# david-m-rosen/Optimization

Hardware: AMD Instinct MI355X
Metric: TNT Steihaug-CG HVP+inner-product throughput (higher is better)
Workload: dtype f64

## Files before the change

### include/mi355opt.h

```cpp
#ifndef MI355OPT_H
#define MI355OPT_H

#include <stddef.h>
#include <stdint.h>

#ifdef __cplusplus
extern "C" {
#endif

#define MI_API __attribute__((visibility("default")))

typedef enum mi_status {
  MI_OK = 0,
  MI_ERR_INVALID_ARGUMENT = 1,
  MI_ERR_HIP = 2,
  MI_ERR_OOM = 3,
  MI_ERR_NO_DEVICE = 4,
  MI_ERR_COMM = 5,
  MI_ERR_INTERNAL = 6,
  MI_DECLINED = 7
} mi_status;

typedef struct mi_ctx mi_ctx;
typedef struct mi_vec mi_vec;
typedef struct mi_csr mi_csr;
typedef struct mi_bsr3 mi_bsr3;
typedef struct mi_op mi_op;
typedef struct mi_precon mi_precon;
typedef struct mi_stiefel_rq mi_stiefel_rq;
typedef struct mi_so3n mi_so3n;

MI_API const char *mi_version(void);
MI_API const char *mi_last_error(void);
MI_API const char *mi_status_string(int status);
MI_API int mi_device_count(int *count);
MI_API int mi_ctx_create(int device, mi_ctx **out);
MI_API int mi_ctx_destroy(mi_ctx *ctx);
MI_API int mi_ctx_sync(mi_ctx *ctx);
MI_API int mi_ctx_sync_count(mi_ctx *ctx, size_t *count);
typedef struct mi_fusion_counters {
  unsigned long long fused_stpcg_solves;
  unsigned long long generic_stpcg_solves;
  unsigned long long fused_lsqr_solves;
  unsigned long long generic_lsqr_solves;
  unsigned long long fused_trial_steps;
  unsigned long long generic_trial_steps;
  unsigned long long generic_inner_products;
} mi_fusion_counters;
enum { MI_GENERIC_STPCG = 0, MI_GENERIC_LSQR = 1, MI_GENERIC_TRIAL = 2 };
MI_API int mi_ctx_fusion_counters(mi_ctx *ctx, mi_fusion_counters *out);
MI_API int mi_ctx_fusion_counters_reset(mi_ctx *ctx);
MI_API int mi_ctx_note_generic(mi_ctx *ctx, int what, const char *why);
MI_API int mi_ctx_stream(mi_ctx *ctx, void **stream);
MI_API int mi_ctx_device_name(mi_ctx *ctx, char *buf, size_t buflen);
MI_API int mi_ctx_pool_bytes(mi_ctx *ctx, size_t *bytes_reserved);

enum {
  MI_K_NONE = 0,
  MI_K_CG_INIT, MI_K_CG_DOT3, MI_K_CG_SCALAR_A, MI_K_CG_UPDATE, MI_K_CG_SCALAR_B, MI_K_CG_PUPDATE,
  MI_K_SPMM, MI_K_STIEFEL_SPMM_GRAM, MI_K_STIEFEL_GRAM_REDUCE, MI_K_STIEFEL_FINISH_DOTS,
  MI_K_STIEFEL_RETRACT, MI_K_BSR3_SPMV_DOTS, MI_K_BLAS1, MI_K_LOBPCG_GRAM, MI_K_LOBPCG_UPDATE,
  MI_K_LOBPCG_RESIDUAL, MI_K_STIEFEL_HESS_FUSED,
  MI_K_COMM_ALLREDUCE,
  MI_K_COMM_HALO,
  MI_K_SO3_GRAD,
  MI_K_SO3_RESIDUAL,
  MI_K_SO3_JAC,
  MI_K_SO3_JACT,
  MI_K_SO3_EDGE_WEIGHT,
  MI_K_SO3_INC_REWEIGHT,
  MI_K_COUNT
};
MI_API int mi_ctx_set_option(mi_ctx *ctx, const char *name, long value);
MI_API int mi_ktime_enable(mi_ctx *ctx, int kernel_id, int on);
MI_API int mi_ktime_reset(mi_ctx *ctx);
MI_API int mi_ktime_read(mi_ctx *ctx, int kernel_id, size_t *launches, double *total_ms);
MI_API const char *mi_kernel_name(int kernel_id);
MI_API int mi_range_push(const char *name);
MI_API int mi_range_pop(void);
MI_API int mi_timer_start(mi_ctx *ctx);
MI_API int mi_timer_stop(mi_ctx *ctx, double *ms);

MI_API int mi_vec_create(mi_ctx *ctx, size_t n, mi_vec **out);
MI_API int mi_vec_destroy(mi_vec *v);
MI_API int mi_vec_view(const mi_vec *base, size_t offset, size_t n, mi_vec **out);
MI_API int mi_vec_len(const mi_vec *v, size_t *n);
MI_API int mi_vec_data(const mi_vec *v, void **device_ptr);
MI_API int mi_vec_touch(mi_vec *v);
MI_API int mi_vec_upload(mi_vec *v, const double *host, size_t n);
MI_API int mi_vec_download(const mi_vec *v, double *host, size_t n);
MI_API int mi_vec_copy(mi_vec *dst, const mi_vec *src);
MI_API int mi_vec_fill(mi_vec *v, double a);
MI_API int mi_vec_scale(mi_vec *v, double a);
MI_API int mi_vec_div(mi_vec *v, double a);
MI_API int mi_vec_scale_to(mi_vec *z, double a, const mi_vec *x);
MI_API int mi_vec_axpy(mi_vec *y, double a, const mi_vec *x);
MI_API int mi_vec_axpby(mi_vec *z, double a, const mi_vec *x, double b, const mi_vec *y);
MI_API int mi_vec_dot(const mi_vec *x, const mi_vec *y, double *out);
MI_API int mi_vec_dot_batch(mi_ctx *ctx, int k, const mi_vec *const *x, const mi_vec *const *y,
                            double *out);

MI_API int mi_csr_create(mi_ctx *ctx, size_t n, size_t nnz, const int32_t *rowptr,
                         const int32_t *col, const double *val, mi_csr **out);
MI_API int mi_csr_destroy(mi_csr *A);
MI_API int mi_csr_spmm(const mi_csr *A, int p, const mi_vec *V, mi_vec *W);

typedef int (*mi_apply_fn)(void *user, const mi_vec *in, mi_vec *out);
MI_API int mi_op_create_callback(mi_ctx *ctx, size_t n, mi_apply_fn fn, void *user, mi_op **out);
MI_API int mi_op_create_callback_rect(mi_ctx *ctx, size_t n_in, size_t n_out, mi_apply_fn fn, void *user,
                                      mi_op **out);
typedef struct mi_fused_args {
  double *partials;
  size_t partial_stride;
  int max_rows;
  int required_rows;
  void *stream;
} mi_fused_args;
typedef int (*mi_apply_fused_fn)(void *user, const mi_vec *in, mi_vec *out, const mi_fused_args *args, int *rows);
MI_API int mi_op_create_callback_fused(mi_ctx *ctx, size_t n, mi_apply_fn fn, mi_apply_fused_fn fused, void *user,
                                       mi_op **out);
MI_API int mi_op_create_diag(mi_ctx *ctx, const mi_vec *d, mi_op **out);
MI_API int mi_op_create_csr(mi_ctx *ctx, const mi_csr *A, int p, mi_op **out);
MI_API int mi_op_create_compose(mi_ctx *ctx, mi_op *outer, mi_op *inner, mi_op **out);
MI_API int mi_op_apply(mi_op *op, const mi_vec *in, mi_vec *out);
MI_API int mi_op_dims(const mi_op *op, size_t *n_in, size_t *n_out);
MI_API int mi_op_destroy(mi_op *op);

MI_API int mi_precon_create_callback(mi_ctx *ctx, size_t n, mi_apply_fn fn, void *user,
                                     mi_precon **out);
MI_API int mi_precon_create_diag(mi_ctx *ctx, const mi_vec *dinv, mi_precon **out);
MI_API int mi_precon_create_block3(mi_ctx *ctx, const mi_vec *inv_blocks, mi_precon **out);
MI_API int mi_precon_create_constraint(mi_ctx *ctx, size_t n, size_t m, const mi_vec *A_rowmajor,
                                       const mi_vec *Minv_diag, mi_precon **out);
MI_API int mi_precon_create_constraint_csr(mi_ctx *ctx, size_t n, size_t m, const int32_t *rowptr, const int32_t *col,
                                           const double *val, const mi_vec *Minv, double inner_tol,
                                           size_t inner_max_iterations, mi_precon **out);
MI_API int mi_precon_constraint_info(mi_precon *P, size_t *last_inner_iterations, double *last_relative_residual,
                                     double *worst_relative_residual, int *status_code );
MI_API int mi_precon_constraint_solve(mi_precon *P, const mi_vec *r, mi_vec *v, mi_vec *lambda );
MI_API int mi_precon_constraint_At(mi_precon *P, const mi_vec *lambda, mi_vec *out);
MI_API int mi_precon_apply(mi_precon *P, const mi_vec *r, mi_vec *v);
MI_API int mi_precon_destroy(mi_precon *P);

typedef struct mi_stpcg_params {
  double Delta;
  size_t max_iterations;
  double kappa_fgr;
  double theta;
  double epsilon;
  int run_ahead;
  int constraint_At;
  int defer_result;
} mi_stpcg_params;

enum {
  MI_STPCG_EXIT_RESIDUAL = 0,
  MI_STPCG_EXIT_MAXIT = 1,
  MI_STPCG_EXIT_KERNEL = 2,
  MI_STPCG_EXIT_BOUNDARY = 3,
  MI_STPCG_EXIT_USER = 4
};

typedef struct mi_stpcg_result {
  double update_step_M_norm;
  size_t num_iterations;
  int exit_reason;
  size_t hvp_calls;
  double rv_final;
  int precon_status;
} mi_stpcg_result;

typedef struct mi_stpcg_trace {
  size_t cap, len;
  double *alpha, *beta, *kappa, *rv;
} mi_stpcg_trace;

MI_API void mi_stpcg_default_params(mi_stpcg_params *p);
MI_API int mi_stpcg(mi_ctx *ctx, const mi_vec *g, mi_op *H, mi_precon *P ,
                    const mi_stpcg_params *params, mi_vec *s_out, mi_stpcg_result *result,
                    mi_stpcg_trace *trace );
MI_API int mi_stpcg_observer_available(mi_ctx *ctx, const char **why);
typedef int (*mi_stpcg_observer)(void *user, size_t k, const mi_vec *s, const mi_vec *r, const mi_vec *v,
                                 const mi_vec *p, double alpha);
MI_API int mi_stpcg_observed(mi_ctx *ctx, const mi_vec *g, mi_op *H, mi_precon *P ,
                             const mi_stpcg_params *params, mi_stpcg_observer fn, void *user, mi_vec *s_out,
                             mi_stpcg_result *result, mi_stpcg_trace *trace );
MI_API int mi_stpcg_collect(mi_ctx *ctx, mi_stpcg_result *result);

typedef struct mi_lsqr_params {
  size_t max_iterations;
  double lambda;
  double btol, Atol;
  double Acond_limit;
  double Delta;
  int run_ahead;
} mi_lsqr_params;
enum {
  MI_LSQR_EXIT_MAXIT = 0,
  MI_LSQR_EXIT_S1 = 1,
  MI_LSQR_EXIT_S2 = 2,
  MI_LSQR_EXIT_S3 = 3,
  MI_LSQR_EXIT_S4 = 4,
  MI_LSQR_EXIT_TRIVIAL = 5,
  MI_LSQR_EXIT_USER = 6
};
typedef struct mi_lsqr_result {
  double xnorm;
  size_t num_iterations;
  int exit_reason;
  double rbar_norm, Arnorm, Anorm, Acond;
  size_t operator_applications;
} mi_lsqr_result;
MI_API void mi_lsqr_default_params(mi_lsqr_params *p);
MI_API int mi_lsqr(mi_ctx *ctx, mi_op *A, mi_op *At, const mi_vec *b, const mi_lsqr_params *params,
                   mi_vec *x_out, mi_lsqr_result *result);
MI_API int mi_lsqr_observer_available(mi_ctx *ctx, const char **why);
typedef int (*mi_lsqr_observer)(void *user, size_t k, const mi_vec *x, double xnorm, double rbar_norm, double Arnorm,
                                double Anorm, double Acond);
MI_API int mi_lsqr_observed(mi_ctx *ctx, mi_op *A, mi_op *At, const mi_vec *b, const mi_lsqr_params *params,
                            mi_lsqr_observer fn, void *user, mi_vec *x_out, mi_lsqr_result *result);


MI_API int mi_stiefel_gram(mi_ctx *ctx, size_t n, int p, const mi_vec *X, const mi_vec *Z,
                           double *G_host );
MI_API int mi_stiefel_project(mi_ctx *ctx, size_t n, int p, const mi_vec *X, const mi_vec *Z,
                              mi_vec *out);
MI_API int mi_stiefel_retract(mi_ctx *ctx, size_t n, int p, const mi_vec *X, const mi_vec *V,
                              mi_vec *Y);
MI_API int mi_stiefel_rq_create(mi_ctx *ctx, const mi_csr *A, size_t n, int p, mi_stiefel_rq **out);
MI_API int mi_stiefel_rq_destroy(mi_stiefel_rq *prob);
MI_API int mi_stiefel_rq_objective(mi_stiefel_rq *prob, const mi_vec *X, double *f);
MI_API int mi_stiefel_rq_model(mi_stiefel_rq *prob, const mi_vec *X, mi_vec *grad, mi_op **hess);
MI_API int mi_stiefel_rq_trial(mi_stiefel_rq *prob, const mi_vec *X, const mi_vec *h, const mi_vec *g,
                               mi_vec *X_trial, double out[5]);
MI_API int mi_stiefel_rq_armijo_trial(mi_stiefel_rq *prob, const mi_vec *X, const mi_vec *g, double t, mi_vec *h_out,
                                      mi_vec *X_trial, double out[2]);
MI_API int mi_stiefel_rq_precon(mi_stiefel_rq *prob, const mi_vec *X, const mi_vec *dinv_rows,
                                mi_precon **out);

MI_API int mi_so3n_create(mi_ctx *ctx, size_t N, size_t n_edges, const int32_t *ei,
                          const int32_t *ej, const double *Rt , const double *w,
                          mi_so3n **out);
MI_API int mi_so3n_destroy(mi_so3n *prob);
MI_API int mi_so3n_objective(mi_so3n *prob, const mi_vec *R, double *f);
MI_API int mi_so3n_model(mi_so3n *prob, const mi_vec *R, mi_vec *grad, mi_op **hess,
                         mi_precon **block_jacobi );
MI_API int mi_so3n_retract(mi_so3n *prob, const mi_vec *R, const mi_vec *xi, mi_vec *Y);
MI_API int mi_so3n_trial(mi_so3n *prob, const mi_vec *R, const mi_vec *h, const mi_vec *g, int with_precon,
                         mi_vec *R_trial, double out[6]);
MI_API int mi_so3n_gradient(mi_so3n *prob, const mi_vec *R, mi_vec *grad);
MI_API int mi_so3n_armijo_trial(mi_so3n *prob, const mi_vec *R, const mi_vec *g, double t, mi_vec *h_out,
                                mi_vec *R_trial, double out[2]);
MI_API int mi_so3n_residual(mi_so3n *prob, const mi_vec *R, mi_vec *F_out, double *sqnorm_or_null);
MI_API int mi_so3n_jacobian(mi_so3n *prob, const mi_vec *R, mi_op **dF, mi_op **dFt);
MI_API int mi_so3n_gn_scaling(mi_so3n *prob, mi_op **M);
typedef struct mi_so3n_cert mi_so3n_cert;
struct mi_panel_blocks;
MI_API int mi_so3n_certificate(mi_so3n *prob, const mi_vec *R, mi_so3n_cert **out, double info[3]);
MI_API int mi_so3n_cert_apply(mi_so3n_cert *cert, int k, const mi_vec *X, mi_vec *Z);
MI_API int mi_so3n_cert_apply_blocks(mi_so3n_cert *cert, const struct mi_panel_blocks *X, mi_vec *Z);
MI_API int mi_so3n_cert_null_panel(mi_so3n_cert *cert, mi_vec **Y);
MI_API int mi_so3n_laplacian(mi_so3n *prob, mi_so3n_cert **out);
MI_API int mi_so3n_lap_jacobi(mi_so3n *prob, int k, const mi_vec *X, mi_vec *Z);
MI_API int mi_so3n_round(mi_so3n *prob, const mi_vec *V, mi_vec *R, double info[4]);
MI_API int mi_so3n_project(mi_so3n *prob, const mi_vec *M, mi_vec *R, double info[3]);
enum { MI_ROBUST_L2 = 0, MI_ROBUST_HUBER = 1, MI_ROBUST_CAUCHY = 2, MI_ROBUST_GEMAN_MCCLURE = 3 };
MI_API int mi_so3n_reweight(mi_so3n *prob, const mi_vec *R, int kind, double c, double info[3]);
MI_API int mi_so3n_weights(mi_so3n *prob, double *w_host );

MI_API int mi_lobpcg_gram(mi_ctx *ctx, size_t m, int ka, int kb, const mi_vec *S, const mi_vec *AS,
                          double *G_host);
MI_API int mi_lobpcg_gram_split(mi_ctx *ctx, size_t m, int k, const mi_vec *S, int k1, const mi_vec *T1,
                                const mi_vec *T2, double *G_host);
MI_API int mi_lobpcg_gram_pair(mi_ctx *ctx, size_t m, int k, const mi_vec *S, int k1a, const mi_vec *Ta1,
                               const mi_vec *Ta2, int k1b, const mi_vec *Tb1, const mi_vec *Tb2, double *Ga_host,
                               double *Gb_host);
MI_API int mi_lobpcg_gram_pair_sym(mi_ctx *ctx, size_t m, int k, const mi_vec *S, int k1a, const mi_vec *Ta1,
                                   const mi_vec *Ta2, double *Ga_host, double *Gb_host);
typedef struct mi_panel_blocks {
  int nblocks;
  const mi_vec *block[3];
  int cols[3];
} mi_panel_blocks;
MI_API int mi_lobpcg_gram_pair_sym_blocks(mi_ctx *ctx, size_t m, const mi_panel_blocks *S, int k1a, const mi_vec *Ta1,
                                          const mi_vec *Ta2, double *Ga_host, double *Gb_host);
MI_API int mi_lobpcg_gram_pair_sym_tblocks(mi_ctx *ctx, size_t m, const mi_panel_blocks *S, const mi_panel_blocks *T,
                                           double *Ga_host, double *Gb_host);
MI_API int mi_lobpcg_gram_pair_gen_blocks(mi_ctx *ctx, size_t m, const mi_panel_blocks *S, const mi_panel_blocks *AS,
                                          const mi_panel_blocks *BS, double *Ga_host, double *Gb_host);
MI_API int mi_lobpcg_update2_blocks(mi_ctx *ctx, size_t m, const mi_panel_blocks *S, int kc, const double *C_host,
                                    int ldc, mi_vec *Y, int k1, mi_vec *Y2);
MI_API int mi_csr_spmm_colmajor_blocks(const mi_csr *A, const mi_panel_blocks *X, mi_vec *Y);
MI_API int mi_lobpcg_update(mi_ctx *ctx, size_t m, int ks, int kc, const mi_vec *S,
                            const double *C_host, int ldc, mi_vec *Y);
MI_API int mi_lobpcg_update2(mi_ctx *ctx, size_t m, int ks, int kc, const mi_vec *S, const double *C_host, int ldc,
                             mi_vec *Y, int k1, mi_vec *Y2);
MI_API int mi_lobpcg_residual(mi_ctx *ctx, size_t m, int nx, const mi_vec *AX, const mi_vec *BX,
                              const mi_vec *X, const double *theta_host, mi_vec *R, double *rnorm,
                              double *xnorm);
MI_API int mi_rayleigh_ritz(int n, const double *A, const double *B, double *Theta, double *C);
MI_API int mi_rayleigh_ritz_lowest(int n, int k, const double *A, const double *B, double *Theta, double *C);
MI_API int mi_csr_spmm_colmajor(const mi_csr *A, int k, const mi_vec *X, mi_vec *Y);
MI_API int mi_csr_spmm_colmajor_residual(const mi_csr *A, int nx, const mi_vec *X, const double *theta_host,
                                         mi_vec *AX, mi_vec *R, double *rnorm, double *xnorm);
MI_API int mi_panel_rowscale(mi_ctx *ctx, size_t m, int k, const mi_vec *d, const mi_vec *X, mi_vec *Y);

#define MI_COMM_UID_BYTES 128
MI_API int mi_comm_unique_id(unsigned char uid[MI_COMM_UID_BYTES]);
MI_API int mi_comm_init(mi_ctx *ctx, int world_size, int rank,
                        const unsigned char uid[MI_COMM_UID_BYTES]);
MI_API int mi_comm_finalize(mi_ctx *ctx);
MI_API int mi_comm_info(mi_ctx *ctx, int *world_size, int *rank);
MI_API int mi_comm_rccl_count(mi_ctx *ctx, int *nranks);
#define MI_COMM_IPC_HANDLE_BYTES 64
MI_API int mi_comm_ipc_export(mi_ctx *ctx, unsigned char handle[MI_COMM_IPC_HANDLE_BYTES]);
MI_API int mi_comm_ipc_attach(mi_ctx *ctx, int world_size, int rank,
                              const unsigned char *handles );
MI_API int mi_comm_ipc_selftest(mi_ctx *ctx, int *ok);
MI_API int mi_comm_ipc_enable(mi_ctx *ctx, int on);
MI_API int mi_comm_ipc_error(mi_ctx *ctx, int *err);
MI_API int mi_comm_ipc_fold(mi_ctx *ctx, int on);
MI_API int mi_comm_kernel_launches(mi_ctx *ctx, unsigned long long out[4]);
MI_API int mi_debug_csr_window_info(const mi_csr *A, size_t out[4]);
MI_API int mi_debug_csr_format_info(const mi_csr *A, size_t out[5]);
MI_API int mi_debug_so3n_info(const mi_so3n *q, size_t out[6]);
MI_API int mi_debug_op_apply_sub_scaled(mi_op *op, const mi_vec *in, double scale, int mode, mi_vec *inout,
                                        double *sqnorm);
MI_API int mi_debug_window_runs(int ntiles, int max_wgs, int num_cu, size_t far_stride, int *bounds_out, int cap,
                                int *nb_out);
MI_API int mi_debug_stiefel_hess_form(int p, int gram_count, const size_t traits[9], const int switches[9], int out[14]);
MI_API int mi_debug_stiefel_hess_form_of(const mi_ctx *ctx, const mi_csr *A, int p, int gram_count, int out[14]);
MI_API int mi_debug_words16_option(const char *text, int *on);
MI_API int mi_debug_set_rank(mi_ctx *ctx, int world_size, int rank);
MI_API int mi_debug_csr_set_halo(mi_csr *A, int p, const double *halo_rows_host);
MI_API int mi_debug_time_fused_apply(mi_op *op, const mi_vec *in, mi_vec *out, int reps, double *us_per_call);
MI_API int mi_csr_shard_plan(size_t n_global, int world_size, int rank, const size_t *row_starts,
                             size_t nnz_local, const int64_t *col_global, int32_t *col_local, size_t *need_lo,
                             size_t *need_hi);
MI_API int mi_csr_create_sharded(mi_ctx *ctx, size_t n_global, size_t row_begin, size_t row_end,
                                 size_t nnz_local, const int32_t *rowptr, const int64_t *col_global,
                                 const double *val, const size_t *row_starts ,
                                 mi_csr **out);

#ifdef __cplusplus
}
#endif
#endif
```

### optimization_amd/build.py

```python
import concurrent.futures
import glob
import os
import subprocess
import sys

HERE = os.path.dirname(os.path.abspath(__file__))
ROOT = os.path.dirname(HERE)
CSRC = os.path.join(HERE, "csrc")
_TAG = os.environ.get("MI355OPT_BUILD_TAG", "")
OBJ = os.path.join(HERE, "_build" + ("_" + _TAG if _TAG else ""))
LIB = os.path.join(HERE, "libmi355opt" + ("_" + _TAG if _TAG else "") + ".so")
HIPCC = os.environ.get("HIPCC", "/opt/rocm/bin/hipcc")
ARCH = "gfx950"

CFLAGS = [
    f"--offload-arch={ARCH}", "-O3", "-std=c++17", "-fPIC", "-fvisibility=hidden",
    "-fgpu-rdc" if False else "-fno-gpu-rdc", "-Wall", "-Wno-unused-function",
    "-I", os.path.join(ROOT, "include"), "-I", CSRC, "-I", os.path.join(HERE, "include"), "-I", "/opt/rocm/include",
]
CFLAGS += os.environ.get("MI355OPT_EXTRA_CFLAGS", "").split()
LDFLAGS = ["-shared", "-L/opt/rocm/lib", "-lrccl", "-ldl", "-Wl,-rpath,/opt/rocm/lib", "-Wl,--no-undefined"]


def _newer(src, dst, deps):
    if not os.path.exists(dst):
        return True
    t = os.path.getmtime(dst)
    return any(os.path.getmtime(f) > t for f in [src] + deps)


def _compile(src, force):
    obj = os.path.join(OBJ, os.path.basename(src) + ".o")
    deps = glob.glob(os.path.join(CSRC, "*.h")) + glob.glob(os.path.join(ROOT, "include", "*.h")) + \
        glob.glob(os.path.join(HERE, "include", "Optimization", "LinearAlgebra", "DenseSymmetricEigen.h"))
    if not force and not _newer(src, obj, deps):
        return obj, False, ""
    cmd = [HIPCC] + CFLAGS + ["-c", src, "-o", obj]
    r = subprocess.run(cmd, capture_output=True, text=True)
    if r.returncode != 0:
        raise RuntimeError(f"hipcc failed on {src}:\n{r.stderr[-6000:]}")
    return obj, True, r.stderr


HOST_CXX = os.environ.get("CXX", "g++")
HOST_CFLAGS = ["-O3", "-std=c++17", "-fPIC", "-fvisibility=hidden", "-ffp-contract=off", "-Wall",
               "-I", os.path.join(ROOT, "include"), "-I", CSRC, "-I", os.path.join(HERE, "include")]


def _compile_host(src, force):
    obj = os.path.join(OBJ, os.path.basename(src) + ".o")
    deps = glob.glob(os.path.join(HERE, "include", "Optimization", "LinearAlgebra", "*.h"))
    if not force and not _newer(src, obj, deps):
        return obj, False, ""
    import shutil
    if shutil.which(HOST_CXX):
        cmd = [HOST_CXX] + HOST_CFLAGS
    else:
        cmd = [HIPCC, "-x", "c++"] + HOST_CFLAGS
    r = subprocess.run(cmd + ["-c", src, "-o", obj], capture_output=True, text=True)
    if r.returncode != 0:
        raise RuntimeError(f"{cmd[0]} failed on {src}:\n{r.stderr[-6000:]}")
    return obj, True, r.stderr


UNITY = ["stpcg.hip", "stiefel.hip"]


def build(force=False, jobs=None, verbose=False):
    os.makedirs(OBJ, exist_ok=True)
    srcs = sorted(glob.glob(os.path.join(CSRC, "*.hip")))
    if not srcs:
        raise RuntimeError("no HIP sources found")
    if os.environ.get("MI355OPT_NO_UNITY") != "1":
        unity = os.path.join(OBJ, "hot_unity.hip")
        text = "".join(f'#include "{os.path.join(CSRC, u)}"\n' for u in UNITY)
        if not os.path.exists(unity) or open(unity).read() != text:
            with open(unity, "w") as f:
                f.write(text)
        newest = max(os.path.getmtime(os.path.join(CSRC, u)) for u in UNITY)
        if os.path.getmtime(unity) < newest:
            os.utime(unity, (newest, newest))
        srcs = [s_ for s_ in srcs if os.path.basename(s_) not in UNITY] + [unity]
    jobs = jobs or min(len(srcs), os.cpu_count() or 4)
    objs, rebuilt = [], False
    with concurrent.futures.ThreadPoolExecutor(max_workers=jobs) as ex:
        for obj, did, err in ex.map(lambda s: _compile(s, force), srcs):
            objs.append(obj)
            rebuilt |= did
            if verbose and err.strip():
                print(err, file=sys.stderr)
    for src in sorted(glob.glob(os.path.join(CSRC, "*.cpp"))):
        obj, did, err = _compile_host(src, force)
        objs.append(obj)
        rebuilt |= did
    if rebuilt or not os.path.exists(LIB):
        cmd = [HIPCC, f"--offload-arch={ARCH}"] + objs + LDFLAGS + ["-o", LIB]
        r = subprocess.run(cmd, capture_output=True, text=True)
        if r.returncode != 0:
            raise RuntimeError(f"link failed:\n{r.stderr[-6000:]}")
    return LIB


WLGEN_SRC = os.path.join(HERE, "wlgen.c")
WLGEN_LIB = os.path.join(HERE, "libmi355wl.so")


def build_wlgen(force=False):
    if force or _newer(WLGEN_SRC, WLGEN_LIB, []):
        r = subprocess.run(["gcc", "-O2", "-ffp-contract=off", "-fPIC", "-shared", "-Wall", "-Wextra", WLGEN_SRC,
                            "-o", WLGEN_LIB, "-lm"], capture_output=True, text=True)
        if r.returncode != 0:
            raise RuntimeError("wlgen build failed:\n" + r.stderr[-4000:])
    return WLGEN_LIB


def build_harness(force=False):
    tdir = os.path.join(ROOT, "tests", "cpp")
    inc = ["-I", os.path.join(HERE, "include"), "-I", os.path.join(ROOT, "oracle")]
    common = ["g++", "-std=c++17", "-O2", "-ffp-contract=off", "-fPIC", "-shared", "-Wall", "-Wno-type-limits"]
    hdrs = glob.glob(os.path.join(HERE, "include", "Optimization", "*", "*.h")) + \
        glob.glob(os.path.join(ROOT, "oracle", "*.inc")) + glob.glob(os.path.join(ROOT, "include", "*.h"))
    out = []
    host_src = os.path.join(tdir, "harness_host.cpp")
    host_so = os.path.join(tdir, "libharness_host.so")
    if force or _newer(host_src, host_so, hdrs):
        r = subprocess.run(common + ["-march=x86-64-v3"] + inc + [host_src, "-o", host_so],
                           capture_output=True, text=True)
        if r.returncode != 0:
            raise RuntimeError("host harness build failed:\n" + r.stderr[-6000:])
    out.append(host_so)
    dev_src = os.path.join(tdir, "harness_device.cpp")
    dev_so = os.path.join(tdir, "libharness_device.so")
    if force or _newer(dev_src, dev_so, hdrs + [LIB]):
        cmd = common + inc + ["-I", os.path.join(ROOT, "include"), dev_src, "-o", dev_so, "-L", HERE,
                              "-lmi355opt", "-Wl,-rpath," + HERE, "-Wl,-rpath,/opt/rocm/lib"]
        r = subprocess.run(cmd, capture_output=True, text=True)
        if r.returncode != 0:
            raise RuntimeError("device harness build failed:\n" + r.stderr[-6000:])
        clang = "/opt/rocm/lib/llvm/bin/clang++"
        if os.path.exists(clang):
            r = subprocess.run([clang, "-std=c++17", "-fsyntax-only"] + inc +
                               ["-I", os.path.join(ROOT, "include"), dev_src], capture_output=True, text=True)
            if r.returncode != 0:
                raise RuntimeError("clang front-end check of the template layer failed:\n" + r.stderr[-6000:])
    out.append(dev_so)
    ob_src = os.path.join(tdir, "harness_observer.cpp")
    ob_so = os.path.join(tdir, "libharness_observer.so")
    if force or _newer(ob_src, ob_so, hdrs + [LIB]):
        cmd = common + inc + ["-I", os.path.join(ROOT, "include"), ob_src, "-o", ob_so, "-L", HERE,
                              "-lmi355opt", "-Wl,-rpath," + HERE, "-Wl,-rpath,/opt/rocm/lib"]
        r = subprocess.run(cmd, capture_output=True, text=True)
        if r.returncode != 0:
            raise RuntimeError("observer harness build failed:\n" + r.stderr[-6000:])
    out.append(ob_so)
    for name in ("harness_args", "harness_lsqr_observer", "harness_gd_so3n", "harness_tnls_so3n", "harness_certify_so3n",
                 "harness_robust_so3n", "harness_spectral_so3n"):
        src = os.path.join(tdir, name + ".cpp")
        so = os.path.join(tdir, "lib" + name + ".so")
        if force or _newer(src, so, hdrs + [LIB]):
            clang = "/opt/rocm/lib/llvm/bin/clang++"
            if os.path.exists(clang):
                r = subprocess.run([clang, "-std=c++17", "-fsyntax-only"] + inc +
                                   ["-I", os.path.join(ROOT, "include"), src], capture_output=True, text=True)
                if r.returncode != 0:
                    raise RuntimeError(f"clang front-end check of {name} failed:\n" + r.stderr[-6000:])
            cmd = common + inc + ["-I", os.path.join(ROOT, "include"), src, "-o", so, "-L", HERE,
                                  "-lmi355opt", "-Wl,-rpath," + HERE, "-Wl,-rpath,/opt/rocm/lib"]
            r = subprocess.run(cmd, capture_output=True, text=True)
            if r.returncode != 0:
                raise RuntimeError(f"{name} build failed:\n" + r.stderr[-6000:])
        out.append(so)
    sf_src = os.path.join(tdir, "harness_sinfit.hip")
    sf_so = os.path.join(tdir, "libharness_sinfit.so")
    if force or _newer(sf_src, sf_so, hdrs + [LIB]):
        cmd = [HIPCC, f"--offload-arch={ARCH}", "-std=c++17", "-O2", "-fPIC", "-shared", "-Wall",
               "-I", os.path.join(HERE, "include"), "-I", os.path.join(ROOT, "include"), sf_src, "-o", sf_so,
               "-L", HERE, "-lmi355opt", "-Wl,-rpath," + HERE, "-Wl,-rpath,/opt/rocm/lib"]
        r = subprocess.run(cmd, capture_output=True, text=True)
        if r.returncode != 0:
            raise RuntimeError("sin-fit harness build failed:\n" + r.stderr[-6000:])
    out.append(sf_so)
    bc_src = os.path.join(ROOT, "tools", "bench_client.cpp")
    bc_so = os.path.join(ROOT, "tools", "libbench_client.so")
    if force or _newer(bc_src, bc_so, hdrs + [LIB]):
        cmd = common + ["-I", os.path.join(HERE, "include"), "-I", os.path.join(ROOT, "include"), bc_src, "-o", bc_so,
                        "-L", HERE, "-lmi355opt", "-Wl,-rpath," + HERE, "-Wl,-rpath,/opt/rocm/lib"]
        r = subprocess.run(cmd, capture_output=True, text=True)
        if r.returncode != 0:
            raise RuntimeError("bench client build failed:\n" + r.stderr[-6000:])
    out.append(bc_so)
    exdir = os.path.join(ROOT, "examples")
    os.makedirs(os.path.join(exdir, "bin"), exist_ok=True)
    for src in sorted(glob.glob(os.path.join(exdir, "*.cpp"))):
        exe = os.path.join(exdir, "bin", os.path.splitext(os.path.basename(src))[0])
        if force or _newer(src, exe, hdrs + [LIB]):
            cmd = ["g++", "-std=c++17", "-O2", "-Wall"] + inc + ["-I", os.path.join(ROOT, "include"), src, "-o", exe,
                   "-L", HERE, "-lmi355opt", "-Wl,-rpath," + HERE, "-Wl,-rpath,/opt/rocm/lib"]
            r = subprocess.run(cmd, capture_output=True, text=True)
            if r.returncode != 0:
                raise RuntimeError(f"example build failed ({src}):\n" + r.stderr[-6000:])
        out.append(exe)
    for src in sorted(glob.glob(os.path.join(exdir, "*.hip"))):
        exe = os.path.join(exdir, "bin", os.path.splitext(os.path.basename(src))[0])
        if force or _newer(src, exe, hdrs + [LIB]):
            cmd = [HIPCC, f"--offload-arch={ARCH}", "-std=c++17", "-O2", "-Wall"] + inc + \
                  ["-I", os.path.join(ROOT, "include"), src, "-o", exe, "-L", HERE, "-lmi355opt",
                   "-Wl,-rpath," + HERE, "-Wl,-rpath,/opt/rocm/lib"]
            r = subprocess.run(cmd, capture_output=True, text=True)
            if r.returncode != 0:
                raise RuntimeError(f"example build failed ({src}):\n" + r.stderr[-6000:])
        out.append(exe)
    return out


class SanitizerUnavailable(RuntimeError):
    """The host has no usable ASan / UBSan toolchain or runtime: a reason to SKIP the sanitizer target, never a reason
    to refuse the GPU library."""


def _sanitizer_probe(tdir, san):
    import tempfile
    with tempfile.TemporaryDirectory(dir=tdir) as d:
        src, exe = os.path.join(d, "p.c"), os.path.join(d, "p")
        with open(src, "w") as f:
            f.write("#include <stdlib.h>\nint main(void){void*p=malloc(8);free(p);return 0;}\n")
        try:
            r = subprocess.run(["gcc"] + san + [src, "-o", exe], capture_output=True, text=True)
        except FileNotFoundError as e:
            raise SanitizerUnavailable(str(e))
        if r.returncode != 0:
            raise SanitizerUnavailable("gcc cannot build with -fsanitize=address,undefined here:\n" + r.stderr[-800:])
        for opts in ("detect_leaks=1:abort_on_error=0", "detect_leaks=0:abort_on_error=0"):
            r = subprocess.run([exe], capture_output=True, text=True, env=dict(os.environ, ASAN_OPTIONS=opts))
            if r.returncode == 0:
                if "detect_leaks=0" in opts:
                    print("[build] warning: LeakSanitizer cannot run here (ptrace / seccomp restriction?): the sanitizer "
                          "target runs with detect_leaks=0 -- heap errors and undefined behaviour are still checked, "
                          "leaks are NOT", file=sys.stderr)
                return opts
        raise SanitizerUnavailable("a trivial sanitized program does not run here:\n" + r.stderr[-800:])


_SAN = ["-fsanitize=address,undefined", "-fno-sanitize-recover=all", "-fno-omit-frame-pointer", "-g", "-O1", "-ffp-contract=off"]


def build_sanitize(force=False, run=True):
    tdir = os.path.join(ROOT, "tests", "cpp")
    odir = os.path.join(ROOT, "oracle")
    exe = os.path.join(tdir, "sanitize_host")
    src = os.path.join(tdir, "sanitize_host.cpp")
    deps = glob.glob(os.path.join(HERE, "include", "Optimization", "*", "*.h")) + glob.glob(os.path.join(odir, "*.inc")) + \
        glob.glob(os.path.join(odir, "*.[ch]")) + [os.path.join(tdir, "harness_host.cpp")]
    san = _SAN
    asan_opts = _sanitizer_probe(tdir, san)
    if force or _newer(src, exe, deps):
        objs = []
        for c in ("oracle.c", "problems.c"):
            o = os.path.join(tdir, "san_" + c + ".o")
            r = subprocess.run(["gcc"] + san + ["-I", odir, "-c", os.path.join(odir, c), "-o", o],
                               capture_output=True, text=True)
            if r.returncode != 0:
                raise RuntimeError("sanitizer build failed:\n" + r.stderr[-4000:])
            objs.append(o)
        r = subprocess.run(["g++", "-std=c++17", "-Wall", "-Wno-type-limits"] + san +
                           ["-I", os.path.join(HERE, "include"), "-I", odir, "-I", tdir, src] + objs + ["-lm", "-o", exe],
                           capture_output=True, text=True)
        if r.returncode != 0:
            raise RuntimeError("sanitizer build failed:\n" + r.stderr[-6000:])
    if run:
        r = subprocess.run([exe], capture_output=True, text=True, timeout=600,
                           env=dict(os.environ, ASAN_OPTIONS=asan_opts, UBSAN_OPTIONS="print_stacktrace=1"))
        if r.returncode != 0 or "sanitize_host: ok" not in r.stdout:
            raise RuntimeError("the template layer failed under ASan/UBSan:\n" + r.stdout[-2000:] + r.stderr[-6000:])
    if os.path.exists(os.path.join(tdir, "sanitize_so3_pack.cpp")):
        build_sanitize_so3_pack(force=force, run=run)
    return exe


def build_sanitize_so3_pack(force=False, run=True):
    tdir = os.path.join(ROOT, "tests", "cpp")
    exe, src = os.path.join(tdir, "sanitize_so3_pack"), os.path.join(tdir, "sanitize_so3_pack.cpp")
    asan_opts = _sanitizer_probe(tdir, _SAN)
    if force or _newer(src, exe, [os.path.join(CSRC, "so3_pack.h")]):
        r = subprocess.run(["g++", "-std=c++17", "-Wall"] + _SAN + ["-I", CSRC, src, "-o", exe], capture_output=True, text=True)
        if r.returncode != 0:
            raise RuntimeError("sanitizer build failed:\n" + r.stderr[-6000:])
    if run:
        r = subprocess.run([exe], capture_output=True, text=True, timeout=600,
                           env=dict(os.environ, ASAN_OPTIONS=asan_opts, UBSAN_OPTIONS="print_stacktrace=1"))
        if r.returncode != 0 or "sanitize_so3_pack: ok" not in r.stdout:
            raise RuntimeError("so3_pack.h failed under ASan/UBSan:\n" + r.stdout[-2000:] + r.stderr[-6000:])
    return exe


if __name__ == "__main__":
    force = "--force" in sys.argv
    print(build(force=force, verbose=True))
    print(build_wlgen(force=force))
    print(build_harness(force=force))
    print(build_sanitize(force=force))
```

### optimization_amd/csrc/context.hip

```cpp
#include "mi_internal.h"
#include <chrono>
#include <cstring>
#include <strings.h>
#include <unistd.h>

#include <dlfcn.h>

namespace mi {

static thread_local char g_err[1024] = "";

void set_error(const char *fmt, ...) {
  va_list ap;
  va_start(ap, fmt);
  vsnprintf(g_err, sizeof(g_err), fmt, ap);
  va_end(ap);
}

int hip_fail(hipError_t e, const char *what, const char *file, int line) {
  set_error("HIP error %d (%s) in %s at %s:%d", (int)e, hipGetErrorString(e), what, file, line);
  (void)hipGetLastError();
  if (e == hipErrorNoDevice || e == hipErrorInvalidDevice) return MI_ERR_NO_DEVICE;
  if (e == hipErrorOutOfMemory) return MI_ERR_OOM;
  return MI_ERR_HIP;
}

static int readback_reserve(mi_ctx *ctx, size_t total) {
  if (total > ctx->readback_bytes) {
    MI_HIP(hipStreamSynchronize(ctx->stream));
    if (ctx->readback_host) (void)hipHostFree(ctx->readback_host);
    ctx->readback_host = nullptr;
    ctx->readback_bytes = 0;
    const size_t cap = std::max<size_t>(total, 256 * 1024);
    MI_HIP(hipHostMalloc(&ctx->readback_host, cap, hipHostMallocMapped | hipHostMallocCoherent));
    ctx->readback_bytes = cap;
  }
  return MI_OK;
}
int readback_area(mi_ctx *ctx, size_t bytes, void **host, void **dev) {
  MI_TRY(readback_reserve(ctx, bytes));
  *host = ctx->readback_host;
  MI_HIP(hipHostGetDevicePointer(dev, ctx->readback_host, 0));
  return MI_OK;
}
__global__ void k_host_flag(unsigned long long *flag, unsigned long long seq) {
  __hip_atomic_store(flag, seq, __ATOMIC_RELEASE, __HIP_MEMORY_SCOPE_SYSTEM);
}
unsigned long long poll_begin(mi_ctx *ctx, unsigned long long **flag_dev) {
  if (!ctx->poll_flag || ctx->cfg.no_polled_sync) return 0;
  if (hipHostGetDevicePointer((void **)flag_dev, ctx->poll_flag, 0) != hipSuccess) {
    (void)hipGetLastError();
    return 0;
  }
  return ++ctx->poll_seq;
}
static inline void cpu_relax() {
#if !defined(__HIP_DEVICE_COMPILE__) && (defined(__x86_64__) || defined(__i386__))
  __builtin_ia32_pause();
#endif
}
int poll_finish(mi_ctx *ctx, unsigned long long seq, const char *what) {
  if (seq) {
    const auto t0 = std::chrono::steady_clock::now();
    for (unsigned spins = 1;; ++spins) {
      if (__atomic_load_n(ctx->poll_flag, __ATOMIC_ACQUIRE) >= seq) return MI_OK;
      cpu_relax();
      if ((spins & 1023u) == 0 && std::chrono::steady_clock::now() - t0 > std::chrono::milliseconds(2)) break;
    }
  }
  const hipError_t e = hipStreamSynchronize(ctx->stream);
  if (e != hipSuccess) return hip_fail(e, what, __FILE__, __LINE__);
  return MI_OK;
}
int stream_wait(mi_ctx *ctx, const char *what) {
  ctx->host_syncs++;
  unsigned long long *dev = nullptr;
  const unsigned long long seq = poll_begin(ctx, &dev);
  if (seq) {
    hipLaunchKernelGGL(k_host_flag, dim3(1), dim3(1), 0, ctx->stream, dev, seq);
    if (hipGetLastError() != hipSuccess) return poll_finish(ctx, 0, what);
  }
  return poll_finish(ctx, seq, what);
}
int readback_sync(mi_ctx *ctx, int n, const void *const *dev, const size_t *bytes, void *const *host) {
  size_t total = 0;
  for (int i = 0; i < n; ++i) total += (bytes[i] + 63) / 64 * 64;
  MI_TRY(readback_reserve(ctx, total));
  size_t off = 0;
  hipError_t e = hipSuccess;
  for (int i = 0; i < n && e == hipSuccess; ++i) {
    e = hipMemcpyAsync((char *)ctx->readback_host + off, dev[i], bytes[i], hipMemcpyDeviceToHost, ctx->stream);
    off += (bytes[i] + 63) / 64 * 64;
  }
  if (e == hipSuccess) e = hipStreamSynchronize(ctx->stream);
  ctx->host_syncs++;
  if (e != hipSuccess) return hip_fail(e, "read-back", __FILE__, __LINE__);
  off = 0;
  for (int i = 0; i < n; ++i) {
    memcpy(host[i], (const char *)ctx->readback_host + off, bytes[i]);
    off += (bytes[i] + 63) / 64 * 64;
  }
  return MI_OK;
}

int ensure_device() {
  int count = 0;
  hipError_t e = hipGetDeviceCount(&count);
  if (e != hipSuccess || count <= 0) {
    (void)hipGetLastError();
    set_error("no HIP device available (hipGetDeviceCount: %s, count=%d); libmi355opt has no CPU "
              "fallback",
              hipGetErrorString(e), count);
    return MI_ERR_NO_DEVICE;
  }
  return MI_OK;
}

int pool_alloc(mi_ctx *ctx, size_t bytes, void **out) {
  if (bytes == 0) bytes = 8;
  bytes = (bytes + 255) & ~(size_t)255;
  auto it = ctx->pool_free.find(bytes);
  if (it != ctx->pool_free.end()) {
    *out = it->second;
    ctx->pool_free.erase(it);
    return MI_OK;
  }
  void *p = nullptr;
  hipError_t e = hipMalloc(&p, bytes);
  if (e != hipSuccess) {
    for (auto &kv : ctx->pool_free) {
      (void)hipFree(kv.second);
      ctx->pool_all.erase(kv.second);
      ctx->pool_bytes -= kv.first;
    }
    ctx->pool_free.clear();
    (void)hipGetLastError();
    e = hipMalloc(&p, bytes);
    if (e != hipSuccess) return hip_fail(e, "hipMalloc", __FILE__, __LINE__);
  }
  ctx->pool_all[p] = bytes;
  ctx->pool_bytes += bytes;
  *out = p;
  return MI_OK;
}

void pool_free(mi_ctx *ctx, void *p) {
  if (!p) return;
  auto it = ctx->pool_all.find(p);
  if (it == ctx->pool_all.end()) return;
  ctx->pool_free.insert({it->second, p});
}

int upload(void **dst, const void *src, size_t bytes) {
  void *p = nullptr;
  MI_HIP(hipMalloc(&p, bytes ? bytes : 8));
  const hipError_t e = bytes ? hipMemcpy(p, src, bytes, hipMemcpyHostToDevice) : hipSuccess;
  if (e != hipSuccess) {
    (void)hipFree(p);
    return hip_fail(e, "hipMemcpy(p, src, bytes, hipMemcpyHostToDevice)", __FILE__, __LINE__);
  }
  *dst = p;
  return MI_OK;
}

int stage_upload(mi_ctx *ctx, const void *src, size_t bytes, void *dst_dev) {
  MI_REQUIRE(bytes <= mi_ctx::kStageBytes, "staged upload of %zu bytes exceeds the slot size", bytes);
  const int slot = ctx->stage_next;
  ctx->stage_next = (slot + 1) % mi_ctx::kStageSlots;
  if (!ctx->stage_host[slot]) {
    MI_HIP(hipHostMalloc(&ctx->stage_host[slot], mi_ctx::kStageBytes, hipHostMallocDefault));
    MI_HIP(hipEventCreateWithFlags(&ctx->stage_ev[slot], hipEventDisableTiming));
  } else {
    MI_HIP(hipEventSynchronize(ctx->stage_ev[slot]));
  }
  memcpy(ctx->stage_host[slot], src, bytes);
  MI_HIP(hipMemcpyAsync(dst_dev, ctx->stage_host[slot], bytes, hipMemcpyHostToDevice, ctx->stream));
  MI_HIP(hipEventRecord(ctx->stage_ev[slot], ctx->stream));
  return MI_OK;
}

hipEvent_t event_get(mi_ctx *ctx) {
  if (!ctx->event_pool.empty()) {
    hipEvent_t e = ctx->event_pool.back();
    ctx->event_pool.pop_back();
    return e;
  }
  hipEvent_t e = nullptr;
  if (hipEventCreate(&e) != hipSuccess) return nullptr;
  return e;
}

KScope::KScope(mi_ctx *c, int kid) : ctx(c), id(kid) {
  if (ctx->ktime[id].enabled) {
    e0 = event_get(ctx);
    e1 = event_get(ctx);
    if (e0) (void)hipEventRecord(e0, ctx->stream);
  }
}
KScope::~KScope() {
  if (e0 && e1) {
    (void)hipEventRecord(e1, ctx->stream);
    ctx->ktime[id].pending.push_back({e0, e1});
  }
}

}

using namespace mi;

namespace {
struct OptionDesc {
  const char *name;
  int (*set)(mi_ctx *, long);
  bool integer = false;
};
#define OPT_BOOL(FN, FIELD) \
  int FN(mi_ctx *c, long v) { c->FIELD = v != 0; return MI_OK; }
OPT_BOOL(opt_force_slot_path, force_slot_path)
OPT_BOOL(opt_force_lockstep, force_lockstep)
OPT_BOOL(opt_no_dirgram, no_dirgram)
OPT_BOOL(opt_dirgram_direct, dirgram_direct)
OPT_BOOL(opt_force_uniform_grid, cfg.force_uniform_grid)
OPT_BOOL(opt_no_fold, cfg.no_fold)
OPT_BOOL(opt_halo_push_late, cfg.halo_push_late)
OPT_BOOL(opt_no_packed, cfg.no_packed)
OPT_BOOL(opt_no_window, cfg.no_window)
OPT_BOOL(opt_no_win_bounds, cfg.no_win_bounds)
OPT_BOOL(opt_no_far_computed, cfg.no_far_computed)
OPT_BOOL(opt_words16, cfg.words16)
OPT_BOOL(opt_no_spmm_stream, cfg.no_spmm_stream)
OPT_BOOL(opt_no_spmm_win, cfg.no_spmm_win)
OPT_BOOL(opt_no_spmm_sweep, cfg.no_spmm_sweep)
OPT_BOOL(opt_no_zero_copy, cfg.no_zero_copy)
OPT_BOOL(opt_no_polled_sync, cfg.no_polled_sync)
OPT_BOOL(opt_no_update_mfma, cfg.no_update_mfma)
OPT_BOOL(opt_halo_rprime, cfg.halo_rprime)
OPT_BOOL(opt_no_gram_half, cfg.no_gram_half)
OPT_BOOL(opt_so3_no_quat, cfg.so3_no_quat)
OPT_BOOL(opt_so3_no_rquat, cfg.so3_no_rquat)
OPT_BOOL(opt_early_s, cfg.early_s)
OPT_BOOL(opt_defer_s, cfg.defer_s)
OPT_BOOL(opt_no_fused_observer, cfg.no_fused_observer)
OPT_BOOL(opt_no_fused_lsqr_observer, cfg.no_fused_lsqr_observer)
OPT_BOOL(opt_no_update_pair, cfg.no_update_pair)
OPT_BOOL(opt_two_kernel_step, cfg.two_kernel_step)
OPT_BOOL(opt_warn_generic, warn_generic)
OPT_BOOL(opt_tall_prologue, cfg.tall_prologue)
#undef OPT_BOOL
int opt_max_grid(mi_ctx *c, long v) {
  c->max_grid = (int)std::min<long>(kMaxGrid, std::max<long>(1, v));
  return MI_OK;
}
int opt_wide_quad(mi_ctx *c, long v) {
  c->cfg.wide_quad = v < 0 ? -1 : v != 0;
  return MI_OK;
}
int opt_wide_window(mi_ctx *c, long v) {
  c->cfg.wide_window = v < 0 ? -1 : v != 0;
  return MI_OK;
}
int opt_so3_sort_nbr(mi_ctx *c, long v) {
  c->cfg.so3_sort_nbr = (int)v;
  return MI_OK;
}
int opt_sweep_zsegs(mi_ctx *c, long v) {
  c->cfg.sweep_zsegs = (int)std::max<long>(0, std::min<long>(v, 1024));
  return MI_OK;
}
int opt_reanchor(mi_ctx *c, long v) {
  c->cfg.reanchor = (int)std::max<long>(0, std::min<long>(v, 1 << 20));
  return MI_OK;
}
int opt_ipc_timeout_ms(mi_ctx *c, long v) {
  c->cfg.ipc_timeout_ms = std::max<long>(0, v);
  return MI_OK;
}
const OptionDesc kOptions[] = {
    {"FORCE_SLOT_PATH", opt_force_slot_path}, {"FORCE_LOCKSTEP", opt_force_lockstep},
    {"NO_DIRGRAM", opt_no_dirgram}, {"DIRGRAM_DIRECT", opt_dirgram_direct}, {"MAX_GRID", opt_max_grid, true},
    {"FORCE_UNIFORM_GRID", opt_force_uniform_grid}, {"IPC_TIMEOUT_MS", opt_ipc_timeout_ms, true},
    {"NO_FOLD", opt_no_fold}, {"HALO_PUSH_LATE", opt_halo_push_late}, {"NO_PACKED", opt_no_packed},
    {"NO_WINDOW", opt_no_window}, {"NO_WIN_BOUNDS", opt_no_win_bounds}, {"NO_FAR_COMPUTED", opt_no_far_computed},
    {"WORDS16", opt_words16, true}, {"NO_SPMM_STREAM", opt_no_spmm_stream}, {"NO_SPMM_WIN", opt_no_spmm_win},
    {"NO_SPMM_SWEEP", opt_no_spmm_sweep}, {"SWEEP_ZSEGS", opt_sweep_zsegs, true},
    {"NO_ZERO_COPY", opt_no_zero_copy}, {"NO_POLLED_SYNC", opt_no_polled_sync}, {"WIDE_QUAD", opt_wide_quad, true}, {"WIDE_WINDOW", opt_wide_window, true},
    {"NO_UPDATE_MFMA", opt_no_update_mfma}, {"HALO_RPRIME", opt_halo_rprime}, {"NO_GRAM_HALF", opt_no_gram_half}, {"SO3_NO_QUAT", opt_so3_no_quat}, {"SO3_NO_RQUAT", opt_so3_no_rquat}, {"EARLY_S", opt_early_s}, {"DEFER_S", opt_defer_s}, {"NO_FUSED_OBSERVER", opt_no_fused_observer}, {"NO_FUSED_LSQR_OBSERVER", opt_no_fused_lsqr_observer}, {"NO_UPDATE_PAIR", opt_no_update_pair}, {"TWO_KERNEL_STEP", opt_two_kernel_step}, {"SO3_SORT_NBR", opt_so3_sort_nbr, true},
    {"WARN_GENERIC", opt_warn_generic}, {"TALL_PROLOGUE", opt_tall_prologue}, {"REANCHOR", opt_reanchor, true},
};
bool option_value(const OptionDesc &o, const char *e, long *v) {
  char *end = nullptr;
  *v = strtol(e, &end, 0);
  if (end != e && *end == '\0') return true;
  if (o.integer) {
    fprintf(stderr, "[mi355opt] warning: MI355OPT_%s=\"%s\" is not an integer; ignored (the default stays)\n", o.name, e);
    return false;
  }
  *v = (!strcasecmp(e, "no") || !strcasecmp(e, "false") || !strcasecmp(e, "off")) ? 0 : 1;
  return true;
}
void config_from_env(mi_ctx *ctx) {
  for (const OptionDesc &o : kOptions) {
    char name[64];
    snprintf(name, sizeof(name), "MI355OPT_%s", o.name);
    long v = 0;
    if (const char *e = getenv(name))
      if (option_value(o, e, &v)) (void)o.set(ctx, v);
  }
  static bool warned = false;
  if (warned || !environ) return;
  warned = true;
  for (char **ep = environ; *ep; ++ep) {
    if (strncmp(*ep, "MI355OPT_", 9) != 0) continue;
    const char *nm = *ep + 9, *eq = strchr(nm, '=');
    const size_t len = eq ? (size_t)(eq - nm) : strlen(nm);
    bool known = false;
    for (const OptionDesc &o : kOptions) known |= strlen(o.name) == len && strncmp(o.name, nm, len) == 0;
    for (const char *h : {"LIB", "COMM", "BUILD_TAG", "EXTRA_CFLAGS", "NO_UNITY"})
      known |= strlen(h) == len && strncmp(h, nm, len) == 0;
    known |= len >= 6 && strncmp(nm, "BENCH_", 6) == 0;
    if (!known)
      fprintf(stderr, "[mi355opt] warning: environment variable MI355OPT_%.*s is not a switch of this build (removed "
                      "or misspelt?); it changes nothing\n", (int)len, nm);
  }
}
}

extern "C" {

const char *mi_version(void) { return "mi355opt 0.1.0 (gfx950)"; }
const char *mi_last_error(void) { return g_err; }
const char *mi_status_string(int s) {
  switch (s) {
    case MI_OK: return "ok";
    case MI_ERR_INVALID_ARGUMENT: return "invalid argument";
    case MI_ERR_HIP: return "HIP runtime error";
    case MI_ERR_OOM: return "out of device memory";
    case MI_ERR_NO_DEVICE: return "no MI355X/HIP device (no CPU fallback)";
    case MI_ERR_COMM: return "RCCL communicator error";
    case MI_ERR_INTERNAL: return "internal error";
    case MI_DECLINED: return "declined (nothing was done)";
  }
  return "unknown status";
}

static const char *kKernelNames[MI_K_COUNT] = {
    "none", "cg_init", "cg_dot3", "cg_scalar_a", "cg_update", "cg_scalar_b", "cg_pupdate",
    "csr_spmm", "stiefel_spmm_gram", "stiefel_gram_reduce", "stiefel_finish_dots",
    "stiefel_retract", "bsr3_spmv_dots", "blas1", "lobpcg_gram", "lobpcg_update",
    "lobpcg_residual", "stiefel_hess_fused", "comm_allreduce", "comm_halo", "so3_grad",
    "so3_residual", "so3_jac", "so3_jact", "so3_edge_weight", "so3_inc_reweight"};
const char *mi_kernel_name(int id) {
  if (id < 0 || id >= MI_K_COUNT) return "?";
  return kKernelNames[id];
}

int mi_ctx_set_option(mi_ctx *ctx, const char *name, long value) {
  MI_REQUIRE(ctx && name, "null argument");
  if (strncmp(name, "MI355OPT_", 9) == 0) name += 9;
  for (const OptionDesc &o : kOptions)
    if (strcmp(o.name, name) == 0) return o.set(ctx, value);
  set_error("unknown option '%s'", name);
  return MI_ERR_INVALID_ARGUMENT;
}

int mi_debug_words16_option(const char *text, int *on) {
  MI_REQUIRE(on, "null argument");
  mi_ctx scratch;
  long v = 0;
  for (const OptionDesc &o : kOptions)
    if (strcmp(o.name, "WORDS16") == 0 && text && option_value(o, text, &v)) (void)o.set(&scratch, v);
  *on = scratch.cfg.words16;
  return MI_OK;
}

int mi_device_count(int *count) {
  MI_REQUIRE(count, "count is null");
  int c = 0;
  hipError_t e = hipGetDeviceCount(&c);
  if (e != hipSuccess) {
    (void)hipGetLastError();
    c = 0;
  }
  *count = c;
  return MI_OK;
}

static int ctx_init(mi_ctx *ctx, int device) {
  ctx->device = device;
  hipDeviceProp_t prop;
  MI_HIP(hipGetDeviceProperties(&prop, device));
  snprintf(ctx->device_name, sizeof(ctx->device_name), "%s (%s, %d CUs)",
           prop.name[0] ? prop.name : "AMD Instinct", prop.gcnArchName, prop.multiProcessorCount);
  ctx->num_cu = prop.multiProcessorCount;
  MI_HIP(hipStreamCreateWithFlags(&ctx->stream, hipStreamNonBlocking));
  const size_t pbytes = sizeof(double) * kMaxComps * kMaxRows;
  const size_t slab_bytes = 4u << 20;
  MI_HIP(hipMalloc((void **)&ctx->control_slab, slab_bytes));
  MI_HIP(hipMemsetAsync(ctx->control_slab, 0, slab_bytes, ctx->stream));
  {
    char *top = (char *)ctx->control_slab;
    auto carve = [&](size_t bytes) {
      char *p = top;
      top += (bytes + 255) / 256 * 256;
      return p;
    };
    ctx->cg = (CgState *)carve(2 * sizeof(CgState));
    ctx->cg1 = ctx->cg + 1;
    ctx->scalars = (double *)carve(sizeof(double) * kScalarSlots);
    ctx->partials = (double *)carve(pbytes);
    ctx->partials_b = (double *)carve(pbytes);
    ctx->partials2 = (double *)carve(pbytes);
    ctx->partials_user = (double *)carve(pbytes);
    if ((size_t)(top - (char *)ctx->control_slab) > slab_bytes) {
      set_error("control slab overflow");
      return MI_ERR_INTERNAL;
    }
  }
  MI_HIP(hipHostMalloc((void **)&ctx->host_scalars, sizeof(double) * kScalarSlots,
                       hipHostMallocMapped | hipHostMallocCoherent));
  MI_HIP(hipHostMalloc((void **)&ctx->cg_host, sizeof(CgState) + 16, hipHostMallocMapped | hipHostMallocCoherent)  );
  MI_HIP(hipHostMalloc((void **)&ctx->status, sizeof(HostStatus),
                       hipHostMallocMapped | hipHostMallocCoherent));
  MI_HIP(hipHostMalloc((void **)&ctx->poll_flag, 64, hipHostMallocMapped | hipHostMallocCoherent));
  *ctx->poll_flag = 0;
  memset((void *)ctx->status, 0, sizeof(HostStatus));
  MI_HIP(hipHostGetDevicePointer((void **)&ctx->status_dev, (void *)ctx->status, 0));
  config_from_env(ctx);
  MI_HIP(hipEventCreate(&ctx->t_start));
  MI_HIP(hipEventCreate(&ctx->t_stop));
  return MI_OK;
}

int mi_comm_finalize(mi_ctx *ctx);
int mi_ctx_destroy(mi_ctx *ctx);

int mi_ctx_create(int device, mi_ctx **out) {
  MI_REQUIRE(out, "out is null");
  MI_TRY(ensure_device());
  MI_HIP(hipSetDevice(device));
  mi_ctx *ctx = new mi_ctx();
  const int st = ctx_init(ctx, device);
  if (st != MI_OK) {
    (void)mi_ctx_destroy(ctx);
    return st;
  }
  *out = ctx;
  return MI_OK;
}

int mi_ctx_destroy(mi_ctx *ctx) {
  if (!ctx) return MI_OK;
  (void)hipSetDevice(ctx->device);
  if (ctx->stream) (void)hipStreamSynchronize(ctx->stream);
  (void)mi_comm_finalize(ctx);
  for (auto &kv : ctx->pool_all) (void)hipFree(kv.first);
  for (int i = 0; i < MI_K_COUNT; ++i)
    for (auto &pr : ctx->ktime[i].pending) {
      (void)hipEventDestroy(pr.first);
      (void)hipEventDestroy(pr.second);
    }
  for (auto e : ctx->event_pool) (void)hipEventDestroy(e);
  for (int i = 0; i < mi_ctx::kStageSlots; ++i) {
    if (ctx->stage_ev[i]) (void)hipEventDestroy(ctx->stage_ev[i]);
    if (ctx->stage_host[i]) (void)hipHostFree(ctx->stage_host[i]);
  }
  (void)hipFree(ctx->control_slab);
  (void)hipFree(ctx->trace_dev);
  (void)hipHostFree(ctx->host_scalars);
  if (ctx->readback_host) (void)hipHostFree(ctx->readback_host);
  if (ctx->poll_flag) (void)hipHostFree(ctx->poll_flag);
  if (ctx->cg_deferred_ev) (void)hipEventDestroy(ctx->cg_deferred_ev);
  (void)hipHostFree(ctx->cg_host);
  (void)hipHostFree((void *)ctx->status);
  if (ctx->t_start) (void)hipEventDestroy(ctx->t_start);
  if (ctx->t_stop) (void)hipEventDestroy(ctx->t_stop);
  if (ctx->stream) (void)hipStreamDestroy(ctx->stream);
  (void)hipGetLastError();
  delete ctx;
  return MI_OK;
}

int mi_ctx_sync(mi_ctx *ctx) {
  MI_REQUIRE(ctx, "ctx is null");
  MI_HIP(hipStreamSynchronize(ctx->stream));
  ctx->host_syncs++;
  return MI_OK;
}

int mi_ctx_sync_count(mi_ctx *ctx, size_t *count) {
  MI_REQUIRE(ctx && count, "null argument");
  *count = ctx->host_syncs;
  return MI_OK;
}

int mi_ctx_fusion_counters(mi_ctx *ctx, mi_fusion_counters *out) {
  MI_REQUIRE(ctx && out, "null argument");
  *out = ctx->fusion;
  return MI_OK;
}

int mi_ctx_fusion_counters_reset(mi_ctx *ctx) {
  MI_REQUIRE(ctx, "ctx is null");
  ctx->fusion = mi_fusion_counters{0, 0, 0, 0, 0, 0, 0};
  return MI_OK;
}

int mi_ctx_note_generic(mi_ctx *ctx, int what, const char *why) {
  MI_REQUIRE(ctx, "ctx is null");
  MI_REQUIRE(what >= 0 && what <= 2, "bad kind %d", what);
  static const char *const kKind[3] = {"STPCG", "LSQR", "TNT / GradientDescent trial step"};
  if (what == MI_GENERIC_STPCG) ctx->fusion.generic_stpcg_solves++;
  if (what == MI_GENERIC_LSQR) ctx->fusion.generic_lsqr_solves++;
  if (what == MI_GENERIC_TRIAL) ctx->fusion.generic_trial_steps++;
  if (ctx->warn_generic && !ctx->warned_generic[what]) {
    ctx->warned_generic[what] = true;
    fprintf(stderr, "[mi355opt] note (MI355OPT_WARN_GENERIC): %s on MI355::DeviceVector runs the GENERIC loop (every inner "
                    "product waits for the device): %s\n", kKind[what], why ? why : "a target<>() probe failed");
  }
  return MI_OK;
}

int mi_ctx_stream(mi_ctx *ctx, void **stream) {
  MI_REQUIRE(ctx && stream, "null argument");
  *stream = (void *)ctx->stream;
  return MI_OK;
}

int mi_ctx_device_name(mi_ctx *ctx, char *buf, size_t buflen) {
  MI_REQUIRE(ctx && buf && buflen, "null argument");
  snprintf(buf, buflen, "%s", ctx->device_name);
  return MI_OK;
}

int mi_ctx_pool_bytes(mi_ctx *ctx, size_t *bytes) {
  MI_REQUIRE(ctx && bytes, "null argument");
  *bytes = ctx->pool_bytes;
  return MI_OK;
}

int mi_ktime_enable(mi_ctx *ctx, int id, int on) {
  MI_REQUIRE(ctx && id > 0 && id < MI_K_COUNT, "bad kernel id %d", id);
  ctx->ktime[id].enabled = on != 0;
  return MI_OK;
}

static int ktime_resolve(mi_ctx *ctx, int id) {
  KTimer &t = ctx->ktime[id];
  if (t.pending.empty()) return MI_OK;
  MI_HIP(hipStreamSynchronize(ctx->stream));
  for (auto &pr : t.pending) {
    float ms = 0;
    MI_HIP(hipEventElapsedTime(&ms, pr.first, pr.second));
    t.total_ms += ms;
    t.launches++;
    ctx->event_pool.push_back(pr.first);
    ctx->event_pool.push_back(pr.second);
  }
  t.pending.clear();
  return MI_OK;
}

int mi_ktime_reset(mi_ctx *ctx) {
  MI_REQUIRE(ctx, "ctx is null");
  for (int i = 1; i < MI_K_COUNT; ++i) {
    MI_TRY(ktime_resolve(ctx, i));
    ctx->ktime[i].launches = 0;
    ctx->ktime[i].total_ms = 0;
  }
  return MI_OK;
}

int mi_ktime_read(mi_ctx *ctx, int id, size_t *launches, double *total_ms) {
  MI_REQUIRE(ctx && id > 0 && id < MI_K_COUNT, "bad kernel id %d", id);
  MI_TRY(ktime_resolve(ctx, id));
  if (launches) *launches = ctx->ktime[id].launches;
  if (total_ms) *total_ms = ctx->ktime[id].total_ms;
  return MI_OK;
}

namespace {
struct Roctx {
  int (*push)(const char *) = nullptr;
  int (*pop)() = nullptr;
  Roctx() {
    void *h = dlopen("librocprofiler-sdk-roctx.so.1", RTLD_NOW | RTLD_GLOBAL);
    if (!h) h = dlopen("librocprofiler-sdk-roctx.so", RTLD_NOW | RTLD_GLOBAL);
    if (!h) h = dlopen("libroctx64.so.4", RTLD_NOW | RTLD_GLOBAL);
    if (!h) h = dlopen("libroctx64.so", RTLD_NOW | RTLD_GLOBAL);
    if (!h) return;
    push = reinterpret_cast<int (*)(const char *)>(dlsym(h, "roctxRangePushA"));
    pop = reinterpret_cast<int (*)()>(dlsym(h, "roctxRangePop"));
  }
};
Roctx &roctx() {
  static Roctx r;
  return r;
}
}

int mi_range_push(const char *name) {
  MI_REQUIRE(name, "range name is null");
  if (roctx().push) (void)roctx().push(name);
  return MI_OK;
}

int mi_range_pop(void) {
  if (roctx().pop) (void)roctx().pop();
  return MI_OK;
}

int mi_timer_start(mi_ctx *ctx) {
  MI_REQUIRE(ctx, "ctx is null");
  MI_HIP(hipEventRecord(ctx->t_start, ctx->stream));
  return MI_OK;
}

int mi_timer_stop(mi_ctx *ctx, double *ms) {
  MI_REQUIRE(ctx && ms, "null argument");
  MI_HIP(hipEventRecord(ctx->t_stop, ctx->stream));
  MI_HIP(hipEventSynchronize(ctx->t_stop));
  float f = 0;
  MI_HIP(hipEventElapsedTime(&f, ctx->t_start, ctx->t_stop));
  *ms = f;
  return MI_OK;
}

}
```

### optimization_amd/csrc/mi_internal.h

```cpp
#pragma once

#include <hip/hip_runtime.h>

#include <cstdarg>
#include <cstdint>
#include <cstdio>
#include <cstring>
#include <map>
#include <memory>
#include <string>
#include <set>
#include <vector>

#include "mi355opt.h"

namespace mi {

constexpr int kWave = 64;
constexpr int kBlock = 1024;
constexpr int kWaves = kBlock / kWave;
constexpr int kMaxP = 8;
constexpr int kMaxGrid = 512;
constexpr int kMaxRows = 1024;
constexpr int kMaxComps = 64;
constexpr int kNumXCD = 8;
constexpr int kScalarSlots = 256;

void set_error(const char *fmt, ...);
int hip_fail(hipError_t e, const char *what, const char *file, int line);

#define MI_HIP(expr)                                                   \
  do {                                                                 \
    hipError_t _e = (expr);                                            \
    if (_e != hipSuccess) return ::mi::hip_fail(_e, #expr, __FILE__, __LINE__); \
  } while (0)

#define MI_TRY(expr)          \
  do {                        \
    int _s = (expr);          \
    if (_s != MI_OK) return _s; \
  } while (0)

#define MI_REQUIRE(cond, ...)              \
  do {                                     \
    if (!(cond)) {                         \
      ::mi::set_error(__VA_ARGS__);        \
      return MI_ERR_INVALID_ARGUMENT;      \
    }                                      \
  } while (0)

#define DISPATCH_P(p, ...)                                          \
  switch (p) {                                                      \
    case 1: { constexpr int P = 1; __VA_ARGS__; } break;            \
    case 2: { constexpr int P = 2; __VA_ARGS__; } break;            \
    case 3: { constexpr int P = 3; __VA_ARGS__; } break;            \
    case 4: { constexpr int P = 4; __VA_ARGS__; } break;            \
    case 5: { constexpr int P = 5; __VA_ARGS__; } break;            \
    case 6: { constexpr int P = 6; __VA_ARGS__; } break;            \
    case 7: { constexpr int P = 7; __VA_ARGS__; } break;            \
    case 8: { constexpr int P = 8; __VA_ARGS__; } break;            \
    default: set_error("p must be in [1,%d], got %d", kMaxP, p); return MI_ERR_INVALID_ARGUMENT; \
  }
#define DISPATCH_P4(p, ...)                                         \
  switch (p) {                                                      \
    case 1: { constexpr int P = 1; __VA_ARGS__; } break;            \
    case 2: { constexpr int P = 2; __VA_ARGS__; } break;            \
    case 3: { constexpr int P = 3; __VA_ARGS__; } break;            \
    case 4: { constexpr int P = 4; __VA_ARGS__; } break;            \
    default: set_error("internal: narrow-row kernel asked for p = %d", p); return MI_ERR_INTERNAL; \
  }
#define DISPATCH_3(x, NAME, A, B, C, ...)                   \
  switch (x) {                                              \
    case A: { constexpr int NAME = A; __VA_ARGS__; } break; \
    case B: { constexpr int NAME = B; __VA_ARGS__; } break; \
    default: { constexpr int NAME = C; __VA_ARGS__; } break; \
  }
#define DISPATCH_FLAG(x, NAME, ...)                       \
  if (x) { constexpr bool NAME = true; __VA_ARGS__; }     \
  else { constexpr bool NAME = false; __VA_ARGS__; }

struct HostStatus {
  volatile uint64_t word;
  volatile uint32_t epoch;
};

struct CgState {
  double sk_M_pk, sk_M_2, pk_M_2;
  double target_rk_norm;
  double rv;
  double alpha, beta, kappa, sigma;
  double skplus1_M_2;
  double M_norm;
  unsigned long long k;
  unsigned long long launches;
  int mode;
  int exit_reason;
  double alpha_prev;
};
static_assert(sizeof(CgState) <= 128, "the CG state is meant to fit one 128-byte line");
struct CgConst {
  double Delta, Delta_2, epsilon;
  unsigned long long max_iterations;
  unsigned long long rag0, rag_per;
};
enum CgMode { CG_RUN = 0, CG_KERNEL_PENDING = 1, CG_APPLY_SIGMA = 2, CG_DONE = 3 };

struct Config {
  bool force_uniform_grid = false;
  long ipc_timeout_ms = 0;
  bool no_fold = false;
  bool halo_push_late = false;
  bool no_packed = false;
  bool no_window = false;
  bool no_win_bounds = false;
  bool no_far_computed = false;
  bool words16 = true;
  bool no_spmm_stream = false;
  bool no_spmm_sweep = true;
  int sweep_zsegs = 0;
  bool no_spmm_win = false;
  bool no_zero_copy = false;
  int wide_quad = -1;
  int wide_window = -1;
  bool no_polled_sync = false;
  bool two_kernel_step = false;
  int reanchor = 25;
  bool no_update_pair = false;
  bool no_gram_half = false;
  bool no_update_mfma = false;
  bool halo_rprime = false;
  bool early_s = false;
  bool defer_s = true;
  bool no_fused_observer = false;
  bool no_fused_lsqr_observer = false;
  bool so3_no_rquat = false;
  bool so3_no_quat = false;
  int so3_sort_nbr = 0;
  bool tall_prologue = false;
};

struct KTimer {
  bool enabled = false;
  std::vector<std::pair<hipEvent_t, hipEvent_t>> pending;
  size_t launches = 0;
  double total_ms = 0;
};

}

struct mi_ctx {
  int device = -1;
  hipStream_t stream = nullptr;
  char device_name[128] = {0};
  int num_cu = 256;
  bool uniform_grid = false;
  int max_grid = 512;
  std::multimap<size_t, void *> pool_free;
  std::map<void *, size_t> pool_all;
  size_t pool_bytes = 0;
  void *control_slab = nullptr;
  double *partials = nullptr;
  double *partials_b = nullptr;
  double *partials2 = nullptr;
  double *partials_user = nullptr;
  double *scalars = nullptr;
  double *host_scalars = nullptr;
  mi::CgState *cg = nullptr;
  mi::CgState *cg1 = nullptr;
  mi::CgState *cg_host = nullptr;
  const double *twok_r = nullptr;
  const mi::CgState *cg_live = nullptr;
  hipEvent_t cg_deferred_ev = nullptr;
  bool cg_deferred = false;
  size_t cg_deferred_hvp = 0;
  bool cg_in_observer = false;
  bool lsqr_in_observer = false;
  unsigned long long cg_deferred_seq = 0;
  mi::HostStatus *status = nullptr;
  mi::HostStatus *status_dev = nullptr;
  double *trace_dev = nullptr;
  size_t trace_cap = 0;
  unsigned int epoch = 0;
  uint64_t vec_serial = 0;
  size_t host_syncs = 0;
  mi_fusion_counters fusion = {0, 0, 0, 0, 0, 0, 0};
  bool warn_generic = false;
  bool warned_generic[3] = {false, false, false};
  static constexpr int kStageSlots = 4;
  static constexpr size_t kStageBytes = 96 * 96 * sizeof(double);
  void *stage_host[kStageSlots] = {nullptr, nullptr, nullptr, nullptr};
  hipEvent_t stage_ev[kStageSlots] = {nullptr, nullptr, nullptr, nullptr};
  int stage_next = 0;
  void *readback_host = nullptr;
  size_t readback_bytes = 0;
  unsigned long long *poll_flag = nullptr;
  unsigned long long poll_seq = 0;
  int st_win_occ[4][2][2][2] = {};
  bool st_widewin_lds[5][2][2] = {};
  int spmm_win_occ[2][2][2][2] = {};
  mi::KTimer ktime[MI_K_COUNT];
  std::vector<hipEvent_t> event_pool;
  hipEvent_t t_start = nullptr, t_stop = nullptr;
  void *comm = nullptr;
  int world_size = 1, rank = 0;
  bool force_slot_path = false;
  bool force_lockstep = false;
  bool no_dirgram = false;
  bool dirgram_direct = false;
  mi::Config cfg;
};

struct mi_vec {
  mi_ctx *ctx;
  size_t n;
  double *d;
  bool owned;
  uint64_t serial = 0;
  uint64_t gen = 0;
  mi_vec *root = nullptr;
  uint32_t views = 0;
  bool zombie = false;
};
namespace mi {
inline void touch(mi_vec *v) {
  if (v) ++(v->root ? v->root : v)->gen;
}
inline uint64_t gen_of(const mi_vec *v) { return (v->root ? v->root : v)->gen; }
struct VecKey {
  const mi_vec *v = nullptr;
  const double *d = nullptr;
  uint64_t serial = 0, gen = 0;
  void set(const mi_vec *x) {
    v = x;
    d = x->d;
    serial = x->serial;
    gen = gen_of(x);
  }
  void clear() { v = nullptr; }
  bool is(const mi_vec *x) const { return v == x && d == x->d && serial == x->serial && gen == gen_of(x); }
};
inline bool bound_to(const mi_vec *bound, uint64_t serial, const mi_vec *x) { return x && bound == x && serial == x->serial; }
}

namespace mi {

int pool_alloc(mi_ctx *ctx, size_t bytes, void **out);
void pool_free(mi_ctx *ctx, void *p);
int upload(void **dst, const void *src, size_t bytes);

int stage_upload(mi_ctx *ctx, const void *src, size_t bytes, void *dst_dev);
int readback_sync(mi_ctx *ctx, int n, const void *const *dev, const size_t *bytes, void *const *host);
int readback_area(mi_ctx *ctx, size_t bytes, void **host, void **dev);
int stream_wait(mi_ctx *ctx, const char *what);
unsigned long long poll_begin(mi_ctx *ctx, unsigned long long **flag_dev);
int poll_finish(mi_ctx *ctx, unsigned long long seq, const char *what);
int ensure_device();

inline int uniform_grid(const mi_ctx *ctx, size_t blocks) {
  if (ctx->uniform_grid) return kMaxGrid;
  if (blocks < 1) blocks = 1;
  if (blocks > (size_t)ctx->max_grid) blocks = ctx->max_grid;
  return (int)blocks;
}

inline int grid_for(const mi_ctx *ctx, size_t n, int per_thread) {
  if (ctx->uniform_grid) return kMaxGrid;
  size_t blocks = (n + (size_t)kBlock * per_thread - 1) / ((size_t)kBlock * per_thread);
  if (blocks < 1) blocks = 1;
  if (blocks > (size_t)ctx->max_grid) blocks = ctx->max_grid;
  return (int)blocks;
}

struct RangeScope {
  explicit RangeScope(const char *name) { (void)mi_range_push(name); }
  ~RangeScope() { (void)mi_range_pop(); }
};

struct KScope {
  mi_ctx *ctx;
  int id;
  hipEvent_t e0 = nullptr, e1 = nullptr;
  KScope(mi_ctx *c, int kid);
  ~KScope();
};
hipEvent_t event_get(mi_ctx *ctx);

int comm_allreduce(mi_ctx *ctx, double *buf, int count);
int comm_allreduce_rows(mi_ctx *ctx, double *partials, int k);
bool comm_ipc_enabled(const mi_ctx *ctx);
bool comm_fold_enabled(const mi_ctx *ctx);
inline bool rows_mode(const mi_ctx *ctx) {
  return ctx->comm != nullptr && !ctx->force_slot_path && !comm_ipc_enabled(ctx);
}
inline bool slot_mode(const mi_ctx *ctx) { return ctx->force_slot_path || comm_ipc_enabled(ctx); }

int dot_batch_to_slots(mi_ctx *ctx, int k, const double *const *x, const double *const *y, size_t n,
                       int slot0);
int read_slots_sync(mi_ctx *ctx, int slot0, int k, double *out);
int launch_dot3_partials(mi_ctx *ctx, size_t n, const double *x, const double *y, int *nparts);
int launch_reduce_rows_to_slots(mi_ctx *ctx, const double *partials, int count, int k, double *slots, int nbatch = 1,
                                size_t batch_stride = 0);
int reduce_rows_allreduce(mi_ctx *ctx, const double *partials, int count, int k, double *slots);

enum { SLOT_USER = 0, SLOT_CG = 8, SLOT_GRAM = 16, SLOT_GDIR_P = 40 , SLOT_MISC = 56, SLOT_GDIR = 64,
       SLOT_RAW = 192 };
static_assert(SLOT_GRAM + 3 + 36 <= SLOT_MISC && SLOT_GDIR + SLOT_GDIR_P + 36 <= SLOT_RAW && SLOT_RAW + 64 <= kScalarSlots,
              "slot map");

__device__ __forceinline__ double wave_reduce_sum(double v) {
#pragma unroll
  for (int off = 32; off > 0; off >>= 1) v += __shfl_down(v, off, 64);
  return v;
}

__device__ __forceinline__ double sum16(const double *l) {
  return (((l[0] + l[1]) + (l[2] + l[3])) + ((l[4] + l[5]) + (l[6] + l[7]))) +
         (((l[8] + l[9]) + (l[10] + l[11])) + ((l[12] + l[13]) + (l[14] + l[15])));
}

template <int K>
__device__ __forceinline__ void block_partials_store(const double (&acc)[K], double *lds,
                                                     double *__restrict__ partials) {
  const int lane = threadIdx.x & 63, w = threadIdx.x >> 6;
#pragma unroll
  for (int k = 0; k < K; ++k) {
    const double v = wave_reduce_sum(acc[k]);
    if (lane == 0) lds[k * kWaves + w] = v;
  }
  __syncthreads();
  if (threadIdx.x < K) partials[(size_t)threadIdx.x * kMaxRows + blockIdx.x] = sum16(lds + threadIdx.x * kWaves);
  __syncthreads();
}

template <int K, int NW>
__device__ __forceinline__ void block_partials_store_nw(const double (&acc)[K], double *lds,
                                                        double *__restrict__ partials) {
  const int lane = threadIdx.x & 63, w = threadIdx.x >> 6;
#pragma unroll
  for (int k = 0; k < K; ++k) {
    const double v = wave_reduce_sum(acc[k]);
    if (lane == 0) lds[k * NW + w] = v;
  }
  __syncthreads();
  if (threadIdx.x < K) {
    double t[NW];
#pragma unroll
    for (int i = 0; i < NW; ++i) t[i] = lds[threadIdx.x * NW + i];
#pragma unroll
    for (int span = 1; span < NW; span *= 2)
#pragma unroll
      for (int i = 0; i + span < NW; i += 2 * span) t[i] = t[i] + t[i + span];
    partials[(size_t)threadIdx.x * kMaxRows + blockIdx.x] = t[0];
  }
  __syncthreads();
}

template <int K, class F>
__device__ __forceinline__ void reduce_rows_wide(const double *__restrict__ partials, int count, double (&out)[K],
                                                 double *lds, F &&after_issue) {
  const int lane = threadIdx.x & 63, w = threadIdx.x >> 6;
  constexpr int R = (K + kWaves - 1) / kWaves;
  double v[R];
#pragma unroll
  for (int q = 0; q < R; ++q) {
    const int c = w + q * kWaves;
    double t[kMaxRows / 64];
#pragma unroll
    for (int j = 0; j < kMaxRows / 64; ++j) {
      const int r = lane + 64 * j;
      t[j] = (c < K && r < count) ? partials[(size_t)c * kMaxRows + r] : 0.0;
    }
    if (q == 0) after_issue();
    double a = 0;
#pragma unroll
    for (int j = 0; j < kMaxRows / 64; ++j) a += t[j];
    v[q] = wave_reduce_sum(a);
  }
#pragma unroll
  for (int q = 0; q < R; ++q)
    if (lane == 0 && w + q * kWaves < K) lds[w + q * kWaves] = v[q];
  __syncthreads();
#pragma unroll
  for (int k = 0; k < K; ++k) out[k] = lds[k];
  __syncthreads();
}
template <int K, class F>
__device__ __forceinline__ void reduce_rows(const double *__restrict__ partials, int count,
                                            double (&out)[K], double *lds, F &&after_issue) {
  if constexpr (K > kWaves) {
    reduce_rows_wide<K>(partials, count, out, lds, after_issue);
    return;
  }
  const int lane = threadIdx.x & 63, w = threadIdx.x >> 6;
  double t[kMaxRows / 64];
#pragma unroll
  for (int j = 0; j < kMaxRows / 64; ++j) t[j] = 0.0;
  if (w < K) {
    const double *src = partials + (size_t)w * kMaxRows;
#pragma unroll
    for (int j = 0; j < kMaxRows / 64; ++j) {
      const int r = lane + 64 * j;
      if (r < count) t[j] = src[r];
    }
  }
  after_issue();
  if (w < K) {
    double v = 0;
#pragma unroll
    for (int j = 0; j < kMaxRows / 64; ++j) v += t[j];
    v = wave_reduce_sum(v);
    if (lane == 0) lds[w] = v;
  }
  __syncthreads();
#pragma unroll
  for (int k = 0; k < K; ++k) out[k] = lds[k];
  __syncthreads();
}
template <int K>
__device__ __forceinline__ void reduce_rows(const double *__restrict__ partials, int count,
                                            double (&out)[K], double *lds) {
  reduce_rows<K>(partials, count, out, lds, [] {});
}
template <int K, int NW>
__device__ __forceinline__ void reduce_rows_nw(const double *__restrict__ partials, int count, double (&out)[K],
                                               double *lds) {
  if constexpr (NW == kWaves) {
    reduce_rows<K>(partials, count, out, lds);
  } else {
    const int lane = threadIdx.x & 63, w = threadIdx.x >> 6;
    for (int c = w; c < K; c += NW) {
      const double *src = partials + (size_t)c * kMaxRows;
      double t[kMaxRows / 64];
#pragma unroll
      for (int j = 0; j < kMaxRows / 64; ++j) {
        const int r = lane + 64 * j;
        t[j] = (r < count) ? src[r] : 0.0;
      }
      double a = 0;
#pragma unroll
      for (int j = 0; j < kMaxRows / 64; ++j) a += t[j];
      a = wave_reduce_sum(a);
      if (lane == 0) lds[c] = a;
    }
    __syncthreads();
#pragma unroll
    for (int k = 0; k < K; ++k) out[k] = lds[k];
    __syncthreads();
  }
}
template <int K, int NW>
__device__ __forceinline__ void block_partials_store_w(const double (&acc)[K], double *lds, double *__restrict__ partials) {
  if constexpr (NW == kWaves) block_partials_store<K>(acc, lds, partials);
  else block_partials_store_nw<K, NW>(acc, lds, partials);
}

__device__ __forceinline__ unsigned xcd_remap(unsigned b, unsigned nb) {
  const unsigned q = nb / kNumXCD, r = nb % kNumXCD, xcd = b % kNumXCD, idx = b / kNumXCD;
  const unsigned base = (xcd < r) ? xcd * (q + 1) : r * (q + 1) + (xcd - r) * q;
  return base + idx;
}

}

struct mi_csr {
  mi_ctx *ctx = nullptr;
  size_t n = 0;
  size_t ncols = 0;
  size_t nnz = 0;
  bool symmetric = false;
  size_t padded = 0;
  size_t nslices = 0;
  long long *slice_ptr = nullptr;
  int *col = nullptr;
  double *val = nullptr;
  uint32_t *pk = nullptr;
  double *vtab = nullptr;
  int nvtab = 0;
  int vtab_zero = -1;
  int win_chunks = 0;
  int win_head = 0;
  uint32_t win_zero = 0;
  uint32_t *wk = nullptr;
  int32_t *wfar = nullptr;
  uint32_t *wk16 = nullptr;
  size_t win_far_stride = 0;
  size_t win_far_pure = 0;
  struct WinPlan {
    int *bounds = nullptr;
    int n = 0;
  };
  mutable std::map<int, WinPlan> win_plans;
  size_t halo_lo = 0, halo_hi = 0;
  size_t send_lo = 0, send_hi = 0;
  double *halo = nullptr;
  bool halo_in_arena = false;
  size_t halo_off = 0, peer_lo_rows = 0;
  size_t halo_stride = 0;
  mutable unsigned long long halo_exchanges = 0;
  const double *halo_cur() const { return halo ? halo + (halo_exchanges & 1) * halo_stride : nullptr; }
  mutable double *halo_r = nullptr;
  mutable bool halo_r_in_arena = false;
  mutable size_t halo_r_off = 0;
  mutable unsigned long long halo_r_exchanges = 0;
};

namespace mi {
inline bool csr_row_sharded(const mi_csr *A) { return A->halo_lo + A->halo_hi + A->send_lo + A->send_hi > 0; }
inline bool far_computed(size_t win_far_pure, bool no_far_computed) {
  return win_far_pure > 0 && win_far_pure < ((size_t)1 << 31) && !no_far_computed;
}
inline bool csr_far_computed(const mi_ctx *ctx, const mi_csr *A) {
  return far_computed(A->win_far_pure, ctx->cfg.no_far_computed);
}
int csr_spmv_sub_scaled(const mi_csr *A, const mi_vec *V, const double *scale, const int *mode, const int *gate,
                        mi_vec *W, double *partials, int *nparts);
int csr_spmm_dots(const mi_csr *A, int p, const mi_vec *V, mi_vec *W, int *nparts, bool *unsupported);
int comm_halo_exchange(mi_ctx *ctx, const mi_csr *A, int p, const double *V);
int comm_exchange_halo_counts(mi_ctx *ctx, size_t need_lo, size_t need_hi, size_t *send_lo,
                              size_t *send_hi, size_t *peer_lo_rows, size_t *max_halo_rows);
int comm_halo_alloc(mi_ctx *ctx, size_t bytes, double **ptr, bool *in_arena, size_t *arena_off);
void comm_halo_free(mi_ctx *ctx, double *ptr, bool in_arena);
int csr_spmm_launch(const mi_csr *A, int p, const double *V, double *W);
int window_bounds(mi_ctx *ctx, const mi_csr *A, int wgs, int ntiles, int *grid, const int **bounds_out);
}

struct mi_op {
  mi_ctx *ctx = nullptr;
  size_t n = 0;
  size_t n_out = 0;
  int (*apply)(mi_op *self, const mi_vec *in, mi_vec *out) = nullptr;
  int (*apply_dots)(mi_op *self, const mi_vec *in, mi_vec *out, int *nparts) = nullptr;
  int (*apply_sub_scaled)(mi_op *self, const mi_vec *in, const double *scale, const int *mode, const int *gate,
                          mi_vec *inout, double *partials, int *nparts) = nullptr;
  const struct mi_dirgram *dirgram = nullptr;
  int (*apply_dir)(mi_op *self, const mi_vec *in, mi_vec *out, int gram_count, int *nparts) = nullptr;
  void (*destroy)(mi_op *self) = nullptr;
  void *impl = nullptr;
  bool borrowed = false;
};

struct mi_dirgram {
  int p = 0;
  size_t n = 0;
  const double *X = nullptr;
  const double *Y = nullptr;
  const double *S = nullptr;
  const struct mi_csr *halo_A = nullptr;
  bool twok = false;
};

struct mi_precon {
  mi_ctx *ctx = nullptr;
  size_t n = 0;
  int kind = 0;
  const double *data = nullptr;
  int (*apply)(mi_precon *self, const mi_vec *r, mi_vec *v) = nullptr;
  int (*apply_project)(mi_precon *self, mi_vec *r, mi_vec *v, int subtract) = nullptr;
  void (*destroy)(mi_precon *self) = nullptr;
  void *impl = nullptr;
  bool borrowed = false;
  double *fail_word = nullptr;
};

namespace mi {

struct DevFree {
  void operator()(void *p) const { (void)hipFree(p); }
};
template <class T>
using DevPtr = std::unique_ptr<T, DevFree>;
struct HandleDestroy {
  void operator()(mi_vec *v) const { (void)mi_vec_destroy(v); }
  void operator()(mi_op *o) const {
    o->borrowed = false;
    (void)mi_op_destroy(o);
  }
  void operator()(mi_so3n_cert *c) const;
};
template <class T>
using Owned = std::unique_ptr<T, HandleDestroy>;
template <class T>
int dev_alloc(DevPtr<T> &p, size_t count) {
  void *raw = nullptr;
  MI_HIP(hipMalloc(&raw, count ? count * sizeof(T) : 8));
  p.reset((T *)raw);
  return MI_OK;
}
inline int vec_alloc(mi_ctx *ctx, size_t n, Owned<mi_vec> &out) {
  mi_vec *v = nullptr;
  MI_TRY(mi_vec_create(ctx, n, &v));
  out.reset(v);
  return MI_OK;
}
template <class T>
int dev_upload(DevPtr<T> &p, const T *src, size_t count) {
  void *raw = nullptr;
  MI_TRY(upload(&raw, src, count * sizeof(T)));
  p.reset((T *)raw);
  return MI_OK;
}

}
```

### optimization_amd/csrc/stpcg.hip

```cpp
#include "comm_ipc.h"
#include "mi_internal.h"
#include "stiefel_core.h"

#include <cmath>
#include <type_traits>

using namespace mi;

namespace {

enum { PRE_NONE = 0, PRE_DIAG = 1, PRE_BLOCK3 = 2, PRE_EXTERNAL = 3 };

__device__ __forceinline__ void publish(HostStatus *hs, unsigned long long launches, int done) {
  __hip_atomic_store(&hs->word, (uint64_t)(launches << 1) | (uint64_t)(done ? 1 : 0), __ATOMIC_RELAXED,
                     __HIP_MEMORY_SCOPE_SYSTEM);
}

#define CG_FIELDS(X)                                                                               \
  X(sk_M_pk) X(sk_M_2) X(pk_M_2) X(target_rk_norm) X(rv) X(alpha) X(beta)                          \
  X(kappa) X(sigma) X(skplus1_M_2) X(M_norm) X(k) X(launches) X(mode) X(exit_reason)
__device__ __forceinline__ CgState load_state(const CgState *__restrict__ src) {
  CgState s;
#define X(f) s.f = src->f;
  CG_FIELDS(X)
#undef X
  return s;
}
__device__ __forceinline__ void store_state(CgState *__restrict__ dst, const CgState &s) {
#define X(f) dst->f = s.f;
  CG_FIELDS(X)
#undef X
}


__device__ __forceinline__ void step_a(CgState &s, const CgConst &c, double pHp, double HpHp, double pp) {
#pragma clang fp contract(off)
  const double kappa = pHp;
  s.kappa = kappa;
  if (sqrt(HpHp) / sqrt(pp) < c.epsilon) {
    s.mode = CG_KERNEL_PENDING;
    return;
  }
  const double alpha = s.rv / kappa;
  const double skplus1 = s.sk_M_2 + 2 * alpha * s.sk_M_pk + alpha * alpha * s.pk_M_2;
  if ((kappa <= 0) || (skplus1 > c.Delta_2)) {
    s.sigma = (-s.sk_M_pk + sqrt(s.sk_M_pk * s.sk_M_pk + s.pk_M_2 * (c.Delta_2 - s.sk_M_2))) /
              s.pk_M_2;
    s.mode = CG_APPLY_SIGMA;
    s.exit_reason = MI_STPCG_EXIT_BOUNDARY;
    return;
  }
  s.alpha = alpha;
  s.skplus1_M_2 = skplus1;
}

__device__ __forceinline__ void step_b(CgState &s, const CgConst &c, double red) {
#pragma clang fp contract(off)
  if (s.mode == CG_APPLY_SIGMA) {
    s.M_norm = c.Delta;
    s.mode = CG_DONE;
    return;
  }
  if (s.mode == CG_KERNEL_PENDING) {
    double sk_M_pk = s.sk_M_pk;
    const bool flip = red < 0;
    if (flip) sk_M_pk *= -1;
    const double sigma =
        (-sk_M_pk + sqrt(sk_M_pk * sk_M_pk + s.pk_M_2 * (c.Delta_2 - s.sk_M_2))) / s.pk_M_2;
    s.sk_M_pk = sk_M_pk;
    s.sigma = flip ? -sigma : sigma;
    s.M_norm = c.Delta;
    s.exit_reason = MI_STPCG_EXIT_KERNEL;
    s.mode = CG_DONE;
    return;
  }
  const double rk_vk = red;
  const double beta = rk_vk / (s.alpha * s.kappa);
  s.sk_M_2 = s.skplus1_M_2;
  s.sk_M_pk = beta * (s.sk_M_pk + s.alpha * s.pk_M_2);
  s.pk_M_2 = rk_vk + beta * beta * s.pk_M_2;
  s.rv = rk_vk;
  s.beta = beta;
  s.k = s.k + 1;
  if (s.k >= c.max_iterations) {
    s.exit_reason = MI_STPCG_EXIT_MAXIT;
    s.M_norm = sqrt(s.sk_M_2);
    s.mode = CG_DONE;
  } else if (sqrt(rk_vk) <= s.target_rk_norm) {
    s.exit_reason = MI_STPCG_EXIT_RESIDUAL;
    s.M_norm = sqrt(s.sk_M_2);
    s.mode = CG_DONE;
  }
}

__global__ __launch_bounds__(256) void k_halo_dir(const CgState *__restrict__ st, const double *__restrict__ hr,
                                                  double *__restrict__ hp, size_t count) {
  if (st->mode != CG_RUN) return;
  const double beta = st->beta;
  for (size_t i = (size_t)blockIdx.x * 256 + threadIdx.x; i < count; i += (size_t)gridDim.x * 256)
    hp[i] = -hr[i] + beta * hp[i];
}


template <int PRE>
__global__ __launch_bounds__(kBlock) void k_cg_init(size_t n, const double *__restrict__ g,
                                                    const double *__restrict__ pre,
                                                    double *__restrict__ r, double *__restrict__ v,
                                                    double *__restrict__ p, double *__restrict__ s,
                                                    double *__restrict__ partials) {
  __shared__ double lds[kWaves];
  double acc[1] = {0};
  const size_t stride = (size_t)gridDim.x * kBlock;
  if (PRE == PRE_BLOCK3) {
    const size_t nb = n / 3;
    for (size_t b = (size_t)blockIdx.x * kBlock + threadIdx.x; b < nb; b += stride) {
      const double g0 = g[3 * b], g1 = g[3 * b + 1], g2 = g[3 * b + 2];
      const double *M = pre + 9 * b;
      const double v0 = M[0] * g0 + M[1] * g1 + M[2] * g2;
      const double v1 = M[3] * g0 + M[4] * g1 + M[5] * g2;
      const double v2 = M[6] * g0 + M[7] * g1 + M[8] * g2;
      r[3 * b] = g0; r[3 * b + 1] = g1; r[3 * b + 2] = g2;
      s[3 * b] = 0 * g0; s[3 * b + 1] = 0 * g1; s[3 * b + 2] = 0 * g2;
      v[3 * b] = v0; v[3 * b + 1] = v1; v[3 * b + 2] = v2;
      p[3 * b] = -v0; p[3 * b + 1] = -v1; p[3 * b + 2] = -v2;
      acc[0] += g0 * v0; acc[0] += g1 * v1; acc[0] += g2 * v2;
    }
  } else {
    const size_t n2 = n >> 1;
    for (size_t i = (size_t)blockIdx.x * kBlock + threadIdx.x; i < n2; i += stride) {
      const double2 gv = reinterpret_cast<const double2 *>(g)[i];
      reinterpret_cast<double2 *>(r)[i] = gv;
      reinterpret_cast<double2 *>(s)[i] = make_double2(0 * gv.x, 0 * gv.y);
      if (PRE == PRE_EXTERNAL) continue;
      double2 vv = gv;
      if (PRE == PRE_DIAG) {
        const double2 d = reinterpret_cast<const double2 *>(pre)[i];
        vv.x = d.x * gv.x; vv.y = d.y * gv.y;
        reinterpret_cast<double2 *>(v)[i] = vv;
      }
      reinterpret_cast<double2 *>(p)[i] = make_double2(-vv.x, -vv.y);
      acc[0] += gv.x * vv.x; acc[0] += gv.y * vv.y;
    }
    if ((n & 1) && blockIdx.x == 0 && threadIdx.x == 0) {
      const size_t i = n - 1;
      const double gv = g[i];
      r[i] = gv; s[i] = 0 * gv;
      if (PRE != PRE_EXTERNAL) {
        double vv = gv;
        if (PRE == PRE_DIAG) { vv = pre[i] * gv; v[i] = vv; }
        p[i] = -vv;
        acc[0] += gv * vv;
      }
    }
  }
  if (PRE == PRE_EXTERNAL) return;
  block_partials_store<1>(acc, lds, partials);
}

template <bool NEG_P>
__global__ __launch_bounds__(kBlock) void k_cg_dot_rv(size_t n, const CgState *__restrict__ st,
                                                      const double *__restrict__ r,
                                                      const double *__restrict__ v,
                                                      double *__restrict__ p,
                                                      double *__restrict__ partials) {
  __shared__ double lds[kWaves];
  if (!NEG_P && st->mode != CG_RUN) return;
  double acc[1] = {0};
  const size_t n2 = n >> 1, stride = (size_t)gridDim.x * kBlock;
  for (size_t i = (size_t)blockIdx.x * kBlock + threadIdx.x; i < n2; i += stride) {
    const double2 rv = reinterpret_cast<const double2 *>(r)[i];
    const double2 vv = reinterpret_cast<const double2 *>(v)[i];
    if (NEG_P) reinterpret_cast<double2 *>(p)[i] = make_double2(-vv.x, -vv.y);
    acc[0] += rv.x * vv.x; acc[0] += rv.y * vv.y;
  }
  if ((n & 1) && blockIdx.x == 0 && threadIdx.x == 0) {
    if (NEG_P) p[n - 1] = -v[n - 1];
    acc[0] += r[n - 1] * v[n - 1];
  }
  block_partials_store<1>(acc, lds, partials);
}

__global__ __launch_bounds__(kBlock) void k_cg_dot3(size_t n, const CgState *__restrict__ st,
                                                    const double *__restrict__ x,
                                                    const double *__restrict__ y,
                                                    double *__restrict__ partials) {
  __shared__ double lds[3 * kWaves];
  if (st && st->mode != CG_RUN) return;
  double a[3] = {0, 0, 0};
  const size_t n2 = n >> 1, stride = (size_t)gridDim.x * kBlock;
  for (size_t i = (size_t)blockIdx.x * kBlock + threadIdx.x; i < n2; i += stride) {
    const double2 xv = reinterpret_cast<const double2 *>(x)[i];
    const double2 yv = reinterpret_cast<const double2 *>(y)[i];
    a[0] += xv.x * yv.x; a[0] += xv.y * yv.y;
    a[1] += yv.x * yv.x; a[1] += yv.y * yv.y;
    a[2] += xv.x * xv.x; a[2] += xv.y * xv.y;
  }
  if ((n & 1) && blockIdx.x == 0 && threadIdx.x == 0) {
    const double xv = x[n - 1], yv = y[n - 1];
    a[0] += xv * yv; a[1] += yv * yv; a[2] += xv * xv;
  }
  block_partials_store<3>(a, lds, partials);
}

__device__ __forceinline__ void gdir_from_rows(const double *__restrict__ partials, int count, int gns,
                                               double *__restrict__ gdir) {
  const int lane = threadIdx.x & 63;
  for (int w = threadIdx.x >> 6; w < gns; w += kWaves) {
    const double *src = partials + (size_t)w * kMaxRows;
    double t[kMaxRows / 64];
#pragma unroll
    for (int j = 0; j < kMaxRows / 64; ++j) {
      const int r = lane + 64 * j;
      t[j] = (r < count) ? src[r] : 0.0;
    }
    double v = 0;
#pragma unroll
    for (int j = 0; j < kMaxRows / 64; ++j) v += t[j];
    v = wave_reduce_sum(v);
    if (lane == 0) {
      gdir[SLOT_GDIR_P + w] = v;
      gdir[w] = -v;
    }
  }
}

__device__ __forceinline__ void gdir_rows_to(const double *__restrict__ partials, int count, int gns,
                                             double *__restrict__ dst) {
  const int lane = threadIdx.x & 63;
  for (int w = threadIdx.x >> 6; w < gns; w += kWaves) {
    const double *src = partials + (size_t)w * kMaxRows;
    double t[kMaxRows / 64];
#pragma unroll
    for (int j = 0; j < kMaxRows / 64; ++j) {
      const int r = lane + 64 * j;
      t[j] = (r < count) ? src[r] : 0.0;
    }
    double v = 0;
#pragma unroll
    for (int j = 0; j < kMaxRows / 64; ++j) v += t[j];
    v = wave_reduce_sum(v);
    if (lane == 0) dst[w] = v;
  }
}

struct CgSetup {
  double Delta, kappa_fgr, theta, epsilon;
  unsigned long long max_iterations;
};

template <bool FROM_SLOTS>
__global__ __launch_bounds__(kBlock) void k_cg_scalar_init(CgState *st, CgSetup cfg,
                                                           const double *partials, int nparts,
                                                           const double *slots, HostStatus *hs,
                                                           const double *__restrict__ gpartials, int gcount, int gns,
                                                           double *__restrict__ gdir) {
#pragma clang fp contract(off)
  __shared__ double lds[kWaves + 1];
  if (gdir) gdir_from_rows(gpartials, gcount, gns, gdir);
  double red[1];
  if (FROM_SLOTS) red[0] = slots[0];
  else reduce_rows<1>(partials, nparts, red, lds);
  if (threadIdx.x != 0) return;
  CgState s;
  const double rv0 = red[0];
  s.sk_M_pk = 0;
  s.sk_M_2 = 0;
  s.pk_M_2 = rv0;
  const double r0_norm = sqrt(rv0);
  const double pw = pow(r0_norm, cfg.theta);
  s.target_rk_norm = r0_norm * ((pw < cfg.kappa_fgr) ? pw : cfg.kappa_fgr);
  s.rv = rv0;
  s.alpha = s.beta = s.kappa = s.sigma = s.skplus1_M_2 = 0;
  s.M_norm = 0;
  s.k = 0;
  s.launches = 0;
  s.exit_reason = MI_STPCG_EXIT_MAXIT;
  s.mode = CG_RUN;
  if (cfg.max_iterations == 0) {
    s.mode = CG_DONE;
    s.M_norm = sqrt(0.0);
  } else if (sqrt(rv0) <= s.target_rk_norm) {
    s.mode = CG_DONE;
    s.exit_reason = MI_STPCG_EXIT_RESIDUAL;
    s.M_norm = sqrt(0.0);
  }
  store_state(st, s);
  publish(hs, 0, s.mode == CG_DONE);
}

struct DirGramArgs {
  const double *X, *Y, *S;
  double *gpartials;
  double *gdir;
  int ns;
};

#ifdef MI_FOLD_STAMPS
}
extern "C" __attribute__((visibility("default"))) int mi_debug_fold_stamp_buffer(void *dev_ptr) {
  return (int)hipMemcpyToSymbol(HIP_SYMBOL(mi::g_fold_stamps), &dev_ptr, sizeof(dev_ptr));
}
namespace {
#endif

template <int SP>
struct DirGramLds {
  static constexpr int value = (SymIdx<SP>::NS * kWaves > kWaves + 1) ? SymIdx<SP>::NS * kWaves : kWaves + 1;
};
template <>
struct DirGramLds<0> {
  static constexpr int value = kWaves + 1;
};
static_assert(kWaves + 1 >= kIpcVals, "LDS of the folded exchange");

#define CG_KERNEL_ATTR
#define CG_UPDATE_SIGMA 1
#define CG_UPDATE_NAME k_cg_update
#define CG_PUPDATE_NAME k_cg_pupdate
#include "stpcg_kernels.inc"
#undef CG_KERNEL_ATTR
#undef CG_UPDATE_NAME
#undef CG_PUPDATE_NAME
#define CG_KERNEL_ATTR __attribute__((amdgpu_num_sgpr(80), amdgpu_waves_per_eu(8, 8)))
#define CG_UPDATE_NAME k_cg_update_s80
#define CG_PUPDATE_NAME k_cg_pupdate_s80
#include "stpcg_kernels.inc"
#undef CG_KERNEL_ATTR
#undef CG_UPDATE_NAME
#undef CG_PUPDATE_NAME
#undef CG_UPDATE_SIGMA
#define CG_UPDATE_SIGMA 0
#define CG_KERNEL_ATTR
#define CG_UPDATE_NAME k_cg_update_ns
#define CG_PUPDATE_NAME k_cg_pupdate_ns_unused
#include "stpcg_kernels.inc"
#undef CG_KERNEL_ATTR
#undef CG_UPDATE_NAME
#undef CG_PUPDATE_NAME
#define CG_KERNEL_ATTR __attribute__((amdgpu_num_sgpr(80), amdgpu_waves_per_eu(8, 8)))
#define CG_UPDATE_NAME k_cg_update_ns_s80
#define CG_PUPDATE_NAME k_cg_pupdate_ns_s80_unused
#include "stpcg_kernels.inc"
#undef CG_KERNEL_ATTR
#undef CG_UPDATE_NAME
#undef CG_PUPDATE_NAME
#undef CG_UPDATE_SIGMA

template <class F>
__device__ __forceinline__ void reduce_rows_1x512(const double *__restrict__ partials, int count, double &out, double *lds,
                                                  F &&after_issue) {
  const int lane = threadIdx.x & 63, w = threadIdx.x >> 6;
  double t[8];
#pragma unroll
  for (int j = 0; j < 8; ++j) t[j] = 0.0;
  if (w == 0) {
#pragma unroll
    for (int j = 0; j < 8; ++j) {
      const int r = lane + 64 * j;
      if (r < count) t[j] = partials[r];
    }
  }
  after_issue();
  if (w == 0) {
    double v = 0;
#pragma unroll
    for (int j = 0; j < 8; ++j) v += t[j];
    v = wave_reduce_sum(v);
    if (lane == 0) lds[0] = v;
  }
  __syncthreads();
  out = lds[0];
  __syncthreads();
}

__global__ __launch_bounds__(kBlock) __attribute__((amdgpu_waves_per_eu(8, 8))) void k_cg_pupdate_early(
    size_t n, CgConst cc, const CgState *__restrict__ st_in, CgState *__restrict__ st_out,
    const double *__restrict__ partials_b, int nparts_b, const double *__restrict__ v, double *__restrict__ p,
    double *__restrict__ s, HostStatus *hs, double *__restrict__ trace, size_t trace_cap, DirGramArgs dg) {
  __shared__ double lds[kWaves + 1];
  const unsigned n2 = (unsigned)(n >> 1), stride = gridDim.x * kBlock, i0 = blockIdx.x * kBlock + threadIdx.x;
  const unsigned tail0 = (unsigned)cc.rag0, per = (unsigned)cc.rag_per;
  const unsigned irem = (threadIdx.x < per) ? tail0 + blockIdx.x * per + threadIdx.x : n2;
  auto next_of = [&](unsigned i_) -> unsigned {
    const unsigned j_ = i_ + stride;
    return j_ < tail0 ? j_ : ((i_ < tail0 && irem < n2) ? irem : n2);
  };
  const unsigned ifirst = i0 < tail0 ? i0 : (irem < n2 ? irem : n2);
  unsigned Le[3];
  {
    unsigned L = ifirst;
#pragma unroll
    for (int j = 0; j < 3; ++j) {
      Le[j] = L;
      if (L < n2) L = next_of(L);
    }
  }
  double2 pe[3], ve[3], se[3];
  CgState cs = load_state(st_in);
  const bool leader = blockIdx.x == 0 && threadIdx.x == 0;
  if (cs.mode == CG_DONE) {
    if (leader) store_state(st_out, cs);
    return;
  }
  const int mode_in = cs.mode;
  auto early_s = [&] {
    if (mode_in != CG_RUN) return;
    const double alpha = cs.alpha;
#pragma unroll
    for (int j = 0; j < 3; ++j)
      if (Le[j] < n2) {
        pe[j] = reinterpret_cast<double2 *>(p)[Le[j]];
        se[j] = reinterpret_cast<double2 *>(s)[Le[j]];
      }
#pragma unroll
    for (int j = 0; j < 3; ++j)
      if (Le[j] < n2) ve[j] = reinterpret_cast<const double2 *>(v)[Le[j]];
#pragma unroll
    for (int j = 0; j < 3; ++j)
      if (Le[j] < n2) {
        double2 sv = se[j];
        const double2 pv = pe[j];
        sv.x = sv.x + alpha * pv.x; sv.y = sv.y + alpha * pv.y;
        reinterpret_cast<double2 *>(s)[Le[j]] = sv;
      }
  };
  double red = 0;
  if (mode_in != CG_APPLY_SIGMA) reduce_rows_1x512(partials_b, nparts_b, red, lds, early_s);
  step_b(cs, cc, red);
  cs.launches = cs.launches + 1;
  if (leader) {
    store_state(st_out, cs);
    if (mode_in == CG_RUN && trace && cs.k - 1 < trace_cap) {
      const size_t k = (size_t)(cs.k - 1);
      trace[k] = cs.alpha;
      trace[trace_cap + k] = cs.beta;
      trace[2 * trace_cap + k] = cs.kappa;
      trace[3 * trace_cap + k] = cs.rv;
    }
    publish(hs, cs.launches, cs.mode == CG_DONE);
    if (dg.gdir && mode_in == CG_RUN && cs.mode == CG_RUN) {
      for (int i = 0; i < dg.ns; ++i) dg.gdir[SLOT_GDIR_P + i] = -dg.gdir[i] + cs.beta * dg.gdir[SLOT_GDIR_P + i];
    }
  }
  if (mode_in == CG_KERNEL_PENDING) {
    const double sigma = cs.sigma;
    for (unsigned i = i0; i < n2; i += stride) {
      const double2 pv = reinterpret_cast<const double2 *>(p)[i];
      double2 sv = reinterpret_cast<double2 *>(s)[i];
      sv.x += sigma * pv.x; sv.y += sigma * pv.y;
      reinterpret_cast<double2 *>(s)[i] = sv;
    }
    if ((n & 1) && leader) s[n - 1] += sigma * p[n - 1];
  } else if (mode_in == CG_RUN) {
    const double alpha = cs.alpha, beta = cs.beta;
    const bool dir = cs.mode == CG_RUN;
    if (dir) {
#pragma unroll
      for (int j = 0; j < 3; ++j)
        if (Le[j] < n2) {
          double2 pv = pe[j];
          const double2 vv = ve[j];
          pv.x = -vv.x + beta * pv.x; pv.y = -vv.y + beta * pv.y;
          reinterpret_cast<double2 *>(p)[Le[j]] = pv;
        }
    }
    if ((n & 1) && leader) {
      s[n - 1] = s[n - 1] + alpha * p[n - 1];
      if (dir) p[n - 1] = -v[n - 1] + beta * p[n - 1];
    }
  }
}


template <bool FLUSH>
__global__ __launch_bounds__(kBlock) __attribute__((amdgpu_waves_per_eu(8, 8))) void k_cg_pupdate_ds(
    size_t n, CgConst cc, const CgState *__restrict__ st_in, CgState *__restrict__ st_out,
    const double *__restrict__ partials_b, int nparts_b, const double *__restrict__ v, const double *__restrict__ pc,
    double *__restrict__ px, double *__restrict__ s, HostStatus *hs, double *__restrict__ trace, size_t trace_cap,
    DirGramArgs dg) {
  __shared__ double lds[kWaves + 1];
  CgState cs = load_state(st_in);
  const bool leader = blockIdx.x == 0 && threadIdx.x == 0;
  if (cs.mode == CG_DONE) {
    if (leader) store_state(st_out, cs);
    return;
  }
  const int mode_in = cs.mode;
  const size_t n2 = n >> 1, stride = (size_t)gridDim.x * kBlock;
  const size_t i0 = (size_t)blockIdx.x * kBlock + threadIdx.x;
  const size_t tail0 = cc.rag0, per = cc.rag_per;
  const size_t irem = (threadIdx.x < per) ? tail0 + (size_t)blockIdx.x * per + threadIdx.x : n2;
  auto next_of = [&](size_t i_) -> size_t {
    const size_t j_ = i_ + stride;
    return j_ < tail0 ? j_ : ((i_ < tail0 && irem < n2) ? irem : n2);
  };
  const size_t ifirst = i0 < tail0 ? i0 : (irem < n2 ? irem : n2);
  double2 vv0 = make_double2(0, 0), pv0 = vv0, ov0 = vv0, sv0 = vv0;
  auto prefetch_now = [&] {
    if (ifirst < n2) {
      vv0 = reinterpret_cast<const double2 *>(v)[ifirst];
      pv0 = reinterpret_cast<const double2 *>(pc)[ifirst];
      if (FLUSH) {
        ov0 = reinterpret_cast<double2 *>(px)[ifirst];
        sv0 = reinterpret_cast<double2 *>(s)[ifirst];
      }
    }
  };
  double red[1] = {0};
  if (mode_in != CG_APPLY_SIGMA) reduce_rows<1>(partials_b, nparts_b, red, lds, prefetch_now);
  else prefetch_now();
  step_b(cs, cc, red[0]);
  cs.launches = cs.launches + 1;
  const bool dir = mode_in == CG_RUN && cs.mode == CG_RUN;
  if (leader) {
    store_state(st_out, cs);
    if (!FLUSH && dir) st_out->alpha_prev = cs.alpha;
    if (mode_in == CG_RUN && trace && cs.k - 1 < trace_cap) {
      const size_t k = (size_t)(cs.k - 1);
      trace[k] = cs.alpha;
      trace[trace_cap + k] = cs.beta;
      trace[2 * trace_cap + k] = cs.kappa;
      trace[3 * trace_cap + k] = cs.rv;
    }
    publish(hs, cs.launches, cs.mode == CG_DONE);
    if (dg.gdir && dir) {
      for (int i = 0; i < dg.ns; ++i) dg.gdir[SLOT_GDIR_P + i] = -dg.gdir[i] + cs.beta * dg.gdir[SLOT_GDIR_P + i];
    }
  }
  const double beta = cs.beta;
  if (FLUSH) {
    const double alpha_old = st_out->alpha_prev, alpha = mode_in == CG_RUN ? cs.alpha : cs.sigma;
    double2 vv = vv0, pv = pv0, ov = ov0, sv = sv0;
    for (size_t i = ifirst; i < n2;) {
      const size_t inext = next_of(i);
      double2 vn = vv, pn = pv, on = ov, sn = sv;
      if (inext < n2) {
        vn = reinterpret_cast<const double2 *>(v)[inext];
        pn = reinterpret_cast<const double2 *>(pc)[inext];
        on = reinterpret_cast<double2 *>(px)[inext];
        sn = reinterpret_cast<double2 *>(s)[inext];
      }
      sv.x = sv.x + alpha_old * ov.x; sv.y = sv.y + alpha_old * ov.y;
      sv.x = sv.x + alpha * pv.x; sv.y = sv.y + alpha * pv.y;
      reinterpret_cast<double2 *>(s)[i] = sv;
      if (dir) {
        pv.x = -vv.x + beta * pv.x; pv.y = -vv.y + beta * pv.y;
        reinterpret_cast<double2 *>(px)[i] = pv;
      }
      i = inext; vv = vn; pv = pn; ov = on; sv = sn;
    }
    if ((n & 1) && leader) {
      s[n - 1] = s[n - 1] + alpha_old * px[n - 1];
      s[n - 1] = s[n - 1] + alpha * pc[n - 1];
      if (dir) px[n - 1] = -v[n - 1] + beta * pc[n - 1];
    }
  } else if (dir) {
    double2 vv = vv0, pv = pv0;
    for (size_t i = ifirst; i < n2;) {
      const size_t inext = next_of(i);
      double2 vn = vv, pn = pv;
      if (inext < n2) {
        vn = reinterpret_cast<const double2 *>(v)[inext];
        pn = reinterpret_cast<const double2 *>(pc)[inext];
      }
      pv.x = -vv.x + beta * pv.x; pv.y = -vv.y + beta * pv.y;
      reinterpret_cast<double2 *>(px)[i] = pv;
      i = inext; vv = vn; pv = pn;
    }
    if ((n & 1) && leader) px[n - 1] = -v[n - 1] + beta * pc[n - 1];
  } else if (mode_in != CG_APPLY_SIGMA) {
    const double alpha = mode_in == CG_RUN ? cs.alpha : cs.sigma;
    for (size_t i = i0; i < n2; i += stride) {
      const double2 pv = reinterpret_cast<const double2 *>(pc)[i];
      double2 sv = reinterpret_cast<double2 *>(s)[i];
      sv.x = sv.x + alpha * pv.x; sv.y = sv.y + alpha * pv.y;
      reinterpret_cast<double2 *>(s)[i] = sv;
    }
    if ((n & 1) && leader) s[n - 1] = s[n - 1] + alpha * pc[n - 1];
  }
}


template <int NS>
__global__ __launch_bounds__(kBlock) void k_cg_step2(size_t n, CgConst cc, const CgState *__restrict__ st_in,
                                                     CgState *__restrict__ st_out, const double *__restrict__ partials_a,
                                                     int nparts_a, const double *__restrict__ Hp, double *__restrict__ r,
                                                     double *__restrict__ p, double *__restrict__ s, HostStatus *hs,
                                                     double *__restrict__ trace, size_t trace_cap, DirGramArgs dg) {
  constexpr int KC = 3 + NS + 2;
  __shared__ double lds[3 * (kWaves + 1)];
  static_assert(KC <= kWaves, "one wave per component");
  CgState cs = load_state(st_in);
  const bool leader = blockIdx.x == 0 && threadIdx.x == 0;
  if (cs.mode == CG_DONE) {
    if (leader) store_state(st_out, cs);
    return;
  }
  const size_t n2 = n >> 1, stride = (size_t)gridDim.x * kBlock, i0 = (size_t)blockIdx.x * kBlock + threadIdx.x;
  double2 hv0 = make_double2(0, 0), rv0 = hv0, pv0 = hv0, sv0 = hv0;
  auto prefetch = [&] {
    if (i0 < n2) {
      hv0 = reinterpret_cast<const double2 *>(Hp)[i0];
      rv0 = reinterpret_cast<double2 *>(r)[i0];
      pv0 = reinterpret_cast<double2 *>(p)[i0];
      sv0 = reinterpret_cast<double2 *>(s)[i0];
    }
  };
  double d[KC];
  reduce_rows<KC>(partials_a, nparts_a, d, lds, prefetch);
  step_a(cs, cc, d[0], d[1], d[2]);
  const int mode_a = cs.mode;
  double red = 0;
  {
#pragma clang fp contract(off)
    if (mode_a == CG_RUN) red = cs.rv + 2 * cs.alpha * d[KC - 2] + cs.alpha * cs.alpha * d[1];
    else if (mode_a == CG_KERNEL_PENDING) red = d[KC - 1];
  }
  step_b(cs, cc, red);
  cs.launches = cs.launches + 1;
  if (leader) {
    store_state(st_out, cs);
    if (mode_a == CG_RUN && trace && cs.k - 1 < trace_cap) {
      const size_t k = (size_t)(cs.k - 1);
      trace[k] = cs.alpha;
      trace[trace_cap + k] = cs.beta;
      trace[2 * trace_cap + k] = cs.kappa;
      trace[3 * trace_cap + k] = cs.rv;
    }
    publish(hs, cs.launches, cs.mode == CG_DONE);
    if (mode_a == CG_RUN) {
      for (int i = 0; i < NS; ++i) dg.gdir[i] = dg.gdir[i] + cs.alpha * d[3 + i];
      if (cs.mode == CG_RUN)
        for (int i = 0; i < NS; ++i) dg.gdir[SLOT_GDIR_P + i] = -dg.gdir[i] + cs.beta * dg.gdir[SLOT_GDIR_P + i];
    }
  }
  if (mode_a != CG_RUN) {
    const double sigma = cs.sigma;
    for (size_t i = i0; i < n2; i += stride) {
      const double2 pv = reinterpret_cast<const double2 *>(p)[i];
      double2 sv = reinterpret_cast<double2 *>(s)[i];
      sv.x += sigma * pv.x; sv.y += sigma * pv.y;
      reinterpret_cast<double2 *>(s)[i] = sv;
    }
    if ((n & 1) && leader) s[n - 1] += sigma * p[n - 1];
    return;
  }
  const double alpha = cs.alpha, beta = cs.beta;
  const bool dir = cs.mode == CG_RUN;
  double2 hv = hv0, rv = rv0, pv = pv0, sv = sv0;
  for (size_t i = i0; i < n2;) {
    const size_t inext = i + stride;
    double2 hn = hv, rn = rv, pn = pv, sn = sv;
    if (inext < n2) {
      hn = reinterpret_cast<const double2 *>(Hp)[inext];
      rn = reinterpret_cast<double2 *>(r)[inext];
      pn = reinterpret_cast<double2 *>(p)[inext];
      sn = reinterpret_cast<double2 *>(s)[inext];
    }
    rv.x += alpha * hv.x; rv.y += alpha * hv.y;
    reinterpret_cast<double2 *>(r)[i] = rv;
    sv.x = sv.x + alpha * pv.x; sv.y = sv.y + alpha * pv.y;
    reinterpret_cast<double2 *>(s)[i] = sv;
    if (dir) {
      pv.x = -rv.x + beta * pv.x; pv.y = -rv.y + beta * pv.y;
      reinterpret_cast<double2 *>(p)[i] = pv;
    }
    i = inext; hv = hn; rv = rn; pv = pn; sv = sn;
  }
  if ((n & 1) && leader) {
    const size_t i = n - 1;
    const double rn_ = r[i] + alpha * Hp[i];
    r[i] = rn_;
    s[i] = s[i] + alpha * p[i];
    if (dir) p[i] = -rn_ + beta * p[i];
  }
}

template <int SP>
__global__ __launch_bounds__(StBlk<SP>::threads) void k_cg_dirgram(size_t nrows, const double *__restrict__ p, DirGramArgs dg) {
  constexpr int BLK = StBlk<SP>::threads, NW = StBlk<SP>::waves;
  constexpr bool WIDE = SP > 4;
  __shared__ double lds[SymIdx<SP>::NS * NW];
  __shared__ double SmL[WIDE ? SP * SP : 1];
  double Sm[WIDE ? 1 : SP * SP], G[SP * SP];
#pragma unroll
  for (int i = 0; i < SP * SP; ++i) G[i] = 0;
  if (WIDE) {
    if (threadIdx.x < SP * SP) SmL[threadIdx.x] = dg.S[threadIdx.x];
    __syncthreads();
  } else {
#pragma unroll
    for (int i = 0; i < SP * SP; ++i) Sm[WIDE ? 0 : i] = dg.S[i];
  }
  const size_t stride = (size_t)gridDim.x * BLK;
  for (size_t row = (size_t)blockIdx.x * BLK + threadIdx.x; row < nrows; row += stride) {
    double x[SP], y[SP], pv[SP];
#pragma unroll
    for (int c = 0; c < SP; ++c) { x[c] = dg.X[row * SP + c]; y[c] = dg.Y[row * SP + c]; pv[c] = p[row * SP + c]; }
    if (WIDE) asm volatile("" ::: "memory");
#pragma unroll
    for (int b = 0; b < SP; ++b) {
      double t = 0;
#pragma unroll
      for (int a = 0; a < SP; ++a) t += pv[a] * (WIDE ? SmL[a * SP + b] : Sm[WIDE ? 0 : a * SP + b]);
#pragma unroll
      for (int a = 0; a < SP; ++a) G[a * SP + b] += y[a] * pv[b] - x[a] * t;
    }
  }
  store_sym_partials<SP>(G, lds, dg.gpartials);
}

template <int SP>
__global__ __launch_bounds__(kBlock) void k_cg_dirgram2(size_t nrows, const CgState *__restrict__ st,
                                                        const double *__restrict__ va, const double *__restrict__ vb,
                                                        DirGramArgs dg) {
  static_assert(SP >= 1 && SP <= 4, "narrow rows");
  __shared__ double lds[SymIdx<SP>::NS * kWaves];
  if (st->mode != CG_RUN) return;
  double Sm[SP * SP], Ga[SP * SP], Gb[SP * SP];
#pragma unroll
  for (int i = 0; i < SP * SP; ++i) { Ga[i] = 0; Gb[i] = 0; Sm[i] = dg.S[i]; }
  const size_t stride = (size_t)gridDim.x * kBlock;
  for (size_t row = (size_t)blockIdx.x * kBlock + threadIdx.x; row < nrows; row += stride) {
    double x[SP], y[SP], a[SP], b[SP];
#pragma unroll
    for (int c = 0; c < SP; ++c) {
      x[c] = dg.X[row * SP + c]; y[c] = dg.Y[row * SP + c]; a[c] = va[row * SP + c]; b[c] = vb[row * SP + c];
    }
#pragma unroll
    for (int j = 0; j < SP; ++j) {
      double ta = 0, tb = 0;
#pragma unroll
      for (int i = 0; i < SP; ++i) { ta += a[i] * Sm[i * SP + j]; tb += b[i] * Sm[i * SP + j]; }
#pragma unroll
      for (int i = 0; i < SP; ++i) {
        Ga[i * SP + j] += y[i] * a[j] - x[i] * ta;
        Gb[i * SP + j] += y[i] * b[j] - x[i] * tb;
      }
    }
  }
  store_sym_partials<SP>(Ga, lds, dg.gpartials);
  __syncthreads();
  store_sym_partials<SP>(Gb, lds, dg.gpartials + (size_t)SymIdx<SP>::NS * kMaxRows);
}

template <int SP>
__global__ __launch_bounds__(StBlk<SP>::threads) void k_cg_init_dirgram(size_t nrows, const double *__restrict__ g,
                                                            double *__restrict__ r, double *__restrict__ p,
                                                            double *__restrict__ s, double *__restrict__ partials,
                                                            DirGramArgs dg) {
  constexpr int BLK = StBlk<SP>::threads, NW = StBlk<SP>::waves;
  constexpr bool WIDE = SP > 4;
  __shared__ double lds[SymIdx<SP>::NS * NW];
  __shared__ double SmL[WIDE ? SP * SP : 1];
  double Sm[WIDE ? 1 : SP * SP], G[SP * SP];
#pragma unroll
  for (int i = 0; i < SP * SP; ++i) G[i] = 0;
  if (WIDE) {
    if (threadIdx.x < SP * SP) SmL[threadIdx.x] = dg.S[threadIdx.x];
    __syncthreads();
  } else {
#pragma unroll
    for (int i = 0; i < SP * SP; ++i) Sm[WIDE ? 0 : i] = dg.S[i];
  }
  double acc[1] = {0};
  const size_t stride = (size_t)gridDim.x * BLK;
  for (size_t row = (size_t)blockIdx.x * BLK + threadIdx.x; row < nrows; row += stride) {
    double x[SP], y[SP], gv[SP], pv[SP];
#pragma unroll
    for (int c = 0; c < SP; ++c) { x[c] = dg.X[row * SP + c]; y[c] = dg.Y[row * SP + c]; gv[c] = g[row * SP + c]; }
#pragma unroll
    for (int c = 0; c < SP; ++c) {
      pv[c] = -gv[c];
      r[row * SP + c] = gv[c];
      s[row * SP + c] = 0 * gv[c];
      p[row * SP + c] = pv[c];
      acc[0] += gv[c] * gv[c];
    }
    if (WIDE) asm volatile("" ::: "memory");
#pragma unroll
    for (int b = 0; b < SP; ++b) {
      double t = 0;
#pragma unroll
      for (int a = 0; a < SP; ++a) t += pv[a] * (WIDE ? SmL[a * SP + b] : Sm[WIDE ? 0 : a * SP + b]);
#pragma unroll
      for (int a = 0; a < SP; ++a) G[a * SP + b] += y[a] * pv[b] - x[a] * t;
    }
  }
  store_sym_partials<SP>(G, lds, dg.gpartials);
  __syncthreads();
  block_partials_store_w<1, NW>(acc, lds, partials);
}

__global__ __launch_bounds__(kBlock) void k_cg_gdir_init(const double *__restrict__ partials, int count, int ns,
                                                         const double *__restrict__ slots, int from_slots,
                                                         double *__restrict__ gdir) {
  if (!from_slots) {
    gdir_from_rows(partials, count, ns, gdir);
    return;
  }
  if (threadIdx.x < ns) {
    const double v = slots[threadIdx.x];
    gdir[SLOT_GDIR_P + threadIdx.x] = v;
    gdir[threadIdx.x] = -v;
  }
}

__global__ __launch_bounds__(kBlock) void k_cg_gdir_anchor(const double *__restrict__ partials, int count, int ns,
                                                           const double *__restrict__ slots, int from_slots,
                                                           const CgState *__restrict__ st, double *__restrict__ dst,
                                                           double *__restrict__ dst2) {
  if (st->mode != CG_RUN) return;
  if (!from_slots) {
    gdir_rows_to(partials, count, ns, dst);
    if (dst2) gdir_rows_to(partials + (size_t)ns * kMaxRows, count, ns, dst2);
    return;
  }
  if (threadIdx.x < ns) dst[threadIdx.x] = slots[threadIdx.x];
  if (dst2 && threadIdx.x < ns) dst2[threadIdx.x] = slots[ns + threadIdx.x];
}

__global__ __launch_bounds__(kBlock) void k_cg_peek(CgConst cc, const CgState *__restrict__ st,
                                                    const double *__restrict__ partials_a, int nparts_a,
                                                    unsigned long long *host, unsigned long long *flag,
                                                    unsigned long long seq) {
  __shared__ double lds[3 * (kWaves + 1)];
  CgState cs = load_state(st);
  const int mode_in = cs.mode;
  if (mode_in == CG_RUN) {
    double d[3];
    reduce_rows<3>(partials_a, nparts_a, d, lds);
    step_a(cs, cc, d[0], d[1], d[2]);
  }
  if (threadIdx.x != 0) return;
  host[0] = (unsigned long long)mode_in;
  host[1] = (unsigned long long)cs.mode;
  reinterpret_cast<double *>(host)[2] = cs.alpha;
  host[3] = cs.k;
  __threadfence_system();
  if (flag) __hip_atomic_store(flag, seq, __ATOMIC_RELEASE, __HIP_MEMORY_SCOPE_SYSTEM);
}

__global__ void k_cg_user_stop(CgState *st, HostStatus *hs) {
#pragma clang fp contract(off)
  if (threadIdx.x != 0 || blockIdx.x != 0) return;
  CgState cs = load_state(st);
  if (cs.mode != CG_RUN) return;
  cs.M_norm = sqrt(cs.sk_M_2);
  cs.exit_reason = MI_STPCG_EXIT_USER;
  cs.mode = CG_DONE;
  store_state(st, cs);
  publish(hs, cs.launches, 1);
}

inline void cpu_relax() { __builtin_ia32_pause(); }

}

namespace mi {
int launch_dot3_partials(mi_ctx *ctx, size_t n, const double *x, const double *y, int *nparts) {
  const int grid = grid_for(ctx, n, 4);
  KScope ks(ctx, MI_K_CG_DOT3);
  hipLaunchKernelGGL(k_cg_dot3, dim3(grid), dim3(kBlock), 0, ctx->stream, n, ctx->cg_live, x, y,
                     ctx->partials);
  *nparts = grid;
  return MI_OK;
}
}

extern "C" {

void mi_stpcg_default_params(mi_stpcg_params *p) {
  if (!p) return;
  p->Delta = 1.0;
  p->max_iterations = 1000;
  p->kappa_fgr = .1;
  p->theta = .5;
  p->epsilon = 1e-8;
  p->run_ahead = 0;
  p->constraint_At = 0;
  p->defer_result = 0;
}

static inline double *precon_fail_host(mi_ctx *ctx) { return reinterpret_cast<double *>(ctx->cg_host + 1); }
static int precon_fail_check(mi_ctx *ctx, mi_stpcg_result *result) {
  const double w = *precon_fail_host(ctx);
  if (result) result->precon_status = (int)w;
  if (w != 1.0) return MI_OK;
  set_error("the preconditioner of this solve reported a failed application (code 1: its inner iteration broke down -- "
            "dependent constraint rows, or NaN / Inf in the residual): the result is not a projected step");
  return MI_ERR_INTERNAL;
}

__global__ void k_cg_result_to_host(unsigned long long *host, const unsigned long long *__restrict__ st,
                                    const double *__restrict__ fail_dev, unsigned long long *flag,
                                    unsigned long long seq) {
  constexpr int kWords = (int)(sizeof(CgState) / 8);
  static_assert(sizeof(CgState) % 8 == 0, "CgState is copied in 8-byte words");
  if (threadIdx.x < kWords) host[threadIdx.x] = st[threadIdx.x];
  if (threadIdx.x == kWords) reinterpret_cast<double *>(host)[kWords] = fail_dev ? *fail_dev : 0.0;
  __threadfence_system();
  __syncthreads();
  if (threadIdx.x == 0) __hip_atomic_store(flag, seq, __ATOMIC_RELEASE, __HIP_MEMORY_SCOPE_SYSTEM);
}
static unsigned long long result_to_host(mi_ctx *ctx, const CgState *st_final, const mi_precon *P) {
  unsigned long long *flag = nullptr, *hdev = nullptr;
  unsigned long long seq = poll_begin(ctx, &flag);
  if (!seq) return 0;
  if (hipHostGetDevicePointer((void **)&hdev, ctx->cg_host, 0) != hipSuccess) {
    (void)hipGetLastError();
    return 0;
  }
  hipLaunchKernelGGL(k_cg_result_to_host, dim3(1), dim3(64), 0, ctx->stream, hdev,
                     reinterpret_cast<const unsigned long long *>(st_final),
                     (const double *)(P ? P->fail_word : nullptr), flag, seq);
  if (hipGetLastError() != hipSuccess) return 0;
  return seq;
}

}

namespace {

#define DISPATCH_4(x, NAME, A, B, C, D, ...)                \
  switch (x) {                                              \
    case A: { constexpr int NAME = A; __VA_ARGS__; } break; \
    case B: { constexpr int NAME = B; __VA_ARGS__; } break; \
    case C: { constexpr int NAME = C; __VA_ARGS__; } break; \
    default: { constexpr int NAME = D; __VA_ARGS__; } break; \
  }
#define DISPATCH_PRE(pre, ...) DISPATCH_4(pre, PRE, PRE_NONE, PRE_DIAG, PRE_BLOCK3, PRE_EXTERNAL, __VA_ARGS__)
#define DISPATCH_KC(kc, ...) DISPATCH_4(kc, KC, 4, 6, 9, 16, __VA_ARGS__)
#define DISPATCH_KC_WIDE(kc, ...) DISPATCH_4(kc, KC, 18, 24, 31, 39, __VA_ARGS__)
#define DISPATCH_SP(sp, ...) \
  if ((sp) == 0) { constexpr int SP = 0; __VA_ARGS__; } else DISPATCH_4(sp, SP, 1, 2, 3, 4, __VA_ARGS__)

template <bool SIGMA, int KC>
auto cg_update_recur_kernel() {
  if constexpr (SIGMA && KC == 16) return &k_cg_update_s80<PRE_NONE, false, KC, NoFold>;
  else if constexpr (SIGMA) return &k_cg_update<PRE_NONE, false, KC, NoFold>;
  else if constexpr (KC == 16) return &k_cg_update_ns_s80<PRE_NONE, false, KC, NoFold>;
  else return &k_cg_update_ns<PRE_NONE, false, KC, NoFold>;
}
template <bool FS, int SP>
auto cg_pupdate_kernel() {
  if constexpr (SP == 1 || (FS && SP == 0)) return &k_cg_pupdate_s80<FS, SP, NoFold>;
  else return &k_cg_pupdate<FS, SP, NoFold>;
}

struct StpcgPlan {
  size_t n;
  bool observed, sharded, rows, lockstep, recur, folded, init_fused, gdir_in_scalar_init;
  bool twok, early, defer;
  int pre, run_ahead, grid, gns, sp, kc, reanchor;
  const mi_dirgram *dgp;
  CgConst cc;
};

int stpcg_plan(const mi_ctx *ctx, const mi_op *H, const mi_precon *P, const mi_stpcg_params *prm, size_t n,
               bool observed, StpcgPlan &pl) {
  pl.n = n;
  pl.observed = observed;
  pl.pre = !P ? PRE_NONE : (P->kind == 1 ? PRE_DIAG : (P->kind == 2 ? PRE_BLOCK3 : PRE_EXTERNAL));
  MI_REQUIRE(pl.pre != PRE_BLOCK3 || n % 3 == 0, "block-Jacobi preconditioner needs n divisible by 3");
  pl.sharded = slot_mode(ctx);
  pl.rows = rows_mode(ctx);
  pl.dgp = (!ctx->no_dirgram && H->dirgram && H->apply_dir) ? H->dirgram : nullptr;
  if (pl.dgp && pl.dgp->p > 4 && (pl.pre != PRE_NONE || ctx->dirgram_direct)) pl.dgp = nullptr;
  MI_REQUIRE(!pl.dgp || (pl.dgp->p >= 1 && pl.dgp->p <= kMaxP && pl.dgp->n * (size_t)pl.dgp->p == n),
             "operator's direction-Gram description does not match the problem dimension");
  pl.run_ahead = prm->run_ahead > 0 ? prm->run_ahead : 3;
  pl.lockstep = (ctx->comm != nullptr && ctx->world_size > 1) || ctx->force_lockstep;
  pl.grid = (pl.pre == PRE_BLOCK3) ? grid_for(ctx, n / 3, 2) : grid_for(ctx, n, 4);
  pl.cc = CgConst{prm->Delta, prm->Delta * prm->Delta, prm->epsilon, (unsigned long long)prm->max_iterations, 0ull, 0ull};
  const size_t n2 = n >> 1, step = (size_t)pl.grid * kBlock;
  pl.cc.rag0 = (n2 / step) * step;
  pl.cc.rag_per = (n2 - pl.cc.rag0 + (size_t)pl.grid - 1) / (size_t)pl.grid;
  pl.recur = pl.dgp && pl.pre == PRE_NONE && !ctx->dirgram_direct;
  pl.gns = pl.dgp ? pl.dgp->p * (pl.dgp->p + 1) / 2 : 0;
  pl.sp = (pl.dgp && !pl.recur) ? pl.dgp->p : 0;
  pl.kc = pl.recur ? dir_comps(pl.dgp->p) : 3;
  pl.folded = pl.sharded && pl.recur && pl.kc <= kIpcVals && comm_fold_enabled(ctx) && !ctx->force_slot_path;
  pl.init_fused = pl.recur && n == pl.dgp->n * (size_t)pl.dgp->p;
  pl.gdir_in_scalar_init = pl.recur && !pl.sharded && !pl.rows;
  pl.twok = ctx->cfg.two_kernel_step && pl.recur && pl.dgp->twok && pl.dgp->p == 3 && !pl.sharded && !pl.rows &&
            !pl.lockstep && pl.init_fused && pl.gdir_in_scalar_init && !observed;
  pl.early = !pl.sharded && !pl.rows && pl.sp == 0 && ctx->cfg.early_s && pl.grid <= 512 &&
             pl.cc.rag0 <= 2ull * (size_t)pl.grid * kBlock && (n >> 1) < ((size_t)1 << 31) && !observed;
  pl.defer = !pl.sharded && !pl.rows && !pl.lockstep && !pl.twok && pl.sp == 0 && !pl.early && ctx->cfg.defer_s &&
             !observed;
  pl.reanchor = (pl.recur && !pl.twok && ctx->cfg.reanchor > 0) ? ctx->cfg.reanchor : 0;
  return MI_OK;
}

struct StpcgBufs {
  mi_ctx *ctx;
  mi_vec *r = nullptr, *v = nullptr, *p = nullptr, *p2 = nullptr, *Hp = nullptr;
  bool ok = false;
  const mi_vec *g = nullptr; mi_vec *s_out = nullptr; mi_op *H = nullptr;
  mi_precon *P = nullptr; const mi_stpcg_params *prm = nullptr;
  double *vd = nullptr;
  const double *pred = nullptr;
  DirGramArgs dga{nullptr, nullptr, nullptr, nullptr, nullptr, 0};
  double *slots_g = nullptr, *slots_a = nullptr, *slots_b = nullptr;
  CgState *st0 = nullptr, *st1 = nullptr;
  double *tr = nullptr;
  size_t tcap = 0;
  bool rprime = false;
  unsigned long long *peek_dev = nullptr;
  explicit StpcgBufs(mi_ctx *c) : ctx(c) {}
  StpcgBufs(const StpcgBufs &) = delete;
  StpcgBufs &operator=(const StpcgBufs &) = delete;
  ~StpcgBufs() {
    ctx->cg_live = nullptr;
    comm_halo_fold_drop(ctx);
    if (!ok) (void)hipStreamSynchronize(ctx->stream);
    for (mi_vec *x : {r, p, p2, Hp, v}) mi_vec_destroy(x);
  }
};

int stpcg_bufs(mi_ctx *ctx, const StpcgPlan &pl, const mi_vec *g, mi_op *H, mi_precon *P, const mi_stpcg_params *prm,
               mi_vec *s_out, const mi_stpcg_trace *trace, StpcgBufs &b) {
  const size_t n = pl.n;
  b.g = g, b.s_out = s_out, b.H = H, b.P = P, b.prm = prm;
  MI_TRY(mi_vec_create(ctx, n, &b.r));
  MI_TRY(mi_vec_create(ctx, n, &b.p));
  MI_TRY(mi_vec_create(ctx, n, &b.Hp));
  if (pl.pre != PRE_NONE) MI_TRY(mi_vec_create(ctx, n, &b.v));
  if (pl.defer) MI_TRY(mi_vec_create(ctx, n, &b.p2));
  b.vd = (pl.pre == PRE_NONE) ? b.r->d : b.v->d;
  b.pred = P ? P->data : nullptr;
  if (trace && trace->cap) {
    if (ctx->trace_cap < trace->cap) {
      if (ctx->trace_dev) MI_HIP(hipFree(ctx->trace_dev));
      MI_HIP(hipMalloc((void **)&ctx->trace_dev, 4 * trace->cap * sizeof(double)));
      ctx->trace_cap = trace->cap;
    }
    b.tcap = ctx->trace_cap;
    b.tr = ctx->trace_dev;
  }
  if (pl.dgp)
    b.dga = DirGramArgs{pl.dgp->X, pl.dgp->Y, pl.dgp->S, ctx->partials2, pl.recur ? ctx->scalars + SLOT_GDIR : nullptr,
                        pl.gns};
  b.slots_g = ctx->scalars + SLOT_GRAM, b.slots_a = ctx->scalars + SLOT_CG, b.slots_b = ctx->scalars + SLOT_CG + 4;
  b.st0 = ctx->cg, b.st1 = ctx->cg1;
  if (pl.observed) {
    const hipError_t e = hipHostGetDevicePointer((void **)&b.peek_dev, ctx->cg_host, 0);
    if (e != hipSuccess) return hip_fail(e, "stpcg observer: device address of the pinned words", __FILE__, __LINE__);
  }
  return MI_OK;
}

int stpcg_allreduce(mi_ctx *ctx, const StpcgPlan &pl, double *partials, int count, int k, double *slots) {
  return pl.sharded ? reduce_rows_allreduce(ctx, partials, count, k, slots)
                    : pl.rows ? comm_allreduce_rows(ctx, partials, k) : MI_OK;
}

int launch_dirgram(mi_ctx *ctx, const StpcgPlan &pl, const StpcgBufs &b, const double *vec) {
  DISPATCH_P(pl.dgp->p, hipLaunchKernelGGL(k_cg_dirgram<P>, dim3(pl.grid), dim3(StBlk<P>::threads), 0, ctx->stream,
                                           pl.dgp->n, vec, b.dga));
  return MI_OK;
}
void launch_gdir_anchor(mi_ctx *ctx, const StpcgPlan &pl, const StpcgBufs &b, double *dst, double *dst2) {
  hipLaunchKernelGGL(k_cg_gdir_anchor, dim3(1), dim3(kBlock), 0, ctx->stream, (const double *)ctx->partials2, pl.grid,
                     pl.gns, (const double *)b.slots_g, pl.sharded ? 1 : 0, (const CgState *)b.st0, dst, dst2);
}
template <class K, class FOLD>
void launch_cg_update(K kernel, mi_ctx *ctx, const StpcgPlan &pl, const StpcgBufs &b, int nparts, const FOLD &fold) {
  hipLaunchKernelGGL(kernel, dim3(pl.grid), dim3(kBlock), 0, ctx->stream, pl.n, pl.cc, (const CgState *)b.st0, b.st1,
                     (const double *)ctx->partials, nparts, (const double *)(pl.recur ? b.slots_g : b.slots_a),
                     (const double *)b.p->d, (const double *)b.Hp->d, b.pred, b.s_out->d, b.r->d, b.vd, ctx->partials_b,
                     b.dga, fold);
}
template <class K, class FOLD>
void launch_cg_pupdate(K kernel, mi_ctx *ctx, const StpcgPlan &pl, const StpcgBufs &b, const FOLD &fold) {
  hipLaunchKernelGGL(kernel, dim3(pl.grid), dim3(kBlock), 0, ctx->stream, pl.n, pl.cc, (const CgState *)b.st1, b.st0,
                     (const double *)ctx->partials_b, pl.grid, (const double *)b.slots_b, (const double *)b.vd, b.p->d,
                     b.s_out->d, ctx->status_dev, b.tr, b.tcap, b.dga, fold);
}

int stpcg_precondition(mi_ctx *ctx, const StpcgPlan &pl, StpcgBufs &b, bool first) {
  mi_precon *P = b.P;
  if (P->apply_project) MI_TRY(P->apply_project(P, b.r, b.v, b.prm->constraint_At));
  else MI_TRY(P->apply(P, b.r, b.v));
  hipLaunchKernelGGL(first ? &k_cg_dot_rv<true> : &k_cg_dot_rv<false>, dim3(pl.grid), dim3(kBlock), 0, ctx->stream, pl.n,
                     (const CgState *)(first ? b.st0 : b.st1), (const double *)b.r->d, (const double *)b.v->d, b.p->d,
                     ctx->partials_b);
  return MI_OK;
}

int stpcg_setup(mi_ctx *ctx, const StpcgPlan &pl, StpcgBufs &b) {
  hipStream_t st = ctx->stream;
  const int grid = pl.grid;
  {
    KScope ks(ctx, MI_K_CG_INIT);
    if (pl.init_fused) {
      DISPATCH_P(pl.dgp->p, hipLaunchKernelGGL(k_cg_init_dirgram<P>, dim3(grid), dim3(StBlk<P>::threads), 0, st, pl.dgp->n,
                                               (const double *)b.g->d, b.r->d, b.p->d, b.s_out->d, ctx->partials_b, b.dga));
    } else {
      DISPATCH_PRE(pl.pre, hipLaunchKernelGGL(k_cg_init<PRE>, dim3(grid), dim3(kBlock), 0, st, pl.n, (const double *)b.g->d,
                                              b.pred, b.r->d, b.vd, b.p->d, b.s_out->d, ctx->partials_b));
    }
  }
  if (pl.pre == PRE_EXTERNAL) MI_TRY(stpcg_precondition(ctx, pl, b, true));
  if (pl.dgp) {
    if (!pl.init_fused) MI_TRY(launch_dirgram(ctx, pl, b, b.p->d));
    if (pl.recur && !pl.gdir_in_scalar_init) {
      MI_TRY(stpcg_allreduce(ctx, pl, ctx->partials2, grid, pl.gns, b.slots_g));
      hipLaunchKernelGGL(k_cg_gdir_init, dim3(1), dim3(kBlock), 0, st, (const double *)ctx->partials2, grid, pl.gns,
                         (const double *)b.slots_g, pl.sharded ? 1 : 0, b.dga.gdir);
    }
  }
  const CgSetup cfg{b.prm->Delta, b.prm->kappa_fgr, b.prm->theta, b.prm->epsilon,
                    (unsigned long long)b.prm->max_iterations};
  MI_TRY(stpcg_allreduce(ctx, pl, ctx->partials_b, grid, 1, b.slots_b));
  if (pl.sharded)
    hipLaunchKernelGGL(k_cg_scalar_init<true>, dim3(1), dim3(kBlock), 0, st, b.st0, cfg, (const double *)ctx->partials_b,
                       grid, (const double *)b.slots_b, ctx->status_dev, (const double *)nullptr, 0, 0, (double *)nullptr);
  else
    hipLaunchKernelGGL(k_cg_scalar_init<false>, dim3(1), dim3(kBlock), 0, st, b.st0, cfg, (const double *)ctx->partials_b,
                       grid, (const double *)b.slots_b, ctx->status_dev, (const double *)ctx->partials2, grid, pl.gns,
                       pl.gdir_in_scalar_init ? b.dga.gdir : (double *)nullptr);
  const hipError_t e = hipGetLastError();
  if (e != hipSuccess) return hip_fail(e, "stpcg init launch", __FILE__, __LINE__);
  return MI_OK;
}

int stpcg_reanchor(mi_ctx *ctx, const StpcgPlan &pl, StpcgBufs &b) {
  const int grid = pl.grid, gns = pl.gns;
  if (pl.dgp->p <= 4) {
    DISPATCH_P4(pl.dgp->p, hipLaunchKernelGGL(k_cg_dirgram2<P>, dim3(grid), dim3(kBlock), 0, ctx->stream, pl.dgp->n,
                                              (const CgState *)b.st0, (const double *)b.p->d, (const double *)b.r->d, b.dga));
    MI_TRY(stpcg_allreduce(ctx, pl, ctx->partials2, grid, 2 * gns, b.slots_g));
    launch_gdir_anchor(ctx, pl, b, b.dga.gdir + SLOT_GDIR_P, b.dga.gdir);
  } else {
    for (int which = 0; which < 2; ++which) {
      MI_TRY(launch_dirgram(ctx, pl, b, which == 0 ? b.p->d : b.r->d));
      MI_TRY(stpcg_allreduce(ctx, pl, ctx->partials2, grid, gns, b.slots_g));
      launch_gdir_anchor(ctx, pl, b, b.dga.gdir + (which == 0 ? SLOT_GDIR_P : 0), nullptr);
    }
  }
  return MI_OK;
}

int stpcg_operator(mi_ctx *ctx, const StpcgPlan &pl, StpcgBufs &b, int *nparts) {
  if (pl.dgp) return b.H->apply_dir(b.H, b.p, b.Hp, pl.recur ? -1 : pl.grid, nparts);
  if (b.H->apply_dots) return b.H->apply_dots(b.H, b.p, b.Hp, nparts);
  MI_TRY(b.H->apply(b.H, b.p, b.Hp));
  return launch_dot3_partials(ctx, pl.n, b.p->d, b.Hp->d, nparts);
}

int stpcg_step2(mi_ctx *ctx, const StpcgPlan &pl, StpcgBufs &b, size_t k, CgState **st_final) {
  CgState *cur = (k & 1) ? b.st1 : b.st0, *nxt = (k & 1) ? b.st0 : b.st1;
  int nparts = 0;
  ctx->cg_live = cur;
  ctx->twok_r = b.r->d;
  const int st_op = b.H->apply_dir(b.H, b.p, b.Hp, -2, &nparts);
  ctx->twok_r = nullptr;
  MI_TRY(st_op);
  KScope ks(ctx, MI_K_CG_UPDATE);
  hipLaunchKernelGGL(k_cg_step2<6>, dim3(pl.grid), dim3(kBlock), 0, ctx->stream, pl.n, pl.cc, (const CgState *)cur, nxt,
                     (const double *)ctx->partials, nparts, (const double *)b.Hp->d, b.r->d, b.p->d, b.s_out->d,
                     ctx->status_dev, b.tr, b.tcap, b.dga);
  *st_final = nxt;
  return MI_OK;
}

enum ObserverSays { OBS_GO_ON, OBS_STOP, OBS_LAST_PASS };
int stpcg_observe(mi_ctx *ctx, const StpcgPlan &pl, StpcgBufs &b, mi_stpcg_observer observer, void *observer_user,
                  int nparts, ObserverSays *says) {
  hipStream_t st = ctx->stream;
  ctx->host_syncs++;
  unsigned long long *flag = nullptr;
  const unsigned long long seq = poll_begin(ctx, &flag);
  {
    KScope ks(ctx, MI_K_CG_SCALAR_A);
    hipLaunchKernelGGL(k_cg_peek, dim3(1), dim3(kBlock), 0, st, pl.cc, (const CgState *)b.st0,
                       (const double *)ctx->partials, nparts, b.peek_dev, seq ? flag : (unsigned long long *)nullptr, seq);
  }
  hipError_t e = hipGetLastError();
  if (e != hipSuccess) return hip_fail(e, "stpcg observer peek launch", __FILE__, __LINE__);
  MI_TRY(poll_finish(ctx, seq, "stpcg observer peek"));
  const volatile unsigned long long *pk = reinterpret_cast<const volatile unsigned long long *>(ctx->cg_host);
  const int mode_in = (int)pk[0], mode_a = (int)pk[1];
  *says = OBS_STOP;
  if (mode_in == CG_DONE) return MI_OK;
  if (mode_a != CG_RUN) {
    *says = OBS_LAST_PASS;
    return MI_OK;
  }
  double alpha_k;
  const unsigned long long abits = pk[2];
  memcpy(&alpha_k, &abits, sizeof(alpha_k));
  ctx->cg_in_observer = true;
  const int stop = observer(observer_user, (size_t)pk[3], b.s_out, b.r, b.v ? b.v : b.r, b.p, alpha_k);
  ctx->cg_in_observer = false;
  *says = stop ? OBS_STOP : OBS_GO_ON;
  if (!stop) return MI_OK;
  hipLaunchKernelGGL(k_cg_user_stop, dim3(1), dim3(64), 0, st, b.st0, ctx->status_dev);
  e = hipGetLastError();
  if (e != hipSuccess) return hip_fail(e, "stpcg observer stop launch", __FILE__, __LINE__);
  return MI_OK;
}

int stpcg_astep(mi_ctx *ctx, const StpcgPlan &pl, StpcgBufs &b, size_t k, int nparts) {
  const bool sigma_later = pl.defer && (k & 1);
  FoldArgs fold_a;
  if (pl.folded) fold_a = comm_fold_next(ctx);
  else MI_TRY(stpcg_allreduce(ctx, pl, ctx->partials, nparts, pl.kc, pl.recur ? b.slots_g : b.slots_a));
  KScope ks(ctx, MI_K_CG_UPDATE);
  if (!pl.recur) {
    DISPATCH_PRE(pl.pre, launch_cg_update(pl.sharded    ? &k_cg_update<PRE, true, 3, NoFold>
                                          : sigma_later ? &k_cg_update_ns<PRE, false, 3, NoFold>
                                                        : &k_cg_update<PRE, false, 3, NoFold>,
                                          ctx, pl, b, nparts, NoFold{}));
  } else if (pl.kc > 16) {
    DISPATCH_KC_WIDE(pl.kc, launch_cg_update(pl.sharded    ? &k_cg_update<PRE_NONE, true, KC, NoFold>
                                             : sigma_later ? &k_cg_update_ns<PRE_NONE, false, KC, NoFold>
                                                           : &k_cg_update<PRE_NONE, false, KC, NoFold>,
                                             ctx, pl, b, nparts, NoFold{}));
  } else if (pl.folded) {
    DISPATCH_KC(pl.kc, launch_cg_update(&k_cg_update_s80<PRE_NONE, false, KC, FoldArgs>, ctx, pl, b, nparts, fold_a));
  } else {
    DISPATCH_KC(pl.kc, launch_cg_update(pl.sharded    ? &k_cg_update_s80<PRE_NONE, true, KC, NoFold>
                                        : sigma_later ? cg_update_recur_kernel<false, KC>()
                                                      : cg_update_recur_kernel<true, KC>(),
                                        ctx, pl, b, nparts, NoFold{}));
  }
  return MI_OK;
}

int stpcg_bstep(mi_ctx *ctx, const StpcgPlan &pl, StpcgBufs &b, size_t k) {
  hipStream_t st = ctx->stream;
  const mi_dirgram *dgp = pl.dgp;
  const int grid = pl.grid;
  if (pl.folded) {
    const FoldArgs fold_b = comm_fold_next(ctx);
    FoldPush fp{fold_b, HaloPush{}};
    const bool push = dgp->halo_A && k + 1 < b.prm->max_iterations &&
                      comm_halo_fold_next(ctx, dgp->halo_A, dgp->p, b.p->d, &fp.h);
    KScope ks(ctx, MI_K_CG_PUPDATE);
    if (push) launch_cg_pupdate(&k_cg_pupdate_s80<false, 0, FoldPush>, ctx, pl, b, fp);
    else launch_cg_pupdate(&k_cg_pupdate_s80<false, 0, FoldArgs>, ctx, pl, b, fold_b);
  } else if (pl.sharded) {
    MI_TRY(reduce_rows_allreduce(ctx, ctx->partials_b, grid, 1, b.slots_b));
    if (b.rprime) MI_TRY(comm_rprime_exchange(ctx, dgp->halo_A, dgp->p, b.r->d, nullptr, 0));
    KScope ks(ctx, MI_K_CG_PUPDATE);
    DISPATCH_SP(pl.sp, launch_cg_pupdate(cg_pupdate_kernel<true, SP>(), ctx, pl, b, NoFold{}));
  } else {
    if (pl.rows && b.rprime) MI_TRY(comm_rprime_exchange(ctx, dgp->halo_A, dgp->p, b.r->d, ctx->partials_b, 1));
    else if (pl.rows) MI_TRY(comm_allreduce_rows(ctx, ctx->partials_b, 1));
    KScope ks(ctx, MI_K_CG_PUPDATE);
    if (pl.early) {
      hipLaunchKernelGGL(k_cg_pupdate_early, dim3(grid), dim3(kBlock), 0, st, pl.n, pl.cc, (const CgState *)b.st1, b.st0,
                         (const double *)ctx->partials_b, grid, (const double *)b.vd, b.p->d, b.s_out->d, ctx->status_dev,
                         b.tr, b.tcap, b.dga);
    } else if (pl.defer && ((k & 1) || k + 1 < b.prm->max_iterations)) {
      hipLaunchKernelGGL((k & 1) ? &k_cg_pupdate_ds<true> : &k_cg_pupdate_ds<false>, dim3(grid), dim3(kBlock), 0, st,
                         pl.n, pl.cc, (const CgState *)b.st1, b.st0, (const double *)ctx->partials_b, grid,
                         (const double *)b.vd, (const double *)b.p->d, b.p2->d, b.s_out->d, ctx->status_dev, b.tr,
                         b.tcap, b.dga);
      std::swap(b.p, b.p2);
    } else {
      DISPATCH_SP(pl.sp, launch_cg_pupdate(cg_pupdate_kernel<false, SP>(), ctx, pl, b, NoFold{}));
    }
  }
  if (b.rprime && (pl.sharded || pl.rows)) {
    const double *hr = nullptr;
    double *hp = nullptr;
    size_t cnt = 0;
    comm_rprime_buffers(ctx, dgp->halo_A, dgp->p, &hr, &hp, &cnt);
    if (cnt) {
      const int hg = (int)std::max<size_t>(1, std::min<size_t>((cnt + 255) / 256, 512));
      hipLaunchKernelGGL(k_halo_dir, dim3(hg), dim3(256), 0, st, (const CgState *)b.st0, hr, hp, cnt);
    }
    comm_rprime_mark(ctx, dgp->halo_A, dgp->p, b.p->d);
  }
  return MI_OK;
}

int stpcg_result_from_host(mi_ctx *ctx, mi_stpcg_result *result) {
  int ipc_err = 0;
  (void)mi_comm_ipc_error(ctx, &ipc_err);
  if (ipc_err) {
    set_error("a wait in the peer-memory exchange layer timed out: the result of this solve is invalid");
    return MI_ERR_COMM;
  }
  const CgState &f = *ctx->cg_host;
  result->update_step_M_norm = f.M_norm;
  result->num_iterations = (size_t)f.k;
  result->exit_reason = f.exit_reason;
  result->rv_final = f.rv;
  return precon_fail_check(ctx, result);
}

int stpcg_readback(mi_ctx *ctx, const StpcgPlan &pl, const StpcgBufs &b, const CgState *st_final, mi_stpcg_trace *trace,
                   mi_stpcg_result *result) {
  hipStream_t st = ctx->stream;
  const mi_precon *P = b.P;
  const bool tracing = trace && trace->cap;
  *precon_fail_host(ctx) = 0.0;
  if (b.prm->defer_result && !tracing && !pl.observed) {
    hipError_t e = hipSuccess;
    ctx->cg_deferred_seq = result_to_host(ctx, st_final, P);
    if (!ctx->cg_deferred_seq) {
      if (!ctx->cg_deferred_ev) e = hipEventCreateWithFlags(&ctx->cg_deferred_ev, hipEventDisableTiming);
      if (e == hipSuccess) e = hipMemcpyAsync(ctx->cg_host, st_final, sizeof(CgState), hipMemcpyDeviceToHost, st);
      if (e == hipSuccess && P && P->fail_word)
        e = hipMemcpyAsync(precon_fail_host(ctx), P->fail_word, sizeof(double), hipMemcpyDeviceToHost, st);
      if (e == hipSuccess) e = hipEventRecord(ctx->cg_deferred_ev, st);
    }
    if (e != hipSuccess) return hip_fail(e, "stpcg deferred read-back", __FILE__, __LINE__);
    ctx->cg_deferred = true;
    ctx->cg_deferred_hvp = result->hvp_calls;
    result->update_step_M_norm = result->rv_final = 0;
    result->num_iterations = 0, result->exit_reason = -1, result->precon_status = 0;
    return MI_OK;
  }
  ctx->host_syncs++;
  if (const unsigned long long seq = result_to_host(ctx, st_final, P)) {
    MI_TRY(poll_finish(ctx, seq, "stpcg read-back"));
  } else {
    hipError_t e = hipMemcpyAsync(ctx->cg_host, st_final, sizeof(CgState), hipMemcpyDeviceToHost, st);
    if (e == hipSuccess && P && P->fail_word)
      e = hipMemcpyAsync(precon_fail_host(ctx), P->fail_word, sizeof(double), hipMemcpyDeviceToHost, st);
    if (e == hipSuccess) e = hipStreamSynchronize(st);
    if (e != hipSuccess) return hip_fail(e, "stpcg read-back", __FILE__, __LINE__);
  }
  MI_TRY(stpcg_result_from_host(ctx, result));
  if (tracing) {
    const size_t len = result->num_iterations < trace->cap ? result->num_iterations : trace->cap;
    trace->len = len;
    double *dst[4] = {trace->alpha, trace->beta, trace->kappa, trace->rv};
    for (int c = 0; c < 4; ++c)
      if (dst[c] && len) {
        const hipError_t e = hipMemcpy(dst[c], ctx->trace_dev + (size_t)c * b.tcap, len * sizeof(double),
                                       hipMemcpyDeviceToHost);
        if (e != hipSuccess) return hip_fail(e, "stpcg trace copy", __FILE__, __LINE__);
      }
  }
  return MI_OK;
}

int stpcg_solve(mi_ctx *ctx, const mi_vec *g, mi_op *H, mi_precon *P, const mi_stpcg_params *prm,
                mi_stpcg_observer observer, void *observer_user, mi_vec *s_out, mi_stpcg_result *result,
                mi_stpcg_trace *trace) {
  MI_REQUIRE(ctx && g && H && prm && s_out && result, "null argument");
  MI_REQUIRE(g->ctx == ctx && s_out->ctx == ctx && H->ctx == ctx, "objects belong to another context");
  MI_REQUIRE(g->n == s_out->n && g->n == H->n, "dimension mismatch: g %zu, s %zu, H %zu", g->n,
             s_out->n, H->n);
  MI_REQUIRE(g->d != s_out->d, "g and s_out must not alias");
  MI_REQUIRE(!ctx->cg_in_observer, "a solve was started on this context from inside an STPCG observer");
  const bool observed = observer != nullptr;
  if (observed) {
    const char *why = nullptr;
    if (mi_stpcg_observer_available(ctx, &why) != MI_OK) {
      set_error("mi_stpcg_observed declined: %s", why);
      return MI_DECLINED;
    }
  }
  touch(s_out);
  ctx->fusion.fused_stpcg_solves++;
  MI_REQUIRE(!P || (P->ctx == ctx && P->n == g->n), "preconditioner dimension/context mismatch");
  MI_REQUIRE(!prm->constraint_At || (P && P->apply_project),
             "constraint_At needs a constraint preconditioner (mi_precon_create_constraint)");
  MI_REQUIRE(!(P && P->kind == 3 && ctx->world_size > 1),
             "the constraint preconditioner is single-rank: its reductions are not completed across ranks");
  MI_REQUIRE(prm->Delta > 0, "Trust-region radius (Delta) must be a positive real value");
  MI_REQUIRE(prm->kappa_fgr >= 0 && prm->kappa_fgr < 1,
             "Target fractional reduction of the gradient norm (kappa_fgr) must be a real value in "
             "the range [0,1)");
  MI_REQUIRE(prm->theta >= 0 && prm->theta <= 1,
             "Target superlinear convergence rate (theta) must be a real value in the range [0,1]");
  MI_REQUIRE(prm->epsilon > 0 && prm->epsilon < 1,
             "Relative norm tolerance for declaring a vector to lie in the kernel of H (epsilon) "
             "should be a small positive number in the range (0,1)");

  RangeScope range("mi_stpcg");
  comm_halo_fold_drop(ctx);
  StpcgPlan plan;
  MI_TRY(stpcg_plan(ctx, H, P, prm, g->n, observed, plan));
  const StpcgPlan &pl = plan;
  StpcgBufs b(ctx);
  if (pl.recur && !pl.folded && pl.dgp->halo_A) MI_TRY(comm_rprime_prepare(ctx, pl.dgp->halo_A, &b.rprime));
  if (P && P->fail_word) MI_HIP(hipMemsetAsync(P->fail_word, 0, sizeof(double), ctx->stream));
  MI_TRY(stpcg_bufs(ctx, pl, g, H, P, prm, s_out, trace, b));
  ctx->cg_deferred = false;
  ctx->cg_deferred_seq = 0;
  ctx->epoch++;
  ctx->status->word = 0;
  ctx->status->epoch = ctx->epoch;
  ctx->cg_live = b.st0;
  MI_TRY(stpcg_setup(ctx, pl, b));

  CgState *st_final = b.st0;
  size_t hvp = 0;
  for (size_t k = 0; k < prm->max_iterations; ++k) {
    uint64_t w = ctx->status->word;
    while (!observed && !(w & 1) && k > (w >> 1) + (uint64_t)pl.run_ahead) {
      cpu_relax();
      w = ctx->status->word;
    }
    if (w & 1) {
      if (!pl.lockstep || k >= (w >> 1) + (uint64_t)pl.run_ahead) break;
    }
    if (pl.reanchor && k > 0 && k % (size_t)pl.reanchor == 0) MI_TRY(stpcg_reanchor(ctx, pl, b));
    if (pl.twok) {
      MI_TRY(stpcg_step2(ctx, pl, b, k, &st_final));
      ++hvp;
      continue;
    }
    int nparts = 0;
    MI_TRY(stpcg_operator(ctx, pl, b, &nparts));
    ++hvp;
    ObserverSays says = OBS_GO_ON;
    if (observed) MI_TRY(stpcg_observe(ctx, pl, b, observer, observer_user, nparts, &says));
    if (says == OBS_STOP) break;
    MI_TRY(stpcg_astep(ctx, pl, b, k, nparts));
    if (pl.pre == PRE_EXTERNAL) MI_TRY(stpcg_precondition(ctx, pl, b, false));
    MI_TRY(stpcg_bstep(ctx, pl, b, k));
    if (says == OBS_LAST_PASS) break;
  }
  result->hvp_calls = hvp;
  comm_halo_fold_drop(ctx);
  MI_TRY(stpcg_readback(ctx, pl, b, st_final, trace, result));
  b.ok = true;
  return MI_OK;
}

}

extern "C" {

int mi_stpcg_collect(mi_ctx *ctx, mi_stpcg_result *result) {
  MI_REQUIRE(ctx && result, "null argument");
  MI_REQUIRE(ctx->cg_deferred, "mi_stpcg_collect: no deferred solve is pending on this context");
  ctx->cg_deferred = false;
  if (ctx->cg_deferred_seq) {
    const unsigned long long seq = ctx->cg_deferred_seq;
    ctx->cg_deferred_seq = 0;
    if (__atomic_load_n(ctx->poll_flag, __ATOMIC_ACQUIRE) < seq) {
      ctx->host_syncs++;
      MI_TRY(poll_finish(ctx, seq, "stpcg deferred read-back"));
    }
  } else {
    hipError_t e = hipEventQuery(ctx->cg_deferred_ev);
    if (e == hipErrorNotReady) {
      e = hipEventSynchronize(ctx->cg_deferred_ev);
      ctx->host_syncs++;
    }
    if (e != hipSuccess) return hip_fail(e, "stpcg deferred read-back", __FILE__, __LINE__);
  }
  result->hvp_calls = ctx->cg_deferred_hvp;
  return stpcg_result_from_host(ctx, result);
}

int mi_stpcg_observer_available(mi_ctx *ctx, const char **why) {
  MI_REQUIRE(ctx, "null argument");
  const char *w = nullptr;
  if (ctx->cfg.no_fused_observer) w = "MI355OPT_NO_FUSED_OBSERVER is set";
  else if (ctx->world_size > 1) w = "the context is one of several ranks";
  else if (ctx->force_lockstep) w = "MI355OPT_FORCE_LOCKSTEP is set";
  else if (slot_mode(ctx) || rows_mode(ctx)) w = "the context completes its reductions through an exchange layer";
  if (why) *why = w ? w : "";
  return w ? MI_DECLINED : MI_OK;
}

int mi_stpcg(mi_ctx *ctx, const mi_vec *g, mi_op *H, mi_precon *P, const mi_stpcg_params *prm, mi_vec *s_out,
             mi_stpcg_result *result, mi_stpcg_trace *trace) {
  return stpcg_solve(ctx, g, H, P, prm, nullptr, nullptr, s_out, result, trace);
}

int mi_stpcg_observed(mi_ctx *ctx, const mi_vec *g, mi_op *H, mi_precon *P, const mi_stpcg_params *prm,
                      mi_stpcg_observer fn, void *user, mi_vec *s_out, mi_stpcg_result *result, mi_stpcg_trace *trace) {
  MI_REQUIRE(fn, "mi_stpcg_observed: null observer (mi_stpcg is the solve without one)");
  return stpcg_solve(ctx, g, H, P, prm, fn, user, s_out, result, trace);
}

}
```

### optimization_amd/csrc/stpcg_kernels.inc

```

template <int PRE, bool FROM_SLOTS, int KC = 3, class FOLD = NoFold>
__global__ __launch_bounds__(kBlock) CG_KERNEL_ATTR void CG_UPDATE_NAME(size_t n, CgConst cc, const CgState *__restrict__ st_in,
                                                      CgState *__restrict__ st_out,
                                                      const double *__restrict__ partials_a, int nparts_a,
                                                      const double *__restrict__ slots,
                                                      const double *__restrict__ p,
                                                      const double *__restrict__ Hp,
                                                      const double *__restrict__ pre,
                                                      double *__restrict__ s, double *__restrict__ r,
                                                      double *__restrict__ v,
                                                      double *__restrict__ partials_b, DirGramArgs dg,
                                                      FOLD fold) {
  __shared__ double lds[3 * (kWaves + 1)];
  static_assert(KC >= 3 && KC <= 3 * (kWaves + 1), "3 curvature dots + at most 36 Gram components (p <= 8)");
  CgState cs = load_state(st_in);
  if (cs.mode == CG_DONE) {
    if (blockIdx.x == 0 && threadIdx.x == 0) store_state(st_out, cs);
    return;
  }
  FOLD_STAMP(0);
  const size_t n2 = n >> 1, stride = (size_t)gridDim.x * kBlock;
  const size_t i0 = (size_t)blockIdx.x * kBlock + threadIdx.x;
  auto next_of = [&](size_t i_) -> size_t { return i_ + stride; };
  const size_t ifirst = i0;
  double2 hv0 = make_double2(0, 0), rv0 = hv0;
  constexpr bool kFolded = !std::is_same<FOLD, NoFold>::value;
  auto prefetch_now = [&] {
    if (PRE != PRE_BLOCK3 && ifirst < n2) {
      hv0 = reinterpret_cast<const double2 *>(Hp)[ifirst];
      rv0 = reinterpret_cast<double2 *>(r)[ifirst];
    }
  };
  auto prefetch = [&] {
    if (kFolded && threadIdx.x < 64) return;
    prefetch_now();
  };
  double d[KC];
  if (FROM_SLOTS) {
    prefetch_now();
#pragma unroll
    for (int i = 0; i < KC; ++i) d[i] = slots[i];
  } else {
    reduce_rows<KC>(partials_a, nparts_a, d, lds, prefetch);
    fold_maybe<KC>(d, fold, lds);
    if (kFolded && threadIdx.x < 64) prefetch_now();
    if (!kFolded) FOLD_STAMP(1);
  }
  step_a(cs, cc, d[0], d[1], d[2]);
  if (!kFolded) FOLD_STAMP(5);
  if (blockIdx.x == 0 && threadIdx.x == 0) {
    store_state(st_out, cs);
    if (KC > 3 && cs.mode == CG_RUN) {
#pragma unroll
      for (int i = 0; i < KC - 3; ++i)
        if (i < dg.ns) dg.gdir[i] = dg.gdir[i] + cs.alpha * d[3 + i];
    }
  }

  const int mode = cs.mode;
  double acc[1] = {0};
  if (mode == CG_APPLY_SIGMA) {
    if (!CG_UPDATE_SIGMA) return;
    const double sigma = cs.sigma;
    for (size_t i = i0; i < n2; i += stride) {
      const double2 pv = reinterpret_cast<const double2 *>(p)[i];
      double2 sv = reinterpret_cast<double2 *>(s)[i];
      sv.x += sigma * pv.x; sv.y += sigma * pv.y;
      reinterpret_cast<double2 *>(s)[i] = sv;
    }
    if ((n & 1) && blockIdx.x == 0 && threadIdx.x == 0) s[n - 1] += sigma * p[n - 1];
    return;
  }
  if (mode == CG_KERNEL_PENDING) {
    for (size_t i = i0; i < n2; i += stride) {
      const double2 pv = reinterpret_cast<const double2 *>(p)[i];
      const double2 rv = reinterpret_cast<const double2 *>(r)[i];
      acc[0] += pv.x * rv.x; acc[0] += pv.y * rv.y;
    }
    if ((n & 1) && blockIdx.x == 0 && threadIdx.x == 0) acc[0] += p[n - 1] * r[n - 1];
  } else {
    const double alpha = cs.alpha;
    if (PRE == PRE_BLOCK3) {
      const size_t nb = n / 3;
      for (size_t b = i0; b < nb; b += stride) {
        double rr[3];
#pragma unroll
        for (int c = 0; c < 3; ++c) {
          const size_t i = 3 * b + c;
          rr[c] = r[i] + alpha * Hp[i];
          r[i] = rr[c];
        }
        const double *M = pre + 9 * b;
#pragma unroll
        for (int c = 0; c < 3; ++c) {
          const double vv = M[3 * c] * rr[0] + M[3 * c + 1] * rr[1] + M[3 * c + 2] * rr[2];
          v[3 * b + c] = vv;
          acc[0] += rr[c] * vv;
        }
      }
    } else {
      double2 hv = hv0, rv = rv0;
      for (size_t i = ifirst; i < n2;) {
        const size_t inext = next_of(i);
        double2 hn = hv, rn = rv;
        if (inext < n2) {
          hn = reinterpret_cast<const double2 *>(Hp)[inext];
          rn = reinterpret_cast<double2 *>(r)[inext];
        }
        rv.x += alpha * hv.x; rv.y += alpha * hv.y;
        reinterpret_cast<double2 *>(r)[i] = rv;
        if (PRE != PRE_EXTERNAL) {
          double2 vv = rv;
          if (PRE == PRE_DIAG) {
            const double2 dd = reinterpret_cast<const double2 *>(pre)[i];
            vv.x = dd.x * rv.x; vv.y = dd.y * rv.y;
            reinterpret_cast<double2 *>(v)[i] = vv;
          }
          acc[0] += rv.x * vv.x; acc[0] += rv.y * vv.y;
        }
        i = inext; hv = hn; rv = rn;
      }
      if ((n & 1) && blockIdx.x == 0 && threadIdx.x == 0) {
        const size_t i = n - 1;
        const double rv = r[i] + alpha * Hp[i];
        r[i] = rv;
        if (PRE != PRE_EXTERNAL) {
          double vv = rv;
          if (PRE == PRE_DIAG) { vv = pre[i] * rv; v[i] = vv; }
          acc[0] += rv * vv;
        }
      }
    }
    if (PRE == PRE_EXTERNAL) return;
  }
  block_partials_store<1>(acc, lds, partials_b);
  FOLD_STAMP(6);
}

template <bool FROM_SLOTS, int SP, class FOLD = NoFold>
__global__ __launch_bounds__(kBlock) CG_KERNEL_ATTR void CG_PUPDATE_NAME(size_t n, CgConst cc, const CgState *__restrict__ st_in,
                                                       CgState *__restrict__ st_out,
                                                       const double *__restrict__ partials_b, int nparts_b,
                                                       const double *__restrict__ slots,
                                                       const double *__restrict__ v,
                                                       double *__restrict__ p, double *__restrict__ s,
                                                       HostStatus *hs, double *__restrict__ trace,
                                                       size_t trace_cap, DirGramArgs dg, FOLD fold) {
  __shared__ double lds[DirGramLds<SP>::value];
  CgState cs = load_state(st_in);
  const bool leader = blockIdx.x == 0 && threadIdx.x == 0;
  if (cs.mode == CG_DONE) {
    if (leader) store_state(st_out, cs);
    return;
  }
  const int mode_in = cs.mode;
  const size_t n2 = n >> 1, stride = (size_t)gridDim.x * kBlock;
  const size_t i0 = (size_t)blockIdx.x * kBlock + threadIdx.x;
  const size_t tail0 = cc.rag0, per = cc.rag_per;
  const size_t irem = (threadIdx.x < per) ? tail0 + (size_t)blockIdx.x * per + threadIdx.x : n2;
  auto next_of = [&](size_t i_) -> size_t {
    const size_t j_ = i_ + stride;
    return j_ < tail0 ? j_ : ((i_ < tail0 && irem < n2) ? irem : n2);
  };
  const size_t ifirst = i0 < tail0 ? i0 : (irem < n2 ? irem : n2);
  double2 vv0 = make_double2(0, 0), pv0 = vv0, sv0 = vv0;
  constexpr int SPN = SP > 0 ? SP : 1;
  double rv0[SPN], rp0[SPN], rs0[SPN], rx0[SPN], ry0[SPN];
#pragma unroll
  for (int c = 0; c < SPN; ++c) { rv0[c] = 0; rp0[c] = 0; rs0[c] = 0; rx0[c] = 0; ry0[c] = 0; }
  auto prefetch_now = [&] {
    if (SP > 0) {
      if (mode_in == CG_RUN && i0 < n / SPN) {
#pragma unroll
        for (int c = 0; c < SPN; ++c) {
          rv0[c] = v[i0 * SPN + c];
          rp0[c] = p[i0 * SPN + c];
          rs0[c] = s[i0 * SPN + c];
          rx0[c] = dg.X[i0 * SPN + c];
          ry0[c] = dg.Y[i0 * SPN + c];
        }
      }
    } else if (ifirst < n2) {
      const size_t q0 = halo_phys(fold, ifirst);
      vv0 = reinterpret_cast<const double2 *>(v)[q0];
      pv0 = reinterpret_cast<double2 *>(p)[q0];
      sv0 = reinterpret_cast<double2 *>(s)[q0];
    }
  };
  double red[1] = {0};
  if (mode_in != CG_APPLY_SIGMA && !FROM_SLOTS) {
    reduce_rows<1>(partials_b, nparts_b, red, lds, prefetch_now);
    fold_maybe<1>(red, fold, lds);
  } else {
    prefetch_now();
    if (mode_in != CG_APPLY_SIGMA) red[0] = slots[0];
  }
  step_b(cs, cc, red[0]);
  cs.launches = cs.launches + 1;
  if (leader) {
    store_state(st_out, cs);
    if (mode_in == CG_RUN && trace && cs.k - 1 < trace_cap) {
      const size_t k = (size_t)(cs.k - 1);
      trace[k] = cs.alpha;
      trace[trace_cap + k] = cs.beta;
      trace[2 * trace_cap + k] = cs.kappa;
      trace[3 * trace_cap + k] = cs.rv;
    }
    publish(hs, cs.launches, cs.mode == CG_DONE);
    if (SP == 0 && dg.gdir && mode_in == CG_RUN && cs.mode == CG_RUN) {
      for (int i = 0; i < dg.ns; ++i) dg.gdir[SLOT_GDIR_P + i] = -dg.gdir[i] + cs.beta * dg.gdir[SLOT_GDIR_P + i];
    }
  }
  if (mode_in == CG_KERNEL_PENDING) {
    const double sigma = cs.sigma;
    for (size_t i = i0; i < n2; i += stride) {
      const double2 pv = reinterpret_cast<const double2 *>(p)[i];
      double2 sv = reinterpret_cast<double2 *>(s)[i];
      sv.x += sigma * pv.x; sv.y += sigma * pv.y;
      reinterpret_cast<double2 *>(s)[i] = sv;
    }
    if ((n & 1) && leader) s[n - 1] += sigma * p[n - 1];
  } else if (mode_in == CG_RUN) {
    const double alpha = cs.alpha, beta = cs.beta;
    const bool dir = cs.mode == CG_RUN;
    if (SP > 0) {
      const size_t nrows = n / SPN;
      double Sm[SPN * SPN], G[SPN * SPN];
#pragma unroll
      for (int i = 0; i < SPN * SPN; ++i) { Sm[i] = dg.S[i]; G[i] = 0; }
      double rv[SPN], rp[SPN], rs[SPN], x[SPN], y[SPN];
#pragma unroll
      for (int c = 0; c < SPN; ++c) { rv[c] = rv0[c]; rp[c] = rp0[c]; rs[c] = rs0[c]; x[c] = rx0[c]; y[c] = ry0[c]; }
      for (size_t row = i0; row < nrows;) {
        const size_t rnext = row + stride;
        double vn[SPN], pn[SPN], sn[SPN], xn[SPN], yn[SPN];
#pragma unroll
        for (int c = 0; c < SPN; ++c) { vn[c] = rv[c]; pn[c] = rp[c]; sn[c] = rs[c]; xn[c] = x[c]; yn[c] = y[c]; }
        if (rnext < nrows) {
#pragma unroll
          for (int c = 0; c < SPN; ++c) {
            vn[c] = v[rnext * SPN + c];
            pn[c] = p[rnext * SPN + c];
            sn[c] = s[rnext * SPN + c];
            xn[c] = dg.X[rnext * SPN + c];
            yn[c] = dg.Y[rnext * SPN + c];
          }
        }
#pragma unroll
        for (int c = 0; c < SPN; ++c) {
          rs[c] = rs[c] + alpha * rp[c];
          s[row * SPN + c] = rs[c];
        }
        if (dir) {
#pragma unroll
          for (int c = 0; c < SPN; ++c) {
            rp[c] = -rv[c] + beta * rp[c];
            p[row * SPN + c] = rp[c];
          }
#pragma unroll
          for (int b = 0; b < SPN; ++b) {
            double t = 0;
#pragma unroll
            for (int a = 0; a < SPN; ++a) t += rp[a] * Sm[a * SPN + b];
#pragma unroll
            for (int a = 0; a < SPN; ++a) G[a * SPN + b] += y[a] * rp[b] - x[a] * t;
          }
        }
        row = rnext;
#pragma unroll
        for (int c = 0; c < SPN; ++c) { rv[c] = vn[c]; rp[c] = pn[c]; rs[c] = sn[c]; x[c] = xn[c]; y[c] = yn[c]; }
      }
      if (dir) store_sym_partials<SPN>(G, lds, dg.gpartials);
      return;
    }
    double2 vv = vv0, pv = pv0, sv = sv0;
    bool pushed = false;
    for (size_t L = ifirst; L < n2;) {
      const size_t Lnext = next_of(L), q = halo_phys(fold, L);
      double2 vn = vv, pn = pv, sn = sv;
      if (Lnext < n2) {
        const size_t qn = halo_phys(fold, Lnext);
        vn = reinterpret_cast<const double2 *>(v)[qn];
        pn = reinterpret_cast<double2 *>(p)[qn];
        sn = reinterpret_cast<double2 *>(s)[qn];
      }
      sv.x = sv.x + alpha * pv.x; sv.y = sv.y + alpha * pv.y;
      reinterpret_cast<double2 *>(s)[q] = sv;
      if (dir) {
        pv.x = -vv.x + beta * pv.x; pv.y = -vv.y + beta * pv.y;
        reinterpret_cast<double2 *>(p)[q] = pv;
        pushed |= halo_push_store(fold, q, pv);
        if (L == ifirst) halo_push_first_step_done(fold);
      }
      L = Lnext; vv = vn; pv = pn; sv = sn;
    }
    if ((n & 1) && leader) {
      s[n - 1] = s[n - 1] + alpha * p[n - 1];
      if (dir) p[n - 1] = -v[n - 1] + beta * p[n - 1];
    }
    if (dir) halo_push_finish(fold, pushed);
  }
}
```

Measured before the change: 5930.

## Skip r/s initialization writes in CG setup by reading g directly in first iterations

Adds a lean set-up path, on by default, in which the fused init kernel no longer writes r=g and s=0. The first update kernel reads r from g (passed in the preconditioner slot), and the first two deferred p-update kernels treat s as zero instead of loading it. This removes two full-vector writes and the matching later reads from the set-up. The cost is extra kernel variants, a special case in the loop break logic for k==0, and a CG_DONE fallback that zero-fills s.

```diff
diff --git a/include/mi355opt.h b/include/mi355opt.h
--- a/include/mi355opt.h
+++ b/include/mi355opt.h
@@ -331,6 +331,7 @@
 MI_API int mi_debug_stiefel_hess_form(int p, int gram_count, const size_t traits[9], const int switches[9], int out[14]);
 MI_API int mi_debug_stiefel_hess_form_of(const mi_ctx *ctx, const mi_csr *A, int p, int gram_count, int out[14]);
 MI_API int mi_debug_words16_option(const char *text, int *on);
+MI_API int mi_debug_stpcg_plan(const long in[12], int out[8]);
 MI_API int mi_debug_set_rank(mi_ctx *ctx, int world_size, int rank);
 MI_API int mi_debug_csr_set_halo(mi_csr *A, int p, const double *halo_rows_host);
 MI_API int mi_debug_time_fused_apply(mi_op *op, const mi_vec *in, mi_vec *out, int reps, double *us_per_call);
diff --git a/optimization_amd/build.py b/optimization_amd/build.py
--- a/optimization_amd/build.py
+++ b/optimization_amd/build.py
@@ -31,7 +31,8 @@
 
 def _compile(src, force):
     obj = os.path.join(OBJ, os.path.basename(src) + ".o")
-    deps = glob.glob(os.path.join(CSRC, "*.h")) + glob.glob(os.path.join(ROOT, "include", "*.h")) + \
+    deps = glob.glob(os.path.join(CSRC, "*.h")) + glob.glob(os.path.join(CSRC, "*.inc")) + \
+        glob.glob(os.path.join(ROOT, "include", "*.h")) + \
         glob.glob(os.path.join(HERE, "include", "Optimization", "LinearAlgebra", "DenseSymmetricEigen.h"))
     if not force and not _newer(src, obj, deps):
         return obj, False, ""
diff --git a/optimization_amd/csrc/context.hip b/optimization_amd/csrc/context.hip
--- a/optimization_amd/csrc/context.hip
+++ b/optimization_amd/csrc/context.hip
@@ -240,6 +240,7 @@
 OPT_BOOL(opt_so3_no_rquat, cfg.so3_no_rquat)
 OPT_BOOL(opt_early_s, cfg.early_s)
 OPT_BOOL(opt_defer_s, cfg.defer_s)
+OPT_BOOL(opt_lean_setup, cfg.lean_setup)
 OPT_BOOL(opt_no_fused_observer, cfg.no_fused_observer)
 OPT_BOOL(opt_no_fused_lsqr_observer, cfg.no_fused_lsqr_observer)
 OPT_BOOL(opt_no_update_pair, cfg.no_update_pair)
@@ -284,7 +285,7 @@
     {"WORDS16", opt_words16, true}, {"NO_SPMM_STREAM", opt_no_spmm_stream}, {"NO_SPMM_WIN", opt_no_spmm_win},
     {"NO_SPMM_SWEEP", opt_no_spmm_sweep}, {"SWEEP_ZSEGS", opt_sweep_zsegs, true},
     {"NO_ZERO_COPY", opt_no_zero_copy}, {"NO_POLLED_SYNC", opt_no_polled_sync}, {"WIDE_QUAD", opt_wide_quad, true}, {"WIDE_WINDOW", opt_wide_window, true},
-    {"NO_UPDATE_MFMA", opt_no_update_mfma}, {"HALO_RPRIME", opt_halo_rprime}, {"NO_GRAM_HALF", opt_no_gram_half}, {"SO3_NO_QUAT", opt_so3_no_quat}, {"SO3_NO_RQUAT", opt_so3_no_rquat}, {"EARLY_S", opt_early_s}, {"DEFER_S", opt_defer_s}, {"NO_FUSED_OBSERVER", opt_no_fused_observer}, {"NO_FUSED_LSQR_OBSERVER", opt_no_fused_lsqr_observer}, {"NO_UPDATE_PAIR", opt_no_update_pair}, {"TWO_KERNEL_STEP", opt_two_kernel_step}, {"SO3_SORT_NBR", opt_so3_sort_nbr, true},
+    {"NO_UPDATE_MFMA", opt_no_update_mfma}, {"HALO_RPRIME", opt_halo_rprime}, {"NO_GRAM_HALF", opt_no_gram_half}, {"SO3_NO_QUAT", opt_so3_no_quat}, {"SO3_NO_RQUAT", opt_so3_no_rquat}, {"EARLY_S", opt_early_s}, {"DEFER_S", opt_defer_s}, {"LEAN_SETUP", opt_lean_setup}, {"NO_FUSED_OBSERVER", opt_no_fused_observer}, {"NO_FUSED_LSQR_OBSERVER", opt_no_fused_lsqr_observer}, {"NO_UPDATE_PAIR", opt_no_update_pair}, {"TWO_KERNEL_STEP", opt_two_kernel_step}, {"SO3_SORT_NBR", opt_so3_sort_nbr, true},
     {"WARN_GENERIC", opt_warn_generic}, {"TALL_PROLOGUE", opt_tall_prologue}, {"REANCHOR", opt_reanchor, true},
 };
 bool option_value(const OptionDesc &o, const char *e, long *v) {
diff --git a/optimization_amd/csrc/mi_internal.h b/optimization_amd/csrc/mi_internal.h
--- a/optimization_amd/csrc/mi_internal.h
+++ b/optimization_amd/csrc/mi_internal.h
@@ -131,6 +131,7 @@
   bool halo_rprime = false;
   bool early_s = false;
   bool defer_s = true;
+  bool lean_setup = true;
   bool no_fused_observer = false;
   bool no_fused_lsqr_observer = false;
   bool so3_no_rquat = false;
diff --git a/optimization_amd/csrc/stpcg.hip b/optimization_amd/csrc/stpcg.hip
--- a/optimization_amd/csrc/stpcg.hip
+++ b/optimization_amd/csrc/stpcg.hip
@@ -315,6 +315,11 @@
 
 #define CG_KERNEL_ATTR
 #define CG_UPDATE_SIGMA 1
+#define CG_UPDATE_FIRST 0
+#define CG_R_IN(i) r[i]
+#define CG_R_IN2(i) reinterpret_cast<double2 *>(r)[i]
+#define CG_S_IN2(i) reinterpret_cast<double2 *>(s)[i]
+#define CG_S_ADD(i, x) s[i] += x
 #define CG_UPDATE_NAME k_cg_update
 #define CG_PUPDATE_NAME k_cg_pupdate
 #include "stpcg_kernels.inc"
@@ -345,6 +350,37 @@
 #undef CG_UPDATE_NAME
 #undef CG_PUPDATE_NAME
 #undef CG_UPDATE_SIGMA
+#undef CG_UPDATE_FIRST
+#undef CG_R_IN
+#undef CG_R_IN2
+#undef CG_S_IN2
+#undef CG_S_ADD
+#define CG_UPDATE_SIGMA 1
+#define CG_UPDATE_FIRST 1
+#define CG_R_IN(i) pre[i]
+#define CG_R_IN2(i) reinterpret_cast<const double2 *>(pre)[i]
+#define CG_S_IN2(i) make_double2(0.0, 0.0)
+#define CG_S_ADD(i, x) s[i] = 0.0 + (x)
+#define CG_KERNEL_ATTR
+#define CG_UPDATE_NAME k_cg_first_update
+#define CG_PUPDATE_NAME k_cg_first_pupdate_unused
+#include "stpcg_kernels.inc"
+#undef CG_KERNEL_ATTR
+#undef CG_UPDATE_NAME
+#undef CG_PUPDATE_NAME
+#define CG_KERNEL_ATTR __attribute__((amdgpu_num_sgpr(80), amdgpu_waves_per_eu(8, 8)))
+#define CG_UPDATE_NAME k_cg_first_update_s80
+#define CG_PUPDATE_NAME k_cg_first_pupdate_s80_unused
+#include "stpcg_kernels.inc"
+#undef CG_KERNEL_ATTR
+#undef CG_UPDATE_NAME
+#undef CG_PUPDATE_NAME
+#undef CG_UPDATE_SIGMA
+#undef CG_UPDATE_FIRST
+#undef CG_R_IN
+#undef CG_R_IN2
+#undef CG_S_IN2
+#undef CG_S_ADD
 
 template <class F>
 __device__ __forceinline__ void reduce_rows_1x512(const double *__restrict__ partials, int count, double &out, double *lds,
@@ -472,113 +508,20 @@
 }
 
 
-template <bool FLUSH>
-__global__ __launch_bounds__(kBlock) __attribute__((amdgpu_waves_per_eu(8, 8))) void k_cg_pupdate_ds(
-    size_t n, CgConst cc, const CgState *__restrict__ st_in, CgState *__restrict__ st_out,
-    const double *__restrict__ partials_b, int nparts_b, const double *__restrict__ v, const double *__restrict__ pc,
-    double *__restrict__ px, double *__restrict__ s, HostStatus *hs, double *__restrict__ trace, size_t trace_cap,
-    DirGramArgs dg) {
-  __shared__ double lds[kWaves + 1];
-  CgState cs = load_state(st_in);
-  const bool leader = blockIdx.x == 0 && threadIdx.x == 0;
-  if (cs.mode == CG_DONE) {
-    if (leader) store_state(st_out, cs);
-    return;
-  }
-  const int mode_in = cs.mode;
-  const size_t n2 = n >> 1, stride = (size_t)gridDim.x * kBlock;
-  const size_t i0 = (size_t)blockIdx.x * kBlock + threadIdx.x;
-  const size_t tail0 = cc.rag0, per = cc.rag_per;
-  const size_t irem = (threadIdx.x < per) ? tail0 + (size_t)blockIdx.x * per + threadIdx.x : n2;
-  auto next_of = [&](size_t i_) -> size_t {
-    const size_t j_ = i_ + stride;
-    return j_ < tail0 ? j_ : ((i_ < tail0 && irem < n2) ? irem : n2);
-  };
-  const size_t ifirst = i0 < tail0 ? i0 : (irem < n2 ? irem : n2);
-  double2 vv0 = make_double2(0, 0), pv0 = vv0, ov0 = vv0, sv0 = vv0;
-  auto prefetch_now = [&] {
-    if (ifirst < n2) {
-      vv0 = reinterpret_cast<const double2 *>(v)[ifirst];
-      pv0 = reinterpret_cast<const double2 *>(pc)[ifirst];
-      if (FLUSH) {
-        ov0 = reinterpret_cast<double2 *>(px)[ifirst];
-        sv0 = reinterpret_cast<double2 *>(s)[ifirst];
-      }
-    }
-  };
-  double red[1] = {0};
-  if (mode_in != CG_APPLY_SIGMA) reduce_rows<1>(partials_b, nparts_b, red, lds, prefetch_now);
-  else prefetch_now();
-  step_b(cs, cc, red[0]);
-  cs.launches = cs.launches + 1;
-  const bool dir = mode_in == CG_RUN && cs.mode == CG_RUN;
-  if (leader) {
-    store_state(st_out, cs);
-    if (!FLUSH && dir) st_out->alpha_prev = cs.alpha;
-    if (mode_in == CG_RUN && trace && cs.k - 1 < trace_cap) {
-      const size_t k = (size_t)(cs.k - 1);
-      trace[k] = cs.alpha;
-      trace[trace_cap + k] = cs.beta;
-      trace[2 * trace_cap + k] = cs.kappa;
-      trace[3 * trace_cap + k] = cs.rv;
-    }
-    publish(hs, cs.launches, cs.mode == CG_DONE);
-    if (dg.gdir && dir) {
-      for (int i = 0; i < dg.ns; ++i) dg.gdir[SLOT_GDIR_P + i] = -dg.gdir[i] + cs.beta * dg.gdir[SLOT_GDIR_P + i];
-    }
-  }
-  const double beta = cs.beta;
-  if (FLUSH) {
-    const double alpha_old = st_out->alpha_prev, alpha = mode_in == CG_RUN ? cs.alpha : cs.sigma;
-    double2 vv = vv0, pv = pv0, ov = ov0, sv = sv0;
-    for (size_t i = ifirst; i < n2;) {
-      const size_t inext = next_of(i);
-      double2 vn = vv, pn = pv, on = ov, sn = sv;
-      if (inext < n2) {
-        vn = reinterpret_cast<const double2 *>(v)[inext];
-        pn = reinterpret_cast<const double2 *>(pc)[inext];
-        on = reinterpret_cast<double2 *>(px)[inext];
-        sn = reinterpret_cast<double2 *>(s)[inext];
-      }
-      sv.x = sv.x + alpha_old * ov.x; sv.y = sv.y + alpha_old * ov.y;
-      sv.x = sv.x + alpha * pv.x; sv.y = sv.y + alpha * pv.y;
-      reinterpret_cast<double2 *>(s)[i] = sv;
-      if (dir) {
-        pv.x = -vv.x + beta * pv.x; pv.y = -vv.y + beta * pv.y;
-        reinterpret_cast<double2 *>(px)[i] = pv;
-      }
-      i = inext; vv = vn; pv = pn; ov = on; sv = sn;
-    }
-    if ((n & 1) && leader) {
-      s[n - 1] = s[n - 1] + alpha_old * px[n - 1];
-      s[n - 1] = s[n - 1] + alpha * pc[n - 1];
-      if (dir) px[n - 1] = -v[n - 1] + beta * pc[n - 1];
-    }
-  } else if (dir) {
-    double2 vv = vv0, pv = pv0;
-    for (size_t i = ifirst; i < n2;) {
-      const size_t inext = next_of(i);
-      double2 vn = vv, pn = pv;
-      if (inext < n2) {
-        vn = reinterpret_cast<const double2 *>(v)[inext];
-        pn = reinterpret_cast<const double2 *>(pc)[inext];
-      }
-      pv.x = -vv.x + beta * pv.x; pv.y = -vv.y + beta * pv.y;
-      reinterpret_cast<double2 *>(px)[i] = pv;
-      i = inext; vv = vn; pv = pn;
-    }
-    if ((n & 1) && leader) px[n - 1] = -v[n - 1] + beta * pc[n - 1];
-  } else if (mode_in != CG_APPLY_SIGMA) {
-    const double alpha = mode_in == CG_RUN ? cs.alpha : cs.sigma;
-    for (size_t i = i0; i < n2; i += stride) {
-      const double2 pv = reinterpret_cast<const double2 *>(pc)[i];
-      double2 sv = reinterpret_cast<double2 *>(s)[i];
-      sv.x = sv.x + alpha * pv.x; sv.y = sv.y + alpha * pv.y;
-      reinterpret_cast<double2 *>(s)[i] = sv;
-    }
-    if ((n & 1) && leader) s[n - 1] = s[n - 1] + alpha * pc[n - 1];
-  }
-}
+#define CG_DS_NAME k_cg_pupdate_ds
+#define CG_S_IN(i) s[i]
+#define CG_S_IN2(i) reinterpret_cast<double2 *>(s)[i]
+#include "stpcg_ds_kernel.inc"
+#undef CG_DS_NAME
+#undef CG_S_IN
+#undef CG_S_IN2
+#define CG_DS_NAME k_cg_first_pupdate_ds
+#define CG_S_IN(i) 0.0
+#define CG_S_IN2(i) make_double2(0.0, 0.0)
+#include "stpcg_ds_kernel.inc"
+#undef CG_DS_NAME
+#undef CG_S_IN
+#undef CG_S_IN2
 
 
 template <int NS>
@@ -744,7 +687,7 @@
   store_sym_partials<SP>(Gb, lds, dg.gpartials + (size_t)SymIdx<SP>::NS * kMaxRows);
 }
 
-template <int SP>
+template <int SP, bool LEAN = false>
 __global__ __launch_bounds__(StBlk<SP>::threads) void k_cg_init_dirgram(size_t nrows, const double *__restrict__ g,
                                                             double *__restrict__ r, double *__restrict__ p,
                                                             double *__restrict__ s, double *__restrict__ partials,
@@ -772,8 +715,10 @@
 #pragma unroll
     for (int c = 0; c < SP; ++c) {
       pv[c] = -gv[c];
-      r[row * SP + c] = gv[c];
-      s[row * SP + c] = 0 * gv[c];
+      if (!LEAN) {
+        r[row * SP + c] = gv[c];
+        s[row * SP + c] = 0 * gv[c];
+      }
       p[row * SP + c] = pv[c];
       acc[0] += gv[c] * gv[c];
     }
@@ -952,6 +897,7 @@
   size_t n;
   bool observed, sharded, rows, lockstep, recur, folded, init_fused, gdir_in_scalar_init;
   bool twok, early, defer;
+  bool lean_setup;
   int pre, run_ahead, grid, gns, sp, kc, reanchor;
   const mi_dirgram *dgp;
   CgConst cc;
@@ -990,6 +936,7 @@
   pl.defer = !pl.sharded && !pl.rows && !pl.lockstep && !pl.twok && pl.sp == 0 && !pl.early && ctx->cfg.defer_s &&
              !observed;
   pl.reanchor = (pl.recur && !pl.twok && ctx->cfg.reanchor > 0) ? ctx->cfg.reanchor : 0;
+  pl.lean_setup = ctx->cfg.lean_setup && pl.init_fused && pl.defer && prm->max_iterations > 0;
   return MI_OK;
 }
 
@@ -1072,6 +1019,13 @@
                      (const double *)b.p->d, (const double *)b.Hp->d, b.pred, b.s_out->d, b.r->d, b.vd, ctx->partials_b,
                      b.dga, fold);
 }
+template <class K>
+void launch_cg_first_update(K kernel, mi_ctx *ctx, const StpcgPlan &pl, const StpcgBufs &b, int nparts) {
+  hipLaunchKernelGGL(kernel, dim3(pl.grid), dim3(kBlock), 0, ctx->stream, pl.n, pl.cc, (const CgState *)b.st0, b.st1,
+                     (const double *)ctx->partials, nparts, (const double *)b.slots_g, (const double *)b.p->d,
+                     (const double *)b.Hp->d, (const double *)b.g->d, b.s_out->d, b.r->d, b.vd, ctx->partials_b, b.dga,
+                     NoFold{});
+}
 template <class K, class FOLD>
 void launch_cg_pupdate(K kernel, mi_ctx *ctx, const StpcgPlan &pl, const StpcgBufs &b, const FOLD &fold) {
   hipLaunchKernelGGL(kernel, dim3(pl.grid), dim3(kBlock), 0, ctx->stream, pl.n, pl.cc, (const CgState *)b.st1, b.st0,
@@ -1094,7 +1048,11 @@
   const int grid = pl.grid;
   {
     KScope ks(ctx, MI_K_CG_INIT);
-    if (pl.init_fused) {
+    if (pl.lean_setup) {
+      DISPATCH_P(pl.dgp->p, hipLaunchKernelGGL((k_cg_init_dirgram<P, true>), dim3(grid), dim3(StBlk<P>::threads), 0, st,
+                                               pl.dgp->n, (const double *)b.g->d, b.r->d, b.p->d, b.s_out->d,
+                                               ctx->partials_b, b.dga));
+    } else if (pl.init_fused) {
       DISPATCH_P(pl.dgp->p, hipLaunchKernelGGL(k_cg_init_dirgram<P>, dim3(grid), dim3(StBlk<P>::threads), 0, st, pl.dgp->n,
                                                (const double *)b.g->d, b.r->d, b.p->d, b.s_out->d, ctx->partials_b, b.dga));
     } else {
@@ -1209,7 +1167,13 @@
   if (pl.folded) fold_a = comm_fold_next(ctx);
   else MI_TRY(stpcg_allreduce(ctx, pl, ctx->partials, nparts, pl.kc, pl.recur ? b.slots_g : b.slots_a));
   KScope ks(ctx, MI_K_CG_UPDATE);
-  if (!pl.recur) {
+  if (pl.lean_setup && k == 0) {
+    if (pl.kc > 16) {
+      DISPATCH_KC_WIDE(pl.kc, launch_cg_first_update(&k_cg_first_update<PRE_NONE, false, KC, NoFold>, ctx, pl, b, nparts));
+    } else {
+      DISPATCH_KC(pl.kc, launch_cg_first_update(&k_cg_first_update_s80<PRE_NONE, false, KC, NoFold>, ctx, pl, b, nparts));
+    }
+  } else if (!pl.recur) {
     DISPATCH_PRE(pl.pre, launch_cg_update(pl.sharded    ? &k_cg_update<PRE, true, 3, NoFold>
                                           : sigma_later ? &k_cg_update_ns<PRE, false, 3, NoFold>
                                                         : &k_cg_update<PRE, false, 3, NoFold>,
@@ -1255,6 +1219,12 @@
       hipLaunchKernelGGL(k_cg_pupdate_early, dim3(grid), dim3(kBlock), 0, st, pl.n, pl.cc, (const CgState *)b.st1, b.st0,
                          (const double *)ctx->partials_b, grid, (const double *)b.vd, b.p->d, b.s_out->d, ctx->status_dev,
                          b.tr, b.tcap, b.dga);
+    } else if (pl.lean_setup && k <= 1) {
+      hipLaunchKernelGGL(k ? &k_cg_first_pupdate_ds<true> : &k_cg_first_pupdate_ds<false>, dim3(grid), dim3(kBlock), 0, st,
+                         pl.n, pl.cc, (const CgState *)b.st1, b.st0, (const double *)ctx->partials_b, grid,
+                         (const double *)b.vd, (const double *)b.p->d, b.p2->d, b.s_out->d, ctx->status_dev, b.tr,
+                         b.tcap, b.dga);
+      std::swap(b.p, b.p2);
     } else if (pl.defer && ((k & 1) || k + 1 < b.prm->max_iterations)) {
       hipLaunchKernelGGL((k & 1) ? &k_cg_pupdate_ds<true> : &k_cg_pupdate_ds<false>, dim3(grid), dim3(kBlock), 0, st,
                          pl.n, pl.cc, (const CgState *)b.st1, b.st0, (const double *)ctx->partials_b, grid,
@@ -1402,7 +1372,7 @@
       w = ctx->status->word;
     }
     if (w & 1) {
-      if (!pl.lockstep || k >= (w >> 1) + (uint64_t)pl.run_ahead) break;
+      if ((!pl.lockstep || k >= (w >> 1) + (uint64_t)pl.run_ahead) && !(pl.lean_setup && k == 0)) break;
     }
     if (pl.reanchor && k > 0 && k % (size_t)pl.reanchor == 0) MI_TRY(stpcg_reanchor(ctx, pl, b));
     if (pl.twok) {
@@ -1455,6 +1425,31 @@
   return stpcg_result_from_host(ctx, result);
 }
 
+int mi_debug_stpcg_plan(const long in[12], int out[8]) {
+  MI_REQUIRE(in && out, "null argument");
+  MI_REQUIRE(in[0] >= 0 && in[0] <= kMaxP && in[11] > 0, "p in [0, %d], n > 0", kMaxP);
+  mi_ctx scratch;
+  mi_dirgram dg;
+  mi_op H;
+  mi_precon P;
+  mi_stpcg_params prm;
+  mi_stpcg_default_params(&prm);
+  const size_t n = (size_t)in[11] * (size_t)(in[0] ? in[0] : 1);
+  dg.p = (int)in[0], dg.n = (size_t)in[11], dg.twok = in[6] != 0;
+  H.ctx = &scratch, H.n = n;
+  if (in[0]) H.dirgram = &dg, H.apply_dir = [](mi_op *, const mi_vec *, mi_vec *, int, int *) { return (int)MI_OK; };
+  P.kind = in[1] == 3 ? 0 : (int)in[1];
+  scratch.force_slot_path = in[3] != 0, scratch.force_lockstep = in[4] != 0, scratch.dirgram_direct = in[5] != 0;
+  scratch.cfg.two_kernel_step = in[6] != 0, scratch.cfg.early_s = in[7] != 0, scratch.cfg.defer_s = in[8] != 0;
+  scratch.cfg.lean_setup = in[9] != 0;
+  prm.max_iterations = (size_t)in[10];
+  StpcgPlan pl;
+  MI_TRY(stpcg_plan(&scratch, &H, in[1] ? &P : nullptr, &prm, n, in[2] != 0, pl));
+  const int o[8] = {pl.recur, pl.init_fused, pl.twok, pl.early, pl.defer, pl.lean_setup, pl.sp, pl.kc};
+  for (int i = 0; i < 8; ++i) out[i] = o[i];
+  return MI_OK;
+}
+
 int mi_stpcg_observer_available(mi_ctx *ctx, const char **why) {
   MI_REQUIRE(ctx, "null argument");
   const char *w = nullptr;
diff --git a/optimization_amd/csrc/stpcg_ds_kernel.inc b/optimization_amd/csrc/stpcg_ds_kernel.inc
--- /dev/null
+++ b/optimization_amd/csrc/stpcg_ds_kernel.inc
@@ -0,0 +1,108 @@
+
+template <bool FLUSH>
+__global__ __launch_bounds__(kBlock) __attribute__((amdgpu_waves_per_eu(8, 8))) void CG_DS_NAME(
+    size_t n, CgConst cc, const CgState *__restrict__ st_in, CgState *__restrict__ st_out,
+    const double *__restrict__ partials_b, int nparts_b, const double *__restrict__ v, const double *__restrict__ pc,
+    double *__restrict__ px, double *__restrict__ s, HostStatus *hs, double *__restrict__ trace, size_t trace_cap,
+    DirGramArgs dg) {
+  __shared__ double lds[kWaves + 1];
+  CgState cs = load_state(st_in);
+  const bool leader = blockIdx.x == 0 && threadIdx.x == 0;
+  if (cs.mode == CG_DONE) {
+    if (leader) store_state(st_out, cs);
+    return;
+  }
+  const int mode_in = cs.mode;
+  const size_t n2 = n >> 1, stride = (size_t)gridDim.x * kBlock;
+  const size_t i0 = (size_t)blockIdx.x * kBlock + threadIdx.x;
+  const size_t tail0 = cc.rag0, per = cc.rag_per;
+  const size_t irem = (threadIdx.x < per) ? tail0 + (size_t)blockIdx.x * per + threadIdx.x : n2;
+  auto next_of = [&](size_t i_) -> size_t {
+    const size_t j_ = i_ + stride;
+    return j_ < tail0 ? j_ : ((i_ < tail0 && irem < n2) ? irem : n2);
+  };
+  const size_t ifirst = i0 < tail0 ? i0 : (irem < n2 ? irem : n2);
+  double2 vv0 = make_double2(0, 0), pv0 = vv0, ov0 = vv0, sv0 = vv0;
+  auto prefetch_now = [&] {
+    if (ifirst < n2) {
+      vv0 = reinterpret_cast<const double2 *>(v)[ifirst];
+      pv0 = reinterpret_cast<const double2 *>(pc)[ifirst];
+      if (FLUSH) {
+        ov0 = reinterpret_cast<double2 *>(px)[ifirst];
+        sv0 = CG_S_IN2(ifirst);
+      }
+    }
+  };
+  double red[1] = {0};
+  if (mode_in != CG_APPLY_SIGMA) reduce_rows<1>(partials_b, nparts_b, red, lds, prefetch_now);
+  else prefetch_now();
+  step_b(cs, cc, red[0]);
+  cs.launches = cs.launches + 1;
+  const bool dir = mode_in == CG_RUN && cs.mode == CG_RUN;
+  if (leader) {
+    store_state(st_out, cs);
+    if (!FLUSH && dir) st_out->alpha_prev = cs.alpha;
+    if (mode_in == CG_RUN && trace && cs.k - 1 < trace_cap) {
+      const size_t k = (size_t)(cs.k - 1);
+      trace[k] = cs.alpha;
+      trace[trace_cap + k] = cs.beta;
+      trace[2 * trace_cap + k] = cs.kappa;
+      trace[3 * trace_cap + k] = cs.rv;
+    }
+    publish(hs, cs.launches, cs.mode == CG_DONE);
+    if (dg.gdir && dir) {
+      for (int i = 0; i < dg.ns; ++i) dg.gdir[SLOT_GDIR_P + i] = -dg.gdir[i] + cs.beta * dg.gdir[SLOT_GDIR_P + i];
+    }
+  }
+  const double beta = cs.beta;
+  if (FLUSH) {
+    const double alpha_old = st_out->alpha_prev, alpha = mode_in == CG_RUN ? cs.alpha : cs.sigma;
+    double2 vv = vv0, pv = pv0, ov = ov0, sv = sv0;
+    for (size_t i = ifirst; i < n2;) {
+      const size_t inext = next_of(i);
+      double2 vn = vv, pn = pv, on = ov, sn = sv;
+      if (inext < n2) {
+        vn = reinterpret_cast<const double2 *>(v)[inext];
+        pn = reinterpret_cast<const double2 *>(pc)[inext];
+        on = reinterpret_cast<double2 *>(px)[inext];
+        sn = CG_S_IN2(inext);
+      }
+      sv.x = sv.x + alpha_old * ov.x; sv.y = sv.y + alpha_old * ov.y;
+      sv.x = sv.x + alpha * pv.x; sv.y = sv.y + alpha * pv.y;
+      reinterpret_cast<double2 *>(s)[i] = sv;
+      if (dir) {
+        pv.x = -vv.x + beta * pv.x; pv.y = -vv.y + beta * pv.y;
+        reinterpret_cast<double2 *>(px)[i] = pv;
+      }
+      i = inext; vv = vn; pv = pn; ov = on; sv = sn;
+    }
+    if ((n & 1) && leader) {
+      s[n - 1] = CG_S_IN(n - 1) + alpha_old * px[n - 1];
+      s[n - 1] = s[n - 1] + alpha * pc[n - 1];
+      if (dir) px[n - 1] = -v[n - 1] + beta * pc[n - 1];
+    }
+  } else if (dir) {
+    double2 vv = vv0, pv = pv0;
+    for (size_t i = ifirst; i < n2;) {
+      const size_t inext = next_of(i);
+      double2 vn = vv, pn = pv;
+      if (inext < n2) {
+        vn = reinterpret_cast<const double2 *>(v)[inext];
+        pn = reinterpret_cast<const double2 *>(pc)[inext];
+      }
+      pv.x = -vv.x + beta * pv.x; pv.y = -vv.y + beta * pv.y;
+      reinterpret_cast<double2 *>(px)[i] = pv;
+      i = inext; vv = vn; pv = pn;
+    }
+    if ((n & 1) && leader) px[n - 1] = -v[n - 1] + beta * pc[n - 1];
+  } else if (mode_in != CG_APPLY_SIGMA) {
+    const double alpha = mode_in == CG_RUN ? cs.alpha : cs.sigma;
+    for (size_t i = i0; i < n2; i += stride) {
+      const double2 pv = reinterpret_cast<const double2 *>(pc)[i];
+      double2 sv = CG_S_IN2(i);
+      sv.x = sv.x + alpha * pv.x; sv.y = sv.y + alpha * pv.y;
+      reinterpret_cast<double2 *>(s)[i] = sv;
+    }
+    if ((n & 1) && leader) s[n - 1] = CG_S_IN(n - 1) + alpha * pc[n - 1];
+  }
+}
diff --git a/optimization_amd/csrc/stpcg_kernels.inc b/optimization_amd/csrc/stpcg_kernels.inc
--- a/optimization_amd/csrc/stpcg_kernels.inc
+++ b/optimization_amd/csrc/stpcg_kernels.inc
@@ -13,9 +13,19 @@
                                                       FOLD fold) {
   __shared__ double lds[3 * (kWaves + 1)];
   static_assert(KC >= 3 && KC <= 3 * (kWaves + 1), "3 curvature dots + at most 36 Gram components (p <= 8)");
+  static_assert(!CG_UPDATE_FIRST || (PRE == PRE_NONE && !FROM_SLOTS && std::is_same<FOLD, NoFold>::value),
+                "iteration 0 of the lean set-up: one context, no preconditioner (`pre` carries g)");
   CgState cs = load_state(st_in);
   if (cs.mode == CG_DONE) {
     if (blockIdx.x == 0 && threadIdx.x == 0) store_state(st_out, cs);
+    if (CG_UPDATE_FIRST) {
+      const size_t n2 = n >> 1, stride = (size_t)gridDim.x * kBlock;
+      for (size_t i = (size_t)blockIdx.x * kBlock + threadIdx.x; i < n2; i += stride) {
+        const double2 gv = reinterpret_cast<const double2 *>(pre)[i];
+        reinterpret_cast<double2 *>(s)[i] = make_double2(0 * gv.x, 0 * gv.y);
+      }
+      if ((n & 1) && blockIdx.x == 0 && threadIdx.x == 0) s[n - 1] = 0 * pre[n - 1];
+    }
     return;
   }
   FOLD_STAMP(0);
@@ -28,7 +38,7 @@
   auto prefetch_now = [&] {
     if (PRE != PRE_BLOCK3 && ifirst < n2) {
       hv0 = reinterpret_cast<const double2 *>(Hp)[ifirst];
-      rv0 = reinterpret_cast<double2 *>(r)[ifirst];
+      rv0 = CG_R_IN2(ifirst);
     }
   };
   auto prefetch = [&] {
@@ -64,20 +74,20 @@
     const double sigma = cs.sigma;
     for (size_t i = i0; i < n2; i += stride) {
       const double2 pv = reinterpret_cast<const double2 *>(p)[i];
-      double2 sv = reinterpret_cast<double2 *>(s)[i];
+      double2 sv = CG_S_IN2(i);
       sv.x += sigma * pv.x; sv.y += sigma * pv.y;
       reinterpret_cast<double2 *>(s)[i] = sv;
     }
-    if ((n & 1) && blockIdx.x == 0 && threadIdx.x == 0) s[n - 1] += sigma * p[n - 1];
+    if ((n & 1) && blockIdx.x == 0 && threadIdx.x == 0) CG_S_ADD(n - 1, sigma * p[n - 1]);
     return;
   }
   if (mode == CG_KERNEL_PENDING) {
     for (size_t i = i0; i < n2; i += stride) {
       const double2 pv = reinterpret_cast<const double2 *>(p)[i];
-      const double2 rv = reinterpret_cast<const double2 *>(r)[i];
+      const double2 rv = CG_R_IN2(i);
       acc[0] += pv.x * rv.x; acc[0] += pv.y * rv.y;
     }
-    if ((n & 1) && blockIdx.x == 0 && threadIdx.x == 0) acc[0] += p[n - 1] * r[n - 1];
+    if ((n & 1) && blockIdx.x == 0 && threadIdx.x == 0) acc[0] += p[n - 1] * CG_R_IN(n - 1);
   } else {
     const double alpha = cs.alpha;
     if (PRE == PRE_BLOCK3) {
@@ -105,7 +115,7 @@
         double2 hn = hv, rn = rv;
         if (inext < n2) {
           hn = reinterpret_cast<const double2 *>(Hp)[inext];
-          rn = reinterpret_cast<double2 *>(r)[inext];
+          rn = CG_R_IN2(inext);
         }
         rv.x += alpha * hv.x; rv.y += alpha * hv.y;
         reinterpret_cast<double2 *>(r)[i] = rv;
@@ -122,7 +132,7 @@
       }
       if ((n & 1) && blockIdx.x == 0 && threadIdx.x == 0) {
         const size_t i = n - 1;
-        const double rv = r[i] + alpha * Hp[i];
+        const double rv = CG_R_IN(i) + alpha * Hp[i];
         r[i] = rv;
         if (PRE != PRE_EXTERNAL) {
           double vv = rv;
```

Result: no change. 5951 (median of 6 runs) (+0.4%).
